# WPCLab/OpenSeg3D

Measured on AMD Instinct MI355X. Metric: points/sec fwd+bwd, Waymo 1-sweep ~180k pts @0.1m voxel; logit parity, higher is better.
Workload: dtype f32 storage/accumulate, bf16x3 products; 1 GPU; waymo_one_sweep (BASELINE configs[1]): synthetic scene, 174633 pts/step/GPU, voxel [0.1, 0.1, 0.1], grid [1440, 1440, 64], fwd (attention dropout p=0.1, DropPath) + criterion (ohem_ce+lovasz on 3 heads) + bwd + SGD step; mode=fwdbwd, segmentor=segformer, voxels=108690, parallelism=dp1

## Files before the change

### __graft_entry__.py

```python
import os
import subprocess
import sys

ROOT = os.path.dirname(os.path.abspath(__file__))
CSRC = os.path.join(ROOT, "openseg3d_amd", "csrc")
LIB = os.path.join(CSRC, "libseg3d_hip.so")
HIP_SOURCES = ["scan.hip", "voxelize.hip", "group.hip", "rulebook.hip", "spconv.hip", "spconv_split.hip", "linear_stream.hip", "linear_x6.hip", "spconv_dma.hip", "spconv_tile.hip", "wgrad_split.hip", "wgrad_dense.hip", "wgrad_dense_lds.hip", "window.hip",
               "attention.hip", "attention_fused.hip", "attention_fused_bwd.hip", "attention_small.hip", "rownorm.hip", "segment.hip", "knn.hip", "knn_attention.hip", "class_context.hip", "loss.hip", "loss_pointwise.hip", "lovasz.hip", "eval.hip", "augment.hip", "augment_instance.hip", "instance_extract.hip", "frame.hip"]
HIPCC_FLAGS = ["--offload-arch=gfx950", "-O3", "-std=c++17", "-fPIC", "-ffp-contract=off",
               "-fhip-fp32-correctly-rounded-divide-sqrt", "-Wall", "-Wno-unused-function"]


def _stale(target, deps):
    if not os.path.exists(target):
        return True
    t = os.path.getmtime(target)
    return any(os.path.getmtime(d) > t for d in deps)


def build_hip(force=False, verbose=False):
    hipcc = os.environ.get("HIPCC", "/opt/rocm/bin/hipcc")
    common = [os.path.join(CSRC, "common.hpp"), os.path.join(CSRC, "attn_common.hpp"), os.path.join(CSRC, "attn_dropout.hpp"), os.path.join(CSRC, "attn_fused.hpp"),
              os.path.join(ROOT, "include", "seg3d_hip.h")]
    objs = []
    procs = []
    for src in HIP_SOURCES:
        s = os.path.join(CSRC, src)
        o = os.path.join(CSRC, src.replace(".hip", ".o"))
        objs.append(o)
        if force or _stale(o, [s] + common):
            cmd = [hipcc] + HIPCC_FLAGS + ["-c", s, "-o", o]
            if verbose:
                print(" ".join(cmd))
            procs.append((src, subprocess.Popen(cmd, stdout=subprocess.PIPE, stderr=subprocess.STDOUT)))
    failed = False
    for src, p in procs:
        out, _ = p.communicate()
        if p.returncode != 0:
            failed = True
            sys.stderr.write(f"--- hipcc failed on {src}\n{out.decode()}\n")
        elif verbose and out.strip():
            print(out.decode())
    if failed:
        raise RuntimeError("hipcc failed")
    if force or procs or _stale(LIB, objs):
        subprocess.check_call([hipcc, "--offload-arch=gfx950", "-shared", "-fPIC", "-o", LIB] + objs)
    return LIB


def build():
    build_hip()
    subprocess.check_call(["make", "-C", os.path.join(ROOT, "oracle")], stdout=subprocess.DEVNULL)
    sys.path.insert(0, ROOT)
    import openseg3d_amd
    from openseg3d_amd import _lib
    _lib.load()


def smoke():
    sys.path.insert(0, ROOT)
    from openseg3d_amd import selfcheck
    selfcheck.run_smoke()


if __name__ == "__main__":
    build_hip(force="--force" in sys.argv, verbose=True)
```

### include/seg3d_hip.h

```cpp
#ifndef SEG3D_HIP_H
#define SEG3D_HIP_H

#include <stddef.h>
#include <stdint.h>

#ifdef __cplusplus
extern "C" {
#endif

#define SEG3D_OK 0
#define SEG3D_EINVAL (-1)
#define SEG3D_EWORKSPACE (-2)
#define SEG3D_ELAUNCH (-3)

#define SEG3D_REDUCE_SUM 0
#define SEG3D_REDUCE_MEAN 1
#define SEG3D_REDUCE_MAX 2

int seg3d_abi_version(void);

const char* seg3d_last_error(void);

int seg3d_grid_size(const float* voxel_size, const float* range, int32_t* grid_xyz);

size_t seg3d_voxelize_workspace_bytes(int64_t n_points);
int seg3d_voxelize_f32(const float* points, int64_t n_points, int32_t row_stride, int32_t xyz_col,
                       int32_t batch_col, const float* voxel_size, const float* range,
                       int32_t* voxel_coords, int32_t* point_voxel_ids, int32_t* n_voxels,
                       void* workspace, size_t workspace_bytes, void* stream);
int seg3d_voxelize_f64(const double* points, int64_t n_points, int32_t row_stride, int32_t xyz_col,
                       int32_t batch_col, const float* voxel_size, const float* range,
                       int32_t* voxel_coords, int32_t* point_voxel_ids, int32_t* n_voxels,
                       void* workspace, size_t workspace_bytes, void* stream);

size_t seg3d_voxelize_host_workspace_bytes(int64_t n_points);
int seg3d_voxelize_host_f32(const float* points, int64_t n_points, int32_t row_stride, int32_t xyz_col,
                            int32_t batch_col, const float* voxel_size, const float* range,
                            int32_t* voxel_coords, int32_t* point_voxel_ids, int32_t* n_voxels,
                            void* workspace, size_t workspace_bytes);
int seg3d_voxelize_host_f64(const double* points, int64_t n_points, int32_t row_stride, int32_t xyz_col,
                            int32_t batch_col, const float* voxel_size, const float* range,
                            int32_t* voxel_coords, int32_t* point_voxel_ids, int32_t* n_voxels,
                            void* workspace, size_t workspace_bytes);

int seg3d_cart2polar_f32(const float* points, int64_t n_points, int32_t row_stride, int32_t xyz_col,
                         float* out , void* stream);
int seg3d_cart2polar_f64(const double* points, int64_t n_points, int32_t row_stride, int32_t xyz_col,
                         double* out , void* stream);

size_t seg3d_group_index_workspace_bytes(int64_t n, int64_t n_groups);
int seg3d_group_index(const int32_t* group_ids, int64_t n, int64_t n_groups, int32_t* rank,
                      int32_t* order, int32_t* offsets, void* workspace, size_t workspace_bytes,
                      void* stream);

size_t seg3d_coord_hash_bytes(int64_t m);
int seg3d_coord_hash_build(const int32_t* coords, int64_t m, const int32_t* shape_zyx ,
                           void* table, size_t table_bytes, void* stream);
int seg3d_rulebook_subm(const int32_t* coords, int64_t m, const int32_t* shape_zyx ,
                        const void* table, size_t table_bytes, int32_t* nbr, void* stream);
size_t seg3d_downsample_workspace_bytes(int32_t batch_size, const int32_t* shape_in_zyx );
int seg3d_downsample_coords(const int32_t* coords_in, int64_t m_in,
                            const int32_t* m_in_dev ,
                            int32_t batch_size, const int32_t* shape_in_zyx , int32_t* coords_out,
                            int64_t cap_out, int32_t* m_out , void* workspace, size_t workspace_bytes,
                            void* stream);
int seg3d_rulebook_strided(const int32_t* coords_out, int64_t m_out, int64_t m_in,
                           const int32_t* shape_in_zyx , const void* table_in,
                           size_t table_bytes, int32_t* nbr_fwd, int32_t* nbr_inv, void* stream);

size_t seg3d_spconv_packed_bytes(int32_t cin, int32_t cout, int32_t flags);
int seg3d_spconv_pack_weight(const float* weight, int32_t cin, int32_t cout, int32_t flags,
                             void* w_packed, void* stream);
int seg3d_spconv_fwd(const float* x, const int32_t* nbr, int64_t m_out, int64_t m_in,
                     const void* w_packed, int32_t pack_flags, const float* bias ,
                     int32_t cin, int32_t cout, float* y,
                     const int32_t* row_order ,
                     void* stream);
int seg3d_spconv_fwd_act(const float* x, const int32_t* nbr, int64_t m_out, int64_t m_in, const void* w_packed,
                         int32_t pack_flags, const float* bias , const float* addend ,
                         int32_t relu, int32_t cin, int32_t cout, float* y, const int32_t* row_order ,
                         void* stream);
int seg3d_spconv_fwd_act_bf16(const void* x, int32_t x_bf16, const int32_t* nbr, int64_t m_out, int64_t m_in,
                              const void* w_packed, int32_t pack_flags, const float* bias,
                              const void* addend_bf16, int32_t relu, int32_t cin, int32_t cout, void* y_bf16,
                              const int32_t* row_order, void* stream);
size_t seg3d_spconv_presplit_bytes(int64_t m_in, int32_t cin);
int seg3d_spconv_presplit(const float* x, int64_t m_in, int32_t cin, void* xs, void* stream);
int seg3d_spconv_fwd_presplit(const void* xs, const int32_t* nbr, int64_t m_out, int64_t m_in, const void* w_packed,
                              int32_t pack_flags, const float* bias , const float* addend ,
                              int32_t relu, int32_t cin, int32_t cout, float* y,
                              const int32_t* row_order , void* stream);
size_t seg3d_conv_plan_bytes(int64_t m_out);
size_t seg3d_conv_plan_workspace_bytes(int64_t m_out);
int seg3d_conv_plan_build(const int32_t* coords, const int32_t* nbr, int64_t m_out, void* plan, void* workspace,
                          size_t workspace_bytes, void* stream);
int32_t seg3d_spconv_tiled_supported(int32_t cin, int32_t cout);
int seg3d_spconv_fwd_tiled(const float* x, const int32_t* nbr, const void* plan, int64_t m_out, int64_t m_in,
                           const void* w_packed, int32_t pack_flags, const float* bias ,
                           const float* addend , int32_t relu, int32_t cin, int32_t cout, float* y, void* stream);
int seg3d_spconv_fwd_tiled_bf16(const void* x, int32_t x_bf16, const int32_t* nbr, const void* plan, int64_t m_out,
                                int64_t m_in, const void* w_packed, int32_t pack_flags, const float* bias ,
                                const void* addend_bf16 , int32_t relu, int32_t cin, int32_t cout, void* y_bf16,
                                void* stream);
int seg3d_debug_set_conv_nbt(int32_t nbt);
int seg3d_debug_set_linear_stream(int32_t on);
size_t seg3d_spconv_wgrad_workspace_bytes(int64_t m_out, int32_t cin, int32_t cout);
int seg3d_spconv_wgrad(const float* x, const float* dy, const int32_t* nbr, int64_t m_out,
                       int64_t m_in, int32_t cin, int32_t cout, int32_t flags ,
                       float* dw, void* workspace, size_t workspace_bytes, void* stream);

int seg3d_spconv_wgrad_partials(const float* x, const float* dy, const int32_t* nbr, int64_t m_out, int64_t m_in,
                                int32_t cin, int32_t cout, void* workspace, size_t workspace_bytes, int32_t* chunks,
                                void* stream);
int seg3d_spconv_wgrad_partials_xbf16(const uint16_t* x_bf16, const float* dy, const int32_t* nbr, int64_t m_out,
                                      int64_t m_in, int32_t cin, int32_t cout, void* workspace, size_t workspace_bytes,
                                      int32_t* chunks, void* stream);

size_t seg3d_linear_wgrad_workspace_bytes(int64_t m, int32_t cin, int32_t cout);
int seg3d_linear_wgrad(const float* x, const float* dy, int64_t m, int32_t cin, int32_t cout, float* dw,
                       float* db , void* workspace, size_t workspace_bytes, void* stream);
int seg3d_linear_wgrad_partials(const float* x, const float* dy, int64_t m, int32_t cin, int32_t cout, int32_t with_bias,
                                void* workspace, size_t workspace_bytes, int32_t* chunks, void* stream);
int seg3d_linear_wgrad_partials_xbf16(const uint16_t* x_bf16, const float* dy, int64_t m, int32_t cin, int32_t cout,
                                      int32_t with_bias, void* workspace, size_t workspace_bytes, int32_t* chunks,
                                      void* stream);
int seg3d_debug_set_wgrad_lds(int32_t on);
int seg3d_reduce_partials(const float* part, int32_t chunks, int64_t n, int64_t nw, float* dw, float* db, void* stream);
int seg3d_reduce_partials_batched(const void* jobs, int32_t n_jobs, int64_t total_blocks, void* stream);
size_t seg3d_linear_packed_bytes_f32(int32_t cin, int32_t cout);
int seg3d_linear_pack_weight_f32(const float* weight, int32_t cin, int32_t cout, int32_t transpose,
                                 void* w_packed, void* stream);
int seg3d_linear_fwd_f32(const float* x, int64_t m, const void* w_packed, const float* bias ,
                         int32_t cin, int32_t cout, float* y, void* stream);
size_t seg3d_linear_packed_bytes_x6(int32_t cin, int32_t cout);
int seg3d_linear_pack_weight_x6(const float* weight, int32_t cin, int32_t cout, int32_t transpose, void* w_packed,
                                void* stream);
int seg3d_linear_fwd_x6(const float* x, int64_t m, const void* w_packed, const float* bias ,
                        const float* scale , const float* shift , int32_t relu, int32_t cin,
                        int32_t cout, float* y, void* stream);

typedef struct {
  const float* src;
  void* dst;
  int32_t cin, cout;
  int32_t kk, transpose, flip, reserved;
  int64_t first_block;
} seg3d_pack_job;
int seg3d_pack_weights_batched(const void* jobs, int32_t n_jobs, int64_t total_blocks, void* stream);

size_t seg3d_linear_packed_bytes(int32_t cin, int32_t cout, int32_t transpose);
int seg3d_linear_pack_weight(const float* weight, int32_t cin, int32_t cout, int32_t transpose,
                             void* w_packed, void* stream);
int seg3d_linear_fwd(const float* x, int64_t m, const void* w_packed, const float* bias ,
                     const float* addend , int32_t cin, int32_t cout,
                     float* y, void* stream);
int seg3d_linear_fwd_sum(const float* x, const float* x_add, int64_t m, const void* w_packed, const float* bias,
                         int32_t cin, int32_t cout, float* y, void* stream);
int seg3d_linear_layernorm_fwd(const float* x, int64_t m, const void* w_packed, const float* bias, const float* res,
                               const float* gamma, const float* beta, float eps, int32_t cin, int32_t cout, float* y,
                               void* stream);
int seg3d_linear_fwd_mul(const float* x, int64_t m, const void* w_packed, const float* factor, int32_t cin, int32_t cout,
                         float* y, void* stream);

size_t seg3d_window_partition_workspace_bytes(int64_t m, int32_t batch_size, const int32_t* nwin_xyz);
int seg3d_window_partition(const int32_t* coords, int64_t m, int32_t batch_size,
                           const int32_t* win_xyz, const int32_t* nwin_xyz, const int32_t* shift_xyz,
                           int32_t n_levels, const int32_t* level_lo, const int32_t* level_hi,
                           const int32_t* level_cap, int32_t* win_id, int32_t* in_win, int32_t* rank,
                           int32_t* level, int32_t* slot, int32_t* tok, int32_t* win_start,
                           int32_t* win_count, int32_t* win_tile0, int32_t* tile_item,
                           int32_t* qg_item, int32_t* counts, void* workspace,
                           size_t workspace_bytes, void* stream);

int seg3d_pos_embed(const int32_t* in_win, int64_t m, const int32_t* win_xyz ,
                    const float* inv_freq, int32_t c, float* pos, void* stream);

int seg3d_window_attn_supported(int32_t heads, int32_t dh);
size_t seg3d_window_attn_workspace_bytes(int64_t m, int32_t n_tiles, int32_t heads, int32_t dh);
int seg3d_window_attn_schedule(int32_t n_tiles, int32_t n_chunks, int32_t heads, int32_t dh, float dropout_p, int32_t* out);
int seg3d_window_attn_fwd(const float* q, const float* k, const float* v, int32_t ldq, int32_t ldk,
                          int32_t ldv, const int32_t* tok, const int32_t* win_start,
                          const int32_t* win_count, const int32_t* win_tile0,
                          const int32_t* tile_item, int32_t n_tiles, const int32_t* qg_item,
                          int32_t n_qgroups, int64_t m, int32_t n_windows, int32_t heads, int32_t dh,
                          const float* tau, float tau_min, float dropout_p, uint64_t dropout_seed, float* out,
                          float* lse, void* workspace, size_t workspace_bytes, void* stream);
int seg3d_window_attn_bwd(const float* q, const float* k, const float* v, int32_t ldq, int32_t ldk,
                          int32_t ldv, const float* out, const float* dout, const float* lse,
                          const int32_t* tok, const int32_t* win_start, const int32_t* win_count,
                          const int32_t* win_tile0, const int32_t* tile_item, int32_t n_tiles,
                          const int32_t* qg_item, int32_t n_qgroups, int64_t m, int32_t n_windows,
                          int32_t heads, int32_t dh, const float* tau,
                          float tau_min, float dropout_p, uint64_t dropout_seed, float* dq, float* dk,
                          float* dv, int32_t lddq, int32_t lddk,
                          int32_t lddv, float* dtau, void* workspace, size_t workspace_bytes,
                          void* stream);

int seg3d_layernorm_fwd(const float* x, const float* res, const float* gamma, const float* beta,
                        const float* rowscale, float eps, int64_t m, int32_t c, float* y, float* mean,
                        float* rstd, void* stream);
size_t seg3d_layernorm_bwd_workspace_bytes(int64_t m, int32_t c);
int seg3d_layernorm_bwd(const float* dy, const float* x, const float* mean, const float* rstd,
                        const float* gamma, const float* rowscale, int64_t m, int32_t c, float* dx,
                        float* dgamma, float* dbeta, void* workspace, size_t workspace_bytes, void* stream);
int seg3d_layernorm_bwd_partials(const float* dy, const float* x, const float* mean, const float* rstd,
                                 const float* gamma, const float* rowscale, int64_t m, int32_t c, float* dx,
                                 void* workspace, size_t workspace_bytes, int32_t* nblocks, void* stream);
size_t seg3d_batchnorm_workspace_bytes(int64_t m, int32_t c);
int seg3d_colstats(const float* x, int64_t m, int32_t c, float* sums, void* workspace, size_t workspace_bytes,
                   void* stream);
int seg3d_batchnorm_stats(const float* x, int64_t m, int32_t c, float eps, const float* gamma, const float* beta,
                          float momentum, float* running_mean, float* running_var, float* stats, void* workspace,
                          size_t workspace_bytes, void* stream);
int seg3d_gelu_fwd(const float* h, int64_t n, float* g, float* gp, void* stream);
int seg3d_affine_act(const float* x, const float* res, const float* scale, const float* shift, int32_t relu,
                     int64_t m, int32_t c, float* y, void* stream);
int seg3d_batchnorm_bwd(const float* dy, const float* y, const float* x, const float* mean, const float* rstd,
                        const float* gamma, int32_t relu, int64_t m, int32_t c, float* dx, float* dres,
                        float* sums, void* workspace, size_t workspace_bytes, void* stream);
int seg3d_batchnorm_bwd_reduce(const float* dy, const float* y, const float* x, const float* mean,
                               const float* rstd, int32_t relu, int64_t m, int32_t c, float* sums,
                               void* workspace, size_t workspace_bytes, void* stream);
int seg3d_batchnorm_bwd_apply(const float* dy, const float* y, const float* x, const float* mean,
                              const float* rstd, const float* gamma, const float* sums, const float* inv_count,
                              int32_t relu, int64_t m, int32_t c, float* dx, float* dres, void* stream);

int seg3d_segment_reduce_fwd(const float* x, int32_t c, const int32_t* order, const int32_t* offsets,
                             int64_t n_seg, int32_t mode, float* out, int32_t* argmax, void* stream);
int seg3d_segment_reduce_bwd(const float* dout, int32_t c, const int32_t* seg_of_row, int64_t n,
                             const int32_t* offsets, const int32_t* argmax, int64_t n_seg,
                             int32_t mode, float* dx, void* stream);

int seg3d_knn_attention_fwd(const float* q, const float* k, const float* v, const int32_t* idx,
                            const uint8_t* invalid, const float* keep, int64_t n, int64_t n_src,
                            int32_t n_neighbors, int32_t d, float scale, float* out, float* prob, void* stream);
int seg3d_knn_attention_bwd(const float* q, const float* k, const float* v, const int32_t* idx, const float* keep,
                            const float* prob, const float* dout, const int32_t* pair_order,
                            const int32_t* pair_offsets, int64_t n, int64_t n_src, int32_t n_neighbors, int32_t d,
                            float scale, float* dq, float* dk, float* dv, float* scratch, void* stream);

int seg3d_class_context_fwd(const float* feats, const float* probs, const int32_t* offsets, const int32_t* chunks,
                            const int32_t* chunk_offsets, int32_t n_chunks, int32_t batch, int64_t m,
                            int32_t classes, int32_t c, float scale, float* weights, float* partials, float* stats,
                            float* context, void* stream);
int seg3d_class_context_bwd(const float* feats, const float* weights, const float* dcontext,
                            const int32_t* offsets, const int32_t* chunks, const int32_t* chunk_offsets,
                            int32_t n_chunks, int32_t batch, int64_t m, int32_t classes, int32_t c, float scale,
                            float* dfeats, float* dprobs, float* scratch, void* stream);

int seg3d_gather_rows(const float* feats, const int32_t* ids, int64_t n, int32_t c, float* out,
                      void* stream);

int seg3d_knn_query(const float* xyz, int64_t n, const float* new_xyz, int64_t m, const int32_t* offset,
                    const int32_t* new_offset, int32_t batch_size, int32_t k, int32_t* idx, float* dist2,
                    void* stream);

size_t seg3d_knn_level_workspace_bytes(int64_t n);
int seg3d_knn_level_build(const float* xyz, int64_t n, const int32_t* offset, int32_t batch_size, float cell,
                          float* sorted_xyz, int32_t* src_index, int32_t* cell_end, void* table_keys, int32_t* table_vals,
                          int64_t capacity, void* workspace, size_t workspace_bytes, void* stream);
int seg3d_knn_query_order(const float* new_xyz, int64_t m, const int32_t* new_offset, int32_t batch_size, float cell,
                          int32_t* order, void* workspace, size_t workspace_bytes, void* stream);
int seg3d_parity_order(const int32_t* coords, int64_t m, int32_t* order, void* workspace, size_t workspace_bytes,
                       void* stream);
typedef struct {
  const float* sorted_xyz;
  const int32_t* src_index;
  const int32_t* cell_end;
  const void* table_keys;
  const int32_t* table_vals;
  int64_t capacity;
  float cell;
  int32_t max_ring;
} seg3d_knn_level;
int seg3d_knn_grid_query(const seg3d_knn_level* levels, int32_t n_levels, const float* new_xyz,
                         const int32_t* query_order , int64_t m,
                         const int32_t* offset, const int32_t* new_offset, int32_t batch_size, int32_t k,
                         int32_t* idx, float* dist2, void* stream);

int seg3d_voxel_majority_labels(const uint8_t* point_labels, const int32_t* order, const int32_t* offsets,
                                int64_t n_voxels, int32_t ignore_index, uint8_t* voxel_labels, void* stream);

size_t seg3d_cross_entropy_workspace_bytes(int64_t n);
int seg3d_cross_entropy_fwd(const float* logits, const int64_t* labels, int64_t n, int32_t c, int64_t ignore_index,
                            float keep_thresh, float* lse, float* stats, void* workspace, size_t workspace_bytes,
                            void* stream);
int seg3d_cross_entropy_bwd(const float* logits, const int64_t* labels, const float* lse, const float* stats,
                            const float* grad_out, int64_t n, int32_t c, float* dlogits, void* stream);

size_t seg3d_lovasz_workspace_bytes(int64_t n, int32_t c);
int seg3d_lovasz_softmax_fwd(const float* logits, const int64_t* labels, int64_t n, int32_t c, int64_t ignore_index,
                             int32_t classes_mode, const int32_t* include, const float* class_weight, float* coef,
                             float* stats, void* workspace, size_t workspace_bytes, void* stream);
int seg3d_lovasz_softmax_bwd(const float* logits, const float* coef, const float* stats, const float* grad_out,
                             int64_t n, int32_t c, float* dlogits, void* stream);

size_t seg3d_pointwise_loss_workspace_bytes(int64_t n);
int seg3d_focal_loss_fwd(const float* logits, const int64_t* labels, int64_t n, int32_t c, int64_t ignore_index, float gamma,
                         float alpha, const float* class_weight, int32_t reduction, float* stats, void* workspace,
                         size_t workspace_bytes, void* stream);
int seg3d_focal_loss_bwd(const float* logits, const int64_t* labels, const float* stats, const float* grad_out, int64_t n,
                         int32_t c, int64_t ignore_index, float gamma, float alpha, const float* class_weight,
                         int32_t reduction, float* dlogits, void* stream);

int seg3d_dice_loss_fwd(const float* logits, const int64_t* labels, int64_t n, int32_t c, int64_t ignore_index, float smooth,
                        float exponent, const float* class_weight, float loss_weight, float avg_factor, float* loss,
                        void* workspace, size_t workspace_bytes, void* stream);
int seg3d_dice_loss_bwd(const float* logits, const int64_t* labels, const float* grad_out, int64_t n, int32_t c,
                        int64_t ignore_index, float smooth, float exponent, const float* class_weight, float loss_weight,
                        float avg_factor, float* dlogits, void* stream);

#define SEG3D_TTA_MAX_VIEWS 64
typedef struct {
  float scale, cos_a, sin_a;
  int32_t flip_x, flip_y;
} seg3d_tta_view;
typedef struct {
  int32_t n_views;
  int32_t batch_period;
  seg3d_tta_view views[SEG3D_TTA_MAX_VIEWS];
} seg3d_tta_table;
int seg3d_tta_views_f32(const float* points, int64_t n_points, int32_t dim, const seg3d_tta_table* table, float* out,
                        void* stream);
int seg3d_tta_views_host_f32(const float* points, int64_t n_points, int32_t dim, const seg3d_tta_table* table,
                             float* out);

int seg3d_softmax_accumulate_f32(const float* logits, int64_t n_points, int32_t n_views, int32_t c, int32_t first,
                                 float* acc, void* stream);

#define SEG3D_ARGMAX_MAX_CLASSES 64
int seg3d_argmax_confusion(const float* scores, const int64_t* pred_in, int64_t n_points, int32_t c, int32_t n_views,
                           const void* labels, int32_t label_bytes, int64_t* pred, int64_t* hist, void* stream);

#define SEG3D_AUG_MAX_PASTE 8
typedef struct {
  double paste_cos[SEG3D_AUG_MAX_PASTE];
  double paste_sin[SEG3D_AUG_MAX_PASTE];
  double offset[3];
  float rot_cos, rot_sin;
  float scale;
  int32_t n_paste;
  int32_t flip_x, flip_y;
  int32_t global_on;
  int32_t batch_col;
  float batch_id;
} seg3d_aug_params;

size_t seg3d_aug_polarmix_workspace_bytes(int64_t n1, int64_t n2);
int seg3d_aug_polarmix_map(const void* points1, int64_t n1, const void* points2, int64_t n2, int32_t dim,
                           int32_t point_bytes, const void* labels2, int32_t label_bytes, int32_t swap, double alpha,
                           double beta, const uint8_t* instance_classes, int32_t n_classes, int32_t n_paste, int64_t cap,
                           int32_t* src, uint8_t* op, int32_t* counts, void* workspace, size_t workspace_bytes,
                           void* stream);
int seg3d_aug_polarmix_map_host(const void* points1, int64_t n1, const void* points2, int64_t n2, int32_t dim,
                                int32_t point_bytes, const void* labels2, int32_t label_bytes, int32_t swap, double alpha,
                                double beta, const uint8_t* instance_classes, int32_t n_classes, int32_t n_paste,
                                int64_t cap, int32_t* src, uint8_t* op, int32_t* counts);

size_t seg3d_aug_far_near_workspace_bytes(int64_t n);
int seg3d_aug_far_near(const void* frame1, int64_t n1, const void* frame2, int64_t n2, int32_t dim, int32_t point_bytes,
                       const int32_t* src, const uint8_t* op, int64_t n_map, const int32_t* idx, int64_t n,
                       const seg3d_aug_params* params , float sample_range, uint8_t* far_flag, int32_t* far_idx,
                       int32_t* near_idx, int32_t* counts, void* workspace, size_t workspace_bytes, void* stream);
int seg3d_aug_far_near_host(const void* frame1, int64_t n1, const void* frame2, int64_t n2, int32_t dim, int32_t point_bytes,
                            const int32_t* src, const uint8_t* op, int64_t n_map, const int32_t* idx, int64_t n,
                            const seg3d_aug_params* params, float sample_range, uint8_t* far_flag, int32_t* far_idx,
                            int32_t* near_idx, int32_t* counts);

size_t seg3d_aug_sample_workspace_bytes(int64_t n);
int seg3d_aug_sample_device(const uint8_t* far_flag, int64_t n, int64_t n_samples, uint64_t seed, int32_t* out,
                            void* workspace, size_t workspace_bytes, void* stream);
int seg3d_aug_sample_host(const uint8_t* far_flag, int64_t n, int64_t n_samples, uint64_t seed, int32_t* out);

size_t seg3d_aug_cur_map_workspace_bytes(int64_t m, int64_t n_points);
int seg3d_aug_cur_map(const int32_t* src, int64_t m, const int32_t* cur_point_indices, int64_t n_cur, int64_t n_points,
                      int32_t* cur_pos, int32_t* cur_gather, int32_t* count, void* workspace, size_t workspace_bytes,
                      void* stream);
int seg3d_aug_cur_map_host(const int32_t* src, int64_t m, const int32_t* cur_point_indices, int64_t n_cur, int64_t n_points,
                           int32_t* cur_pos, int32_t* cur_gather, int32_t* count);

int seg3d_aug_apply_f32(const float* frame1, int64_t n1, const float* frame2, int64_t n2, int32_t dim, const int32_t* src,
                        const uint8_t* op, int64_t n_out, const seg3d_aug_params* params, float* out, void* stream);
int seg3d_aug_apply_f64in(const double* frame1, int64_t n1, const double* frame2, int64_t n2, int32_t dim,
                          const int32_t* src, const uint8_t* op, int64_t n_out, const seg3d_aug_params* params, float* out,
                          void* stream);
int seg3d_aug_apply_host_f32(const float* frame1, int64_t n1, const float* frame2, int64_t n2, int32_t dim,
                             const int32_t* src, const uint8_t* op, int64_t n_out, const seg3d_aug_params* params,
                             float* out);
int seg3d_aug_apply_host_f64in(const double* frame1, int64_t n1, const double* frame2, int64_t n2, int32_t dim,
                               const int32_t* src, const uint8_t* op, int64_t n_out, const seg3d_aug_params* params,
                               float* out);

int seg3d_aug_gather(const void* a, int64_t na, const void* b, int64_t nb, int64_t row_bytes, const int32_t* idx, int64_t m,
                     void* out, void* stream);
int seg3d_aug_gather_host(const void* a, int64_t na, const void* b, int64_t nb, int64_t row_bytes, const int32_t* idx,
                          int64_t m, void* out);

#define SEG3D_AUG_MAX_ANGLES 20
typedef struct {
  int64_t row_begin;
  int32_t n_rows;
  int32_t label;
  double height;
  double loc_noise[3];
  double rot_cos, rot_sin;
  int32_t local_on;
  int32_t flip;
  int32_t n_angles;
  int32_t reserved;
  double ang_cos[SEG3D_AUG_MAX_ANGLES];
  double ang_sin[SEG3D_AUG_MAX_ANGLES];
} seg3d_aug_instance_plan;

size_t seg3d_aug_instance_workspace_bytes(int64_t n, int64_t max_instance_rows, int32_t k);
int seg3d_aug_instance_paste(const void* points, int64_t n, int32_t dim, int32_t point_bytes, const void* labels,
                             int32_t label_bytes, const uint8_t* ground_ids, int32_t n_ground, const double* bank,
                             int64_t bank_rows, const seg3d_aug_instance_plan* plans, int32_t k, int64_t cap_add,
                             double* add_points, void* add_labels, int32_t* decisions, int32_t* counts, void* workspace,
                             size_t workspace_bytes, void* stream);
int seg3d_aug_instance_paste_host(const void* points, int64_t n, int32_t dim, int32_t point_bytes, const void* labels,
                                  int32_t label_bytes, const uint8_t* ground_ids, int32_t n_ground, const double* bank,
                                  int64_t bank_rows, const seg3d_aug_instance_plan* plans, int32_t k, int64_t cap_add,
                                  double* add_points, void* add_labels, int32_t* decisions, int32_t* counts);

typedef struct {
  int32_t label;
  int32_t begin;
  int32_t rows;
  int32_t kept;
  double center[3];
  double radius;
  double height;
} seg3d_instance_cluster;
size_t seg3d_instance_extract_workspace_bytes(int64_t n, int32_t cap_clusters);
int seg3d_instance_extract(const void* points, int64_t n, int32_t dim, int32_t point_bytes, const void* labels,
                           int32_t label_bytes, const uint8_t* target_ids, const int32_t* min_points, int32_t k,
                           const uint8_t* ground_ids, int32_t g, double eps, int32_t cap_clusters, int32_t* point_cluster,
                           int32_t* cluster_rows, seg3d_instance_cluster* clusters, int32_t* counts, void* workspace,
                           size_t workspace_bytes, void* stream);
int seg3d_instance_extract_host(const void* points, int64_t n, int32_t dim, int32_t point_bytes, const void* labels,
                                int32_t label_bytes, const uint8_t* target_ids, const int32_t* min_points, int32_t k,
                                const uint8_t* ground_ids, int32_t g, double eps, int32_t cap_clusters,
                                int32_t* point_cluster, int32_t* cluster_rows, seg3d_instance_cluster* clusters,
                                int32_t* counts);

#define SEG3D_FRAME_MAX_SWEEPS 8
typedef struct {
  const void* rows;
  int64_t n_rows;
  int64_t stride;
  double matrix[12];
  double lag;
  int32_t transform;
  int32_t reserved;
} seg3d_sweep;
typedef struct {
  int32_t n_sweeps;
  int32_t reserved;
  seg3d_sweep sweeps[SEG3D_FRAME_MAX_SWEEPS];
} seg3d_sweep_table;
int seg3d_frame_assemble(const seg3d_sweep_table* table, int32_t dim, int32_t point_bytes, void* out_rows,
                         float* out_f32, float* out_collated, float batch_id, void* stream);
int seg3d_frame_assemble_host(const seg3d_sweep_table* table, int32_t dim, int32_t point_bytes, void* out_rows,
                              float* out_f32, float* out_collated, float batch_id);

size_t seg3d_range_image_workspace_bytes(int32_t rows, int32_t cols);
int seg3d_range_image_labels(const void* pred, int32_t pred_bytes, const int32_t* points_ri, int64_t n, int32_t rows,
                             int32_t cols, int32_t n_classes, int32_t* image1, int32_t* image2, int32_t* n_outside,
                             void* workspace, size_t workspace_bytes, void* stream);
int seg3d_range_image_labels_host(const void* pred, int32_t pred_bytes, const int32_t* points_ri, int64_t n, int32_t rows,
                                  int32_t cols, int32_t n_classes, int32_t* image1, int32_t* image2, int32_t* n_outside);

#ifdef __cplusplus
}
#endif
#endif
```

### openseg3d_amd/_lib.py

```python
import ctypes
import os
import re

_HERE = os.path.dirname(os.path.abspath(__file__))
LIB_PATH = os.path.join(_HERE, "csrc", "libseg3d_hip.so")
HEADER_PATH = os.path.join(os.path.dirname(_HERE), "include", "seg3d_hip.h")

OK, EINVAL, EWORKSPACE, ELAUNCH = 0, -1, -2, -3
REDUCE_SUM, REDUCE_MEAN, REDUCE_MAX = 0, 1, 2
ABI_VERSION = 47

_p, _i32, _i64, _sz, _f = ctypes.c_void_p, ctypes.c_int32, ctypes.c_int64, ctypes.c_size_t, ctypes.c_float
_u64 = ctypes.c_uint64
_d = ctypes.c_double

SIGNATURES = {
    "seg3d_abi_version": (ctypes.c_int, []),
    "seg3d_last_error": (ctypes.c_char_p, []),
    "seg3d_grid_size": (ctypes.c_int, [_p, _p, _p]),
    "seg3d_voxelize_workspace_bytes": (_sz, [_i64]),
    "seg3d_voxelize_f32": (ctypes.c_int, [_p, _i64, _i32, _i32, _i32, _p, _p, _p, _p, _p, _p, _sz, _p]),
    "seg3d_voxelize_f64": (ctypes.c_int, [_p, _i64, _i32, _i32, _i32, _p, _p, _p, _p, _p, _p, _sz, _p]),
    "seg3d_voxelize_host_workspace_bytes": (_sz, [_i64]),
    "seg3d_voxelize_host_f32": (ctypes.c_int, [_p, _i64, _i32, _i32, _i32, _p, _p, _p, _p, _p, _p, _sz]),
    "seg3d_voxelize_host_f64": (ctypes.c_int, [_p, _i64, _i32, _i32, _i32, _p, _p, _p, _p, _p, _p, _sz]),
    "seg3d_cart2polar_f32": (ctypes.c_int, [_p, _i64, _i32, _i32, _p, _p]),
    "seg3d_cart2polar_f64": (ctypes.c_int, [_p, _i64, _i32, _i32, _p, _p]),
    "seg3d_group_index_workspace_bytes": (_sz, [_i64, _i64]),
    "seg3d_group_index": (ctypes.c_int, [_p, _i64, _i64, _p, _p, _p, _p, _sz, _p]),
    "seg3d_coord_hash_bytes": (_sz, [_i64]),
    "seg3d_coord_hash_build": (ctypes.c_int, [_p, _i64, _p, _p, _sz, _p]),
    "seg3d_rulebook_subm": (ctypes.c_int, [_p, _i64, _p, _p, _sz, _p, _p]),
    "seg3d_downsample_workspace_bytes": (_sz, [_i32, _p]),
    "seg3d_downsample_coords": (ctypes.c_int, [_p, _i64, _p, _i32, _p, _p, _i64, _p, _p, _sz, _p]),
    "seg3d_rulebook_strided": (ctypes.c_int, [_p, _i64, _i64, _p, _p, _sz, _p, _p, _p]),
    "seg3d_spconv_packed_bytes": (_sz, [_i32, _i32, _i32]),
    "seg3d_spconv_pack_weight": (ctypes.c_int, [_p, _i32, _i32, _i32, _p, _p]),
    "seg3d_spconv_fwd": (ctypes.c_int, [_p, _p, _i64, _i64, _p, _i32, _p, _i32, _i32, _p, _p, _p]),
    "seg3d_spconv_fwd_act": (ctypes.c_int, [_p, _p, _i64, _i64, _p, _i32, _p, _p, _i32, _i32, _i32, _p, _p, _p]),
    "seg3d_spconv_fwd_act_bf16": (ctypes.c_int, [_p, _i32, _p, _i64, _i64, _p, _i32, _p, _p, _i32, _i32, _i32, _p, _p, _p]),
    "seg3d_spconv_presplit_bytes": (_sz, [_i64, _i32]),
    "seg3d_spconv_presplit": (ctypes.c_int, [_p, _i64, _i32, _p, _p]),
    "seg3d_spconv_fwd_presplit": (ctypes.c_int, [_p, _p, _i64, _i64, _p, _i32, _p, _p, _i32, _i32, _i32, _p, _p, _p]),
    "seg3d_conv_plan_bytes": (_sz, [_i64]),
    "seg3d_conv_plan_workspace_bytes": (_sz, [_i64]),
    "seg3d_conv_plan_build": (ctypes.c_int, [_p, _p, _i64, _p, _p, _sz, _p]),
    "seg3d_spconv_tiled_supported": (_i32, [_i32, _i32]),
    "seg3d_spconv_fwd_tiled": (ctypes.c_int, [_p, _p, _p, _i64, _i64, _p, _i32, _p, _p, _i32, _i32, _i32, _p, _p]),
    "seg3d_spconv_fwd_tiled_bf16": (ctypes.c_int, [_p, _i32, _p, _p, _i64, _i64, _p, _i32, _p, _p, _i32, _i32, _i32, _p, _p]),
    "seg3d_debug_set_conv_nbt": (ctypes.c_int, [_i32]),
    "seg3d_debug_set_linear_stream": (ctypes.c_int, [_i32]),
    "seg3d_spconv_wgrad_workspace_bytes": (_sz, [_i64, _i32, _i32]),
    "seg3d_spconv_wgrad": (ctypes.c_int, [_p, _p, _p, _i64, _i64, _i32, _i32, _i32, _p, _p, _sz, _p]),
    "seg3d_spconv_wgrad_partials": (ctypes.c_int, [_p, _p, _p, _i64, _i64, _i32, _i32, _p, _sz, _p, _p]),
    "seg3d_spconv_wgrad_partials_xbf16": (ctypes.c_int, [_p, _p, _p, _i64, _i64, _i32, _i32, _p, _sz, _p, _p]),
    "seg3d_linear_wgrad_partials_xbf16": (ctypes.c_int, [_p, _p, _i64, _i32, _i32, _i32, _p, ctypes.c_size_t, _p, _p]),
    "seg3d_linear_packed_bytes_f32": (ctypes.c_size_t, [_i32, _i32]),
    "seg3d_linear_pack_weight_f32": (ctypes.c_int, [_p, _i32, _i32, _i32, _p, _p]),
    "seg3d_linear_fwd_f32": (ctypes.c_int, [_p, _i64, _p, _p, _i32, _i32, _p, _p]),
    "seg3d_debug_set_wgrad_lds": (ctypes.c_int, [_i32]),
    "seg3d_linear_packed_bytes_x6": (ctypes.c_size_t, [_i32, _i32]),
    "seg3d_linear_pack_weight_x6": (ctypes.c_int, [_p, _i32, _i32, _i32, _p, _p]),
    "seg3d_linear_fwd_x6": (ctypes.c_int, [_p, _i64, _p, _p, _p, _p, _i32, _i32, _i32, _p, _p]),
    "seg3d_pack_weights_batched": (ctypes.c_int, [_p, _i32, _i64, _p]),
    "seg3d_linear_wgrad_workspace_bytes": (ctypes.c_size_t, [_i64, _i32, _i32]),
    "seg3d_linear_wgrad": (ctypes.c_int, [_p, _p, _i64, _i32, _i32, _p, _p, _p, ctypes.c_size_t, _p]),
    "seg3d_linear_wgrad_partials": (ctypes.c_int, [_p, _p, _i64, _i32, _i32, _i32, _p, ctypes.c_size_t, _p, _p]),
    "seg3d_reduce_partials": (ctypes.c_int, [_p, _i32, _i64, _i64, _p, _p, _p]),
    "seg3d_reduce_partials_batched": (ctypes.c_int, [_p, _i32, _i64, _p]),
    "seg3d_linear_packed_bytes": (_sz, [_i32, _i32, _i32]),
    "seg3d_linear_pack_weight": (ctypes.c_int, [_p, _i32, _i32, _i32, _p, _p]),
    "seg3d_linear_fwd": (ctypes.c_int, [_p, _i64, _p, _p, _p, _i32, _i32, _p, _p]),
    "seg3d_linear_fwd_sum": (ctypes.c_int, [_p, _p, _i64, _p, _p, _i32, _i32, _p, _p]),
    "seg3d_linear_fwd_mul": (ctypes.c_int, [_p, _i64, _p, _p, _i32, _i32, _p, _p]),
    "seg3d_linear_layernorm_fwd": (ctypes.c_int, [_p, _i64, _p, _p, _p, _p, _p, ctypes.c_float, _i32, _i32, _p, _p]),
    "seg3d_window_partition_workspace_bytes": (_sz, [_i64, _i32, _p]),
    "seg3d_window_partition": (ctypes.c_int, [_p, _i64, _i32, _p, _p, _p, _i32, _p, _p, _p,
                                              _p, _p, _p, _p, _p, _p, _p, _p, _p, _p, _p, _p, _p, _sz, _p]),
    "seg3d_pos_embed": (ctypes.c_int, [_p, _i64, _p, _p, _i32, _p, _p]),
    "seg3d_window_attn_supported": (ctypes.c_int, [_i32, _i32]),
    "seg3d_window_attn_workspace_bytes": (_sz, [_i64, _i32, _i32, _i32]),
    "seg3d_window_attn_schedule": (ctypes.c_int, [_i32, _i32, _i32, _i32, _f, _p]),
    "seg3d_window_attn_fwd": (ctypes.c_int, [_p, _p, _p, _i32, _i32, _i32, _p, _p, _p, _p, _p, _i32, _p, _i32,
                                             _i64, _i32, _i32, _i32, _p, _f, _f, _u64, _p, _p, _p, _sz, _p]),
    "seg3d_window_attn_bwd": (ctypes.c_int, [_p, _p, _p, _i32, _i32, _i32, _p, _p, _p, _p, _p, _p, _p, _p, _i32, _p,
                                             _i32, _i64, _i32, _i32, _i32, _p, _f, _f, _u64, _p, _p, _p, _i32, _i32, _i32,
                                             _p, _p, _sz, _p]),
    "seg3d_layernorm_fwd": (ctypes.c_int, [_p, _p, _p, _p, _p, _f, _i64, _i32, _p, _p, _p, _p]),
    "seg3d_layernorm_bwd_workspace_bytes": (ctypes.c_size_t, [_i64, _i32]),
    "seg3d_layernorm_bwd": (ctypes.c_int, [_p, _p, _p, _p, _p, _p, _i64, _i32, _p, _p, _p, _p, ctypes.c_size_t, _p]),
    "seg3d_layernorm_bwd_partials": (ctypes.c_int, [_p, _p, _p, _p, _p, _p, _i64, _i32, _p, _p, ctypes.c_size_t, _p, _p]),
    "seg3d_batchnorm_workspace_bytes": (ctypes.c_size_t, [_i64, _i32]),
    "seg3d_colstats": (ctypes.c_int, [_p, _i64, _i32, _p, _p, ctypes.c_size_t, _p]),
    "seg3d_batchnorm_stats": (ctypes.c_int, [_p, _i64, _i32, _f, _p, _p, _f, _p, _p, _p, _p, ctypes.c_size_t, _p]),
    "seg3d_affine_act": (ctypes.c_int, [_p, _p, _p, _p, _i32, _i64, _i32, _p, _p]),
    "seg3d_gelu_fwd": (ctypes.c_int, [_p, _i64, _p, _p, _p]),
    "seg3d_batchnorm_bwd": (ctypes.c_int, [_p, _p, _p, _p, _p, _p, _i32, _i64, _i32, _p, _p, _p, _p, ctypes.c_size_t, _p]),
    "seg3d_batchnorm_bwd_reduce": (ctypes.c_int, [_p, _p, _p, _p, _p, _i32, _i64, _i32, _p, _p, ctypes.c_size_t, _p]),
    "seg3d_batchnorm_bwd_apply": (ctypes.c_int, [_p, _p, _p, _p, _p, _p, _p, _p, _i32, _i64, _i32, _p, _p, _p]),
    "seg3d_segment_reduce_fwd": (ctypes.c_int, [_p, _i32, _p, _p, _i64, _i32, _p, _p, _p]),
    "seg3d_segment_reduce_bwd": (ctypes.c_int, [_p, _i32, _p, _i64, _p, _p, _i64, _i32, _p, _p]),
    "seg3d_voxel_majority_labels": (ctypes.c_int, [_p, _p, _p, _i64, _i32, _p, _p]),
    "seg3d_cross_entropy_workspace_bytes": (ctypes.c_size_t, [_i64]),
    "seg3d_cross_entropy_fwd": (ctypes.c_int, [_p, _p, _i64, _i32, _i64, _f, _p, _p, _p, ctypes.c_size_t, _p]),
    "seg3d_cross_entropy_bwd": (ctypes.c_int, [_p, _p, _p, _p, _p, _i64, _i32, _p, _p]),
    "seg3d_lovasz_workspace_bytes": (ctypes.c_size_t, [_i64, _i32]),
    "seg3d_lovasz_softmax_fwd": (ctypes.c_int, [_p, _p, _i64, _i32, _i64, _i32, _p, _p, _p, _p, _p, ctypes.c_size_t, _p]),
    "seg3d_lovasz_softmax_bwd": (ctypes.c_int, [_p, _p, _p, _p, _i64, _i32, _p, _p]),
    "seg3d_pointwise_loss_workspace_bytes": (ctypes.c_size_t, [_i64]),
    "seg3d_focal_loss_fwd": (ctypes.c_int, [_p, _p, _i64, _i32, _i64, _f, _f, _p, _i32, _p, _p, ctypes.c_size_t, _p]),
    "seg3d_focal_loss_bwd": (ctypes.c_int, [_p, _p, _p, _p, _i64, _i32, _i64, _f, _f, _p, _i32, _p, _p]),
    "seg3d_dice_loss_fwd": (ctypes.c_int, [_p, _p, _i64, _i32, _i64, _f, _f, _p, _f, _f, _p, _p, ctypes.c_size_t, _p]),
    "seg3d_dice_loss_bwd": (ctypes.c_int, [_p, _p, _p, _i64, _i32, _i64, _f, _f, _p, _f, _f, _p, _p]),
    "seg3d_knn_level_workspace_bytes": (ctypes.c_size_t, [_i64]),
    "seg3d_knn_level_build": (ctypes.c_int, [_p, _i64, _p, _i32, _f, _p, _p, _p, _p, _p, _i64, _p, ctypes.c_size_t, _p]),
    "seg3d_parity_order": (ctypes.c_int, [_p, _i64, _p, _p, ctypes.c_size_t, _p]),
    "seg3d_knn_query_order": (ctypes.c_int, [_p, _i64, _p, _i32, _f, _p, _p, ctypes.c_size_t, _p]),
    "seg3d_knn_grid_query": (ctypes.c_int, [_p, _i32, _p, _p, _i64, _p, _p, _i32, _i32, _p, _p, _p]),
    "seg3d_knn_query": (ctypes.c_int, [_p, _i64, _p, _i64, _p, _p, _i32, _i32, _p, _p, _p]),
    "seg3d_gather_rows": (ctypes.c_int, [_p, _p, _i64, _i32, _p, _p]),
    "seg3d_class_context_fwd": (ctypes.c_int, [_p, _p, _p, _p, _p, _i32, _i32, _i64, _i32, _i32, _f, _p, _p, _p, _p, _p]),
    "seg3d_class_context_bwd": (ctypes.c_int, [_p, _p, _p, _p, _p, _p, _i32, _i32, _i64, _i32, _i32, _f, _p, _p, _p, _p]),
    "seg3d_knn_attention_fwd": (ctypes.c_int, [_p, _p, _p, _p, _p, _p, _i64, _i64, _i32, _i32, _f, _p, _p, _p]),
    "seg3d_knn_attention_bwd": (ctypes.c_int, [_p, _p, _p, _p, _p, _p, _p, _p, _p, _i64, _i64, _i32, _i32, _f, _p, _p, _p, _p, _p]),
    "seg3d_tta_views_f32": (ctypes.c_int, [_p, _i64, _i32, _p, _p, _p]),
    "seg3d_tta_views_host_f32": (ctypes.c_int, [_p, _i64, _i32, _p, _p]),
    "seg3d_softmax_accumulate_f32": (ctypes.c_int, [_p, _i64, _i32, _i32, _i32, _p, _p]),
    "seg3d_argmax_confusion": (ctypes.c_int, [_p, _p, _i64, _i32, _i32, _p, _i32, _p, _p, _p]),
    "seg3d_aug_polarmix_workspace_bytes": (_sz, [_i64, _i64]),
    "seg3d_aug_polarmix_map": (ctypes.c_int, [_p, _i64, _p, _i64, _i32, _i32, _p, _i32, _i32, _d, _d, _p, _i32, _i32, _i64,
                                              _p, _p, _p, _p, _sz, _p]),
    "seg3d_aug_polarmix_map_host": (ctypes.c_int, [_p, _i64, _p, _i64, _i32, _i32, _p, _i32, _i32, _d, _d, _p, _i32, _i32,
                                                   _i64, _p, _p, _p]),
    "seg3d_aug_far_near_workspace_bytes": (_sz, [_i64]),
    "seg3d_aug_far_near": (ctypes.c_int, [_p, _i64, _p, _i64, _i32, _i32, _p, _p, _i64, _p, _i64, _p, _f, _p, _p, _p, _p,
                                          _p, _sz, _p]),
    "seg3d_aug_far_near_host": (ctypes.c_int, [_p, _i64, _p, _i64, _i32, _i32, _p, _p, _i64, _p, _i64, _p, _f, _p, _p, _p,
                                               _p]),
    "seg3d_aug_sample_workspace_bytes": (_sz, [_i64]),
    "seg3d_aug_sample_device": (ctypes.c_int, [_p, _i64, _i64, _u64, _p, _p, _sz, _p]),
    "seg3d_aug_sample_host": (ctypes.c_int, [_p, _i64, _i64, _u64, _p]),
    "seg3d_aug_cur_map_workspace_bytes": (_sz, [_i64, _i64]),
    "seg3d_aug_cur_map": (ctypes.c_int, [_p, _i64, _p, _i64, _i64, _p, _p, _p, _p, _sz, _p]),
    "seg3d_aug_cur_map_host": (ctypes.c_int, [_p, _i64, _p, _i64, _i64, _p, _p, _p]),
    "seg3d_aug_apply_f32": (ctypes.c_int, [_p, _i64, _p, _i64, _i32, _p, _p, _i64, _p, _p, _p]),
    "seg3d_aug_apply_f64in": (ctypes.c_int, [_p, _i64, _p, _i64, _i32, _p, _p, _i64, _p, _p, _p]),
    "seg3d_aug_apply_host_f32": (ctypes.c_int, [_p, _i64, _p, _i64, _i32, _p, _p, _i64, _p, _p]),
    "seg3d_aug_apply_host_f64in": (ctypes.c_int, [_p, _i64, _p, _i64, _i32, _p, _p, _i64, _p, _p]),
    "seg3d_aug_gather": (ctypes.c_int, [_p, _i64, _p, _i64, _i64, _p, _i64, _p, _p]),
    "seg3d_aug_gather_host": (ctypes.c_int, [_p, _i64, _p, _i64, _i64, _p, _i64, _p]),
    "seg3d_aug_instance_workspace_bytes": (_sz, [_i64, _i64, _i32]),
    "seg3d_aug_instance_paste": (ctypes.c_int, [_p, _i64, _i32, _i32, _p, _i32, _p, _i32, _p, _i64, _p, _i32, _i64, _p, _p,
                                                _p, _p, _p, _sz, _p]),
    "seg3d_aug_instance_paste_host": (ctypes.c_int, [_p, _i64, _i32, _i32, _p, _i32, _p, _i32, _p, _i64, _p, _i32, _i64, _p,
                                                     _p, _p, _p]),
    "seg3d_instance_extract_workspace_bytes": (_sz, [_i64, _i32]),
    "seg3d_instance_extract": (ctypes.c_int, [_p, _i64, _i32, _i32, _p, _i32, _p, _p, _i32, _p, _i32, _d, _i32, _p, _p, _p, _p,
                                              _p, _sz, _p]),
    "seg3d_instance_extract_host": (ctypes.c_int, [_p, _i64, _i32, _i32, _p, _i32, _p, _p, _i32, _p, _i32, _d, _i32, _p, _p, _p,
                                                   _p]),
    "seg3d_frame_assemble": (ctypes.c_int, [_p, _i32, _i32, _p, _p, _p, _f, _p]),
    "seg3d_frame_assemble_host": (ctypes.c_int, [_p, _i32, _i32, _p, _p, _p, _f]),
    "seg3d_range_image_workspace_bytes": (_sz, [_i32, _i32]),
    "seg3d_range_image_labels": (ctypes.c_int, [_p, _i32, _p, _i64, _i32, _i32, _i32, _p, _p, _p, _p, _sz, _p]),
    "seg3d_range_image_labels_host": (ctypes.c_int, [_p, _i32, _p, _i64, _i32, _i32, _i32, _p, _p, _p]),
}

_ERR = {EINVAL: "SEG3D_EINVAL (bad argument)", EWORKSPACE: "SEG3D_EWORKSPACE (workspace too small)",
        ELAUNCH: "SEG3D_ELAUNCH (HIP launch/runtime error)"}

_lib = None


class Seg3dError(RuntimeError):
    pass


def header_symbols():
    with open(HEADER_PATH) as f:
        text = f.read()
    text = re.sub(r"/\*.*?\*/", "", text, flags=re.S)
    return sorted(set(re.findall(r"\b(seg3d_[a-z0-9_]+)\s*\(", text)))


def load():
    global _lib
    if _lib is not None:
        return _lib
    if not os.path.exists(LIB_PATH):
        raise Seg3dError(
            f"{LIB_PATH} not found: the HIP library is required (no CPU fallback). "
            "Build it with `python __graft_entry__.py`.")
    import torch
    lib = ctypes.CDLL(LIB_PATH)
    for name, (res, args) in SIGNATURES.items():
        fn = getattr(lib, name)
        fn.restype = res
        fn.argtypes = args
    if lib.seg3d_abi_version() != ABI_VERSION:
        raise Seg3dError(f"libseg3d_hip.so ABI {lib.seg3d_abi_version()} != binding {ABI_VERSION}")
    _lib = lib
    return lib


def call(name, *args):
    lib = load()
    rc = getattr(lib, name)(*args)
    if rc != OK:
        detail = ""
        if rc == ELAUNCH:
            text = lib.seg3d_last_error()
            detail = f": {text.decode(errors='replace')}" if text else ""
        raise Seg3dError(f"{name} failed: {_ERR.get(rc, rc)}{detail}")


def query(name, *args):
    return int(getattr(load(), name)(*args))
```

### openseg3d_amd/csrc/loss.hip

```cpp
#include "common.hpp"

namespace {

constexpr int kThreads = 256;
constexpr int kMaxBlocks = 1024;

__global__ __launch_bounds__(kThreads) void ce_fwd_kernel(const float* __restrict__ x, const int64_t* __restrict__ label,
                                                          int64_t n, int c, int64_t ignore_index, float keep_thresh,
                                                          float* __restrict__ lse,
                                                          float* __restrict__ part ) {
    float loss = 0.f, cnt = 0.f;
    for (int64_t r = (int64_t)blockIdx.x * kThreads + threadIdx.x; r < n; r += (int64_t)gridDim.x * kThreads) {
        const float* row = x + r * c;
        float m = row[0];
        for (int j = 1; j < c; ++j) m = fmaxf(m, row[j]);
        float s = 0.f;
        for (int j = 0; j < c; ++j) s += expf(row[j] - m);
        const float l = m + logf(s);
        const int64_t y = label[r];
        bool counted = y != ignore_index && y >= 0 && y < c;
        if (counted && keep_thresh > 0.f) counted = expf(row[y] - m) / s < keep_thresh;
        lse[r] = counted ? l : INFINITY;
        if (counted) {
            loss += l - row[y];
            cnt += 1.f;
        }
    }
    for (int off = 32; off > 0; off >>= 1) {
        loss += __shfl_xor(loss, off, SEG3D_WAVE);
        cnt += __shfl_xor(cnt, off, SEG3D_WAVE);
    }
    __shared__ float red[2][kThreads / 64];
    if ((threadIdx.x & 63) == 0) {
        red[0][threadIdx.x >> 6] = loss;
        red[1][threadIdx.x >> 6] = cnt;
    }
    __syncthreads();
    if (threadIdx.x == 0) {
        float a = 0.f, b = 0.f;
        for (int w = 0; w < kThreads / 64; ++w) {
            a += red[0][w];
            b += red[1][w];
        }
        part[2 * blockIdx.x] = a;
        part[2 * blockIdx.x + 1] = b;
    }
}

__global__ __launch_bounds__(kThreads) void ce_finalize_kernel(const float* __restrict__ part, int nblocks,
                                                               float* __restrict__ out) {
    float a = 0.f, b = 0.f;
    for (int i = threadIdx.x; i < nblocks; i += kThreads) {
        a += part[2 * i];
        b += part[2 * i + 1];
    }
    for (int off = 32; off > 0; off >>= 1) {
        a += __shfl_xor(a, off, SEG3D_WAVE);
        b += __shfl_xor(b, off, SEG3D_WAVE);
    }
    __shared__ float red[2][kThreads / 64];
    if ((threadIdx.x & 63) == 0) {
        red[0][threadIdx.x >> 6] = a;
        red[1][threadIdx.x >> 6] = b;
    }
    __syncthreads();
    if (threadIdx.x == 0) {
        float sa = 0.f, sb = 0.f;
        for (int w = 0; w < kThreads / 64; ++w) {
            sa += red[0][w];
            sb += red[1][w];
        }
        out[0] = sb > 0.f ? sa / sb : 0.f;
        out[1] = sb;
    }
}

__global__ __launch_bounds__(kThreads) void ce_bwd_kernel(const float* __restrict__ x, const int64_t* __restrict__ label,
                                                          const float* __restrict__ lse, const float* __restrict__ stats,
                                                          const float* __restrict__ gout, int64_t n, int c,
                                                          float* __restrict__ dx) {
    const float cnt = stats[1];
    const float scale = cnt > 0.f ? gout[0] / cnt : 0.f;
    const int64_t total = n * c;
    for (int64_t e = (int64_t)blockIdx.x * kThreads + threadIdx.x; e < total; e += (int64_t)gridDim.x * kThreads) {
        const int64_t r = e / c;
        const int j = (int)(e - r * c);
        const float l = lse[r];
        float g = 0.f;
        if (l != INFINITY) g = (expf(x[e] - l) - (j == label[r] ? 1.f : 0.f)) * scale;
        dx[e] = g;
    }
}

}

extern "C" size_t seg3d_cross_entropy_workspace_bytes(int64_t n) {
    return n < 0 ? 0 : (size_t)kMaxBlocks * 2 * sizeof(float);
}

extern "C" int seg3d_cross_entropy_fwd(const float* logits, const int64_t* labels, int64_t n, int32_t c,
                                       int64_t ignore_index, float keep_thresh, float* lse,
                                       float* stats ,
                                       void* workspace, size_t workspace_bytes, void* stream) {
    if (n < 0 || c <= 0 || c > 4096 || !stats || !workspace || workspace_bytes < seg3d_cross_entropy_workspace_bytes(n))
        return SEG3D_EINVAL;
    if (n > 0 && (!logits || !labels || !lse)) return SEG3D_EINVAL;
    hipStream_t st = as_stream(stream);
    float* part = static_cast<float*>(workspace);
    int nb = (int)(n > 0 ? ceil_div64(n, kThreads) : 0);
    if (nb > kMaxBlocks) nb = kMaxBlocks;
    if (nb > 0) {
        hipLaunchKernelGGL(ce_fwd_kernel, dim3((unsigned)nb), dim3(kThreads), 0, st, logits, labels, n, c, ignore_index,
                           keep_thresh, lse, part);
        SEG3D_CHECK_LAUNCH();
    }
    hipLaunchKernelGGL(ce_finalize_kernel, dim3(1), dim3(kThreads), 0, st, part, nb, stats);
    SEG3D_CHECK_LAUNCH();
    return SEG3D_OK;
}

extern "C" int seg3d_cross_entropy_bwd(const float* logits, const int64_t* labels, const float* lse, const float* stats,
                                       const float* grad_out , int64_t n, int32_t c, float* dlogits,
                                       void* stream) {
    if (n < 0 || c <= 0 || c > 4096 || !stats || !grad_out) return SEG3D_EINVAL;
    if (n == 0) return SEG3D_OK;
    if (!logits || !labels || !lse || !dlogits) return SEG3D_EINVAL;
    int64_t nb = ceil_div64(n * c, (int64_t)kThreads * 4);
    if (nb > 4096) nb = 4096;
    hipLaunchKernelGGL(ce_bwd_kernel, dim3((unsigned)nb), dim3(kThreads), 0, as_stream(stream), logits, labels, lse, stats,
                       grad_out, n, c, dlogits);
    SEG3D_CHECK_LAUNCH();
    return SEG3D_OK;
}
```

### openseg3d_amd/csrc/lovasz.hip

```cpp
#include <cstring>

#include <rocprim/device/device_radix_sort.hpp>

#include "common.hpp"

namespace {

constexpr int kThreads = 256;
constexpr int kItems = 8;
constexpr int kChunk = kThreads * kItems;
constexpr int kMaxClasses = 64;

__device__ __forceinline__ void softmax_stats(const float* __restrict__ row, int c, float* m_out, float* s_out) {
    float m = row[0];
    for (int j = 1; j < c; ++j) m = fmaxf(m, row[j]);
    float s = 0.f;
    for (int j = 0; j < c; ++j) s += expf(row[j] - m);
    *m_out = m;
    *s_out = s;
}

__global__ __launch_bounds__(kThreads) void lovasz_keys(const float* __restrict__ x, const int64_t* __restrict__ label,
                                                        int n, int c, int64_t ignore_index,
                                                        unsigned long long* __restrict__ keys, uint32_t* __restrict__ vals) {
    const int r = blockIdx.x * kThreads + threadIdx.x;
    if (r >= n) return;
    const float* row = x + (int64_t)r * c;
    float m, s;
    softmax_stats(row, c, &m, &s);
    const int64_t y = label[r];
    const bool valid = y != ignore_index;
    for (int j = 0; j < c; ++j) {
        const bool fg = valid && y == j;
        const float err = valid ? fabsf((fg ? 1.f : 0.f) - expf(row[j] - m) / s) : 0.f;
        const int64_t at = (int64_t)j * n + r;
        keys[at] = ((unsigned long long)j << 32) | __float_as_uint(err);
        vals[at] = (uint32_t)r | (fg ? 0x80000000u : 0u);
    }
}

__global__ __launch_bounds__(kThreads) void lovasz_count(const uint32_t* __restrict__ vals, int n, int nchunks,
                                                         int* __restrict__ chunk_cnt ) {
    const int seg = blockIdx.y, chunk = blockIdx.x;
    const uint32_t* v = vals + (int64_t)seg * n;
    int cnt = 0;
    const int base = chunk * kChunk + threadIdx.x * kItems;
    for (int j = 0; j < kItems; ++j)
        if (base + j < n) cnt += (int)(v[base + j] >> 31);
    for (int off = 32; off > 0; off >>= 1) cnt += __shfl_xor(cnt, off, SEG3D_WAVE);
    __shared__ int red[kThreads / 64];
    if ((threadIdx.x & 63) == 0) red[threadIdx.x >> 6] = cnt;
    __syncthreads();
    if (threadIdx.x == 0) {
        int t = 0;
        for (int w = 0; w < kThreads / 64; ++w) t += red[w];
        chunk_cnt[seg * nchunks + chunk] = t;
    }
}

__global__ __launch_bounds__(64) void lovasz_offsets(const int* __restrict__ chunk_cnt, int nchunks,
                                                     int* __restrict__ chunk_off, int* __restrict__ total) {
    const int seg = blockIdx.x, lane = threadIdx.x;
    int carry = 0;
    for (int t0 = 0; t0 < nchunks; t0 += 64) {
        const int i = t0 + lane;
        const int v = i < nchunks ? chunk_cnt[seg * nchunks + i] : 0;
        int inc = v;
        for (int off = 1; off < 64; off <<= 1) {
            const int o = __shfl_up(inc, off, SEG3D_WAVE);
            if (lane >= off) inc += o;
        }
        if (i < nchunks) chunk_off[seg * nchunks + i] = carry + inc - v;
        carry += __shfl(inc, 63, SEG3D_WAVE);
    }
    if (lane == 0) total[seg] = carry;
}

__global__ __launch_bounds__(kThreads) void lovasz_grad(const unsigned long long* __restrict__ keys,
                                                        const uint32_t* __restrict__ vals, int n, int c, int nchunks,
                                                        const int* __restrict__ chunk_off, const int* __restrict__ total,
                                                        float* __restrict__ coef ,
                                                        float* __restrict__ part ) {
    const int seg = blockIdx.y, chunk = blockIdx.x;
    const int cls = c - 1 - seg;
    const int64_t seg0 = (int64_t)seg * n;
    const int base = chunk * kChunk + threadIdx.x * kItems;
    uint32_t v[kItems];
    float err[kItems];
    int mine = 0;
    for (int j = 0; j < kItems; ++j) {
        const bool in = base + j < n;
        v[j] = in ? vals[seg0 + base + j] : 0u;
        err[j] = in ? __uint_as_float((uint32_t)keys[seg0 + base + j]) : 0.f;
        mine += (int)(v[j] >> 31);
    }
    const int lane = threadIdx.x & 63, wave = threadIdx.x >> 6;
    int inc = mine;
    for (int off = 1; off < 64; off <<= 1) {
        const int o = __shfl_up(inc, off, SEG3D_WAVE);
        if (lane >= off) inc += o;
    }
    __shared__ int wsum[kThreads / 64];
    __shared__ float wdot[kThreads / 64];
    if (lane == 63) wsum[wave] = inc;
    __syncthreads();
    int before = chunk_off[seg * nchunks + chunk] + inc - mine;
    for (int w = 0; w < wave; ++w) before += wsum[w];

    const float gts = (float)total[seg];
    float dot = 0.f;
    int cum = before;
    for (int j = 0; j < kItems; ++j) {
        const int k = base + j;
        if (k >= n) break;
        const int fg = (int)(v[j] >> 31);
        const int cum_prev = cum;
        cum += fg;
        float g = 1.f - (gts - (float)cum) / (gts + (float)(k + 1 - cum));
        if (k > 0) g -= 1.f - (gts - (float)cum_prev) / (gts + (float)(k - cum_prev));
        dot += err[j] * g;
        const float sgn = err[j] == 0.f ? 0.f : (fg ? -1.f : 1.f);
        coef[(int64_t)(v[j] & 0x7FFFFFFFu) * c + cls] = sgn * g;
    }
    for (int off = 32; off > 0; off >>= 1) dot += __shfl_xor(dot, off, SEG3D_WAVE);
    if (lane == 0) wdot[wave] = dot;
    __syncthreads();
    if (threadIdx.x == 0) {
        float t = 0.f;
        for (int w = 0; w < kThreads / 64; ++w) t += wdot[w];
        part[seg * nchunks + chunk] = t;
    }
}

__global__ __launch_bounds__(kMaxClasses) void lovasz_finalize(const float* __restrict__ part, const int* __restrict__ total,
                                                               int c, int nchunks, int mode,
                                                               const int32_t* __restrict__ include,
                                                               const float* __restrict__ class_weight,
                                                               float* __restrict__ stats) {
    __shared__ float loss_c[kMaxClasses];
    __shared__ float w_c[kMaxClasses];
    const int cls = threadIdx.x;
    if (cls < c) {
        const int seg = c - 1 - cls;
        float s = 0.f;
        for (int i = 0; i < nchunks; ++i) s += part[seg * nchunks + i];
        bool use = mode == 0 ? total[seg] > 0 : true;
        if (include) use = include[cls] != 0;
        const float w = use ? (class_weight ? class_weight[cls] : 1.f) : 0.f;
        loss_c[cls] = use ? s * w : 0.f;
        w_c[cls] = use ? w : -1.f;
    }
    __syncthreads();
    if (threadIdx.x == 0) {
        float sum = 0.f;
        int used = 0;
        for (int j = 0; j < c; ++j)
            if (w_c[j] >= 0.f) {
                sum += loss_c[j];
                ++used;
            }
        stats[0] = used ? sum / (float)used : 0.f;
        stats[1] = (float)used;
        for (int j = 0; j < c; ++j) stats[2 + j] = (w_c[j] >= 0.f && used) ? w_c[j] / (float)used : 0.f;
    }
}

__global__ __launch_bounds__(kThreads) void lovasz_bwd(const float* __restrict__ x, const float* __restrict__ coef,
                                                       const float* __restrict__ stats, const float* __restrict__ gout,
                                                       int n, int c, float* __restrict__ dx) {
    const int r = blockIdx.x * kThreads + threadIdx.x;
    if (r >= n) return;
    const float* row = x + (int64_t)r * c;
    float m, s;
    softmax_stats(row, c, &m, &s);
    const float g = gout[0];
    const float* cf = coef + (int64_t)r * c;
    float dot = 0.f;
    for (int j = 0; j < c; ++j) dot += expf(row[j] - m) / s * (cf[j] * stats[2 + j] * g);
    float* out = dx + (int64_t)r * c;
    for (int j = 0; j < c; ++j) out[j] = expf(row[j] - m) / s * (cf[j] * stats[2 + j] * g - dot);
}

using Key = unsigned long long;

int class_bits(int c) {
    int b = 0;
    while ((1 << b) < c) ++b;
    return b;
}

struct Plan {
    int64_t total;
    int nchunks;
    size_t sort_bytes;
};

bool make_plan(int64_t n, int c, Plan* pl) {
    pl->total = n * c;
    pl->nchunks = (int)ceil_div64(n, kChunk);
    pl->sort_bytes = 0;
    if (pl->total == 0) return true;
    rocprim::double_buffer<Key> k(nullptr, nullptr);
    rocprim::double_buffer<uint32_t> v(nullptr, nullptr);
    size_t bytes = 0;
    if (rocprim::radix_sort_pairs_desc(nullptr, bytes, k, v, (size_t)pl->total, 0u, 32u + class_bits(c)) != hipSuccess)
        return false;
    pl->sort_bytes = bytes;
    return true;
}

}

extern "C" size_t seg3d_lovasz_workspace_bytes(int64_t n, int32_t c) {
    if (n < 0 || c <= 0 || c > kMaxClasses || n * c >= (int64_t)1 << 31) return 0;
    Plan pl;
    if (!make_plan(n, c, &pl)) return 0;
    const size_t t = (size_t)pl.total, cc = (size_t)c * pl.nchunks;
    return 2 * align_up(t * sizeof(Key), 256) + 2 * align_up(t * sizeof(uint32_t), 256) + align_up(pl.sort_bytes, 256) +
           2 * align_up(cc * sizeof(int), 256) + align_up(cc * sizeof(float), 256) + align_up(c * sizeof(int), 256) + 256;
}

extern "C" int seg3d_lovasz_softmax_fwd(const float* logits, const int64_t* labels, int64_t n, int32_t c,
                                        int64_t ignore_index, int32_t classes_mode, const int32_t* include,
                                        const float* class_weight, float* coef, float* stats, void* workspace,
                                        size_t workspace_bytes, void* stream) {
    if (n < 0 || c <= 0 || c > kMaxClasses || n * c >= (int64_t)1 << 31 || !stats || (classes_mode != 0 && classes_mode != 1))
        return SEG3D_EINVAL;
    hipStream_t st = as_stream(stream);
    Plan pl;
    if (!make_plan(n, c, &pl)) return SEG3D_ELAUNCH;
    const size_t need = seg3d_lovasz_workspace_bytes(n, c);
    if (!workspace || need == 0 || workspace_bytes < need) return SEG3D_EWORKSPACE;
    if (n > 0 && (!logits || !labels || !coef)) return SEG3D_EINVAL;
    const size_t t = (size_t)pl.total, cc = (size_t)c * (size_t)(pl.nchunks > 0 ? pl.nchunks : 0);
    WsCarver ws(workspace);
    Key* k0 = ws.take<Key>(t);
    Key* k1 = ws.take<Key>(t);
    uint32_t* v0 = ws.take<uint32_t>(t);
    uint32_t* v1 = ws.take<uint32_t>(t);
    void* sort_tmp = ws.take<char>(pl.sort_bytes);
    int* chunk_cnt = ws.take<int>(cc);
    int* chunk_off = ws.take<int>(cc);
    float* part = ws.take<float>(cc);
    int* total = ws.take<int>((size_t)c);
    const int ni = (int)n;
    if (n > 0) {
        hipLaunchKernelGGL(lovasz_keys, dim3((unsigned)ceil_div64(n, kThreads)), dim3(kThreads), 0, st, logits, labels, ni, c,
                           ignore_index, k0, v0);
        SEG3D_CHECK_LAUNCH();
        rocprim::double_buffer<Key> kb(k0, k1);
        rocprim::double_buffer<uint32_t> vb(v0, v1);
        size_t bytes = pl.sort_bytes;
        SEG3D_CHECK_HIP(rocprim::radix_sort_pairs_desc(sort_tmp, bytes, kb, vb, t, 0u, 32u + class_bits(c), st));
        const dim3 grid((unsigned)pl.nchunks, (unsigned)c);
        hipLaunchKernelGGL(lovasz_count, grid, dim3(kThreads), 0, st, vb.current(), ni, pl.nchunks, chunk_cnt);
        SEG3D_CHECK_LAUNCH();
        hipLaunchKernelGGL(lovasz_offsets, dim3((unsigned)c), dim3(64), 0, st, chunk_cnt, pl.nchunks, chunk_off, total);
        SEG3D_CHECK_LAUNCH();
        hipLaunchKernelGGL(lovasz_grad, grid, dim3(kThreads), 0, st, kb.current(), vb.current(), ni, c, pl.nchunks, chunk_off,
                           total, coef, part);
        SEG3D_CHECK_LAUNCH();
    } else {
        hipLaunchKernelGGL(lovasz_offsets, dim3((unsigned)c), dim3(64), 0, st, chunk_cnt, 0, chunk_off, total);
        SEG3D_CHECK_LAUNCH();
    }
    hipLaunchKernelGGL(lovasz_finalize, dim3(1), dim3(kMaxClasses), 0, st, part, total, c, pl.nchunks, classes_mode, include,
                       class_weight, stats);
    SEG3D_CHECK_LAUNCH();
    return SEG3D_OK;
}

extern "C" int seg3d_lovasz_softmax_bwd(const float* logits, const float* coef, const float* stats, const float* grad_out,
                                        int64_t n, int32_t c, float* dlogits, void* stream) {
    if (n < 0 || c <= 0 || c > kMaxClasses || n * c >= (int64_t)1 << 31 || !stats || !grad_out) return SEG3D_EINVAL;
    if (n == 0) return SEG3D_OK;
    if (!logits || !coef || !dlogits) return SEG3D_EINVAL;
    hipLaunchKernelGGL(lovasz_bwd, dim3((unsigned)ceil_div64(n, kThreads)), dim3(kThreads), 0, as_stream(stream), logits, coef,
                       stats, grad_out, (int)n, c, dlogits);
    SEG3D_CHECK_LAUNCH();
    return SEG3D_OK;
}
```

### openseg3d_amd/csrc/voxelize.hip

```cpp
#include <cstdio>

#include "common.hpp"

namespace {

constexpr int kThreads = 256;

struct VoxParams {
    int32_t grid[3];
    int32_t row_stride, xyz_col, batch_col;
};

template <typename T>
struct VoxConst {
    T lo[3];
    T vs[3];
};

__device__ __forceinline__ float floor_t(float v) { return floorf(v); }
__device__ __forceinline__ double floor_t(double v) { return floor(v); }

template <typename T>
__global__ __launch_bounds__(kThreads) void vox_insert(const T* __restrict__ pts, int64_t n, VoxParams p,
                                                       VoxConst<T> c, HashView h, uint32_t* __restrict__ slot_of) {
    const int64_t i = (int64_t)blockIdx.x * kThreads + threadIdx.x;
    const int lane = threadIdx.x & 63;
    bool valid = i < n;
    uint64_t key = 0;
    if (valid) {
        const T* row = pts + i * p.row_stride;
        int32_t cc[3];
#pragma unroll
        for (int j = 0; j < 3; ++j) {
            T v = floor_t((row[p.xyz_col + j] - c.lo[j]) / c.vs[j]);
            if (v < (T)0 || v >= (T)p.grid[j]) valid = false;
            cc[j] = (int32_t)v;
        }
        if (valid) {
            int64_t b = p.batch_col >= 0 ? (int64_t)row[p.batch_col] : 0;
            key = (uint64_t)(((b * p.grid[2] + cc[2]) * p.grid[1] + cc[1]) * (int64_t)p.grid[0] + cc[0]);
        }
    }
    const uint32_t klo = (uint32_t)key, khi = (uint32_t)(key >> 32);
    const uint32_t plo = __shfl_up(klo, 1, SEG3D_WAVE), phi = __shfl_up(khi, 1, SEG3D_WAVE);
    const int pvalid = __shfl_up((int)valid, 1, SEG3D_WAVE);
    const bool head = valid && (lane == 0 || !pvalid || plo != klo || phi != khi);
    const unsigned long long heads = __ballot(head);
    uint32_t slot = 0xFFFFFFFFu;
    if (head) {
        slot = (uint32_t)hash_insert_slot(h, key);
        atomicMin(&h.vals[slot], (int32_t)i);
    }
    const unsigned long long below = heads & ((2ull << lane) - 1ull);
    int src = below ? 63 - __clzll((long long)below) : 0;
    const uint32_t run_slot = __shfl(slot, src, SEG3D_WAVE);
    if (i < n) slot_of[i] = valid ? run_slot : 0xFFFFFFFFu;
}

__global__ __launch_bounds__(kThreads) void vox_flag(const uint32_t* __restrict__ slot_of, int64_t n, HashView h,
                                                     uint32_t* __restrict__ flag) {
    const int64_t i = (int64_t)blockIdx.x * kThreads + threadIdx.x;
    if (i >= n) return;
    const uint32_t s = slot_of[i];
    flag[i] = (s != 0xFFFFFFFFu && h.vals[s] == (int32_t)i) ? 1u : 0u;
}

__global__ __launch_bounds__(kThreads) void vox_emit(const uint32_t* __restrict__ slot_of, const uint32_t* __restrict__ rank,
                                                     int64_t n, HashView h, VoxParams p, int32_t* __restrict__ coords,
                                                     int32_t* __restrict__ ids) {
    const int64_t i = (int64_t)blockIdx.x * kThreads + threadIdx.x;
    if (i >= n) return;
    const uint32_t s = slot_of[i];
    if (s == 0xFFFFFFFFu) {
        ids[i] = -1;
        return;
    }
    const int32_t first = h.vals[s];
    const int32_t id = (int32_t)rank[first];
    ids[i] = id;
    if (first == (int32_t)i) {
        uint64_t key = h.keys[s];
        const int32_t x = (int32_t)(key % (uint64_t)p.grid[0]); key /= (uint64_t)p.grid[0];
        const int32_t y = (int32_t)(key % (uint64_t)p.grid[1]); key /= (uint64_t)p.grid[1];
        const int32_t z = (int32_t)(key % (uint64_t)p.grid[2]); key /= (uint64_t)p.grid[2];
        int4 row = make_int4((int32_t)key, z, y, x);
        reinterpret_cast<int4*>(coords)[id] = row;
    }
}

struct VoxWs {
    void* table;
    uint64_t cap;
    uint32_t *slot_of, *flag, *rank, *tmp;
};

VoxWs carve(void* ws, int64_t n) {
    WsCarver c(ws);
    VoxWs w;
    w.cap = hash_capacity(n);
    w.table = c.take<char>(w.cap * 12);
    w.slot_of = c.take<uint32_t>((size_t)n + 1);
    w.flag = c.take<uint32_t>((size_t)n + 1);
    w.rank = c.take<uint32_t>((size_t)n + 1);
    w.tmp = c.take<uint32_t>(scan_tmp_count(n));
    return w;
}

size_t ws_bytes(int64_t n) {
    WsCarver c(nullptr);
    const uint64_t cap = hash_capacity(n);
    c.take<char>(cap * 12);
    c.take<uint32_t>((size_t)n + 1);
    c.take<uint32_t>((size_t)n + 1);
    c.take<uint32_t>((size_t)n + 1);
    c.take<uint32_t>(scan_tmp_count(n));
    return c.off;
}

template <typename T>
int voxelize_impl(const T* points, int64_t n, int32_t row_stride, int32_t xyz_col, int32_t batch_col,
                  const float* voxel_size, const float* range, int32_t* voxel_coords, int32_t* point_voxel_ids,
                  int32_t* n_voxels, void* workspace, size_t workspace_bytes, void* stream) {
    if (n < 0 || n >= (int64_t)0x7F000000 || !voxel_size || !range || !voxel_coords || !n_voxels || !workspace ||
        row_stride < 3 || xyz_col < 0 || xyz_col + 3 > row_stride || batch_col >= row_stride)
        return SEG3D_EINVAL;
    if (n > 0 && (!points || !point_voxel_ids)) return SEG3D_EINVAL;
    if (workspace_bytes < ws_bytes(n)) return SEG3D_EWORKSPACE;
    hipStream_t st = as_stream(stream);
    VoxParams p;
    if (seg3d_grid_size(voxel_size, range, p.grid) != SEG3D_OK) return SEG3D_EINVAL;
    p.row_stride = row_stride;
    p.xyz_col = xyz_col;
    p.batch_col = batch_col;
    VoxConst<T> c;
    for (int j = 0; j < 3; ++j) {
        c.lo[j] = (T)range[j];
        c.vs[j] = (T)voxel_size[j];
    }
    VoxWs w = carve(workspace, n);
    HashView h = hash_view(w.table, w.cap);
    SEG3D_CHECK_HIP(hipMemsetAsync(h.keys, 0xFF, w.cap * 8, st));
    SEG3D_CHECK_HIP(hipMemsetAsync(h.vals, 0x7F, w.cap * 4, st));
    if (n == 0) {
        SEG3D_CHECK_HIP(hipMemsetAsync(n_voxels, 0, 4, st));
        return SEG3D_OK;
    }
    const unsigned nb = (unsigned)ceil_div64(n, kThreads);
    hipLaunchKernelGGL(vox_insert<T>, dim3(nb), dim3(kThreads), 0, st, points, n, p, c, h, w.slot_of);
    SEG3D_CHECK_LAUNCH();
    hipLaunchKernelGGL(vox_flag, dim3(nb), dim3(kThreads), 0, st, w.slot_of, n, h, w.flag);
    SEG3D_CHECK_LAUNCH();
    int rc = scan_exclusive_u32(w.flag, w.rank, n, reinterpret_cast<uint32_t*>(n_voxels), w.tmp, st);
    if (rc != SEG3D_OK) return rc;
    hipLaunchKernelGGL(vox_emit, dim3(nb), dim3(kThreads), 0, st, w.slot_of, w.rank, n, h, p, voxel_coords,
                       point_voxel_ids);
    SEG3D_CHECK_LAUNCH();
    return SEG3D_OK;
}

__device__ __forceinline__ float atan2_t(float y, float x) { return (float)atan2((double)y, (double)x); }
__device__ __forceinline__ double atan2_t(double y, double x) { return atan2(y, x); }
__device__ __forceinline__ float sqrt_t(float v) { return sqrtf(v); }
__device__ __forceinline__ double sqrt_t(double v) { return sqrt(v); }

template <typename T>
__global__ __launch_bounds__(kThreads) void cart2polar_rows(const T* __restrict__ pts, int64_t n, int row_stride, int xyz_col,
                                                            T* __restrict__ out) {
    const int64_t i = (int64_t)blockIdx.x * kThreads + threadIdx.x;
    if (i >= n) return;
    const T* row = pts + i * row_stride;
    T* o = out + i * (row_stride + 2);
    for (int j = 0; j < xyz_col; ++j) o[j] = row[j];
    const T x = row[xyz_col], y = row[xyz_col + 1], z = row[xyz_col + 2];
    o[xyz_col] = sqrt_t(x * x + y * y);
    o[xyz_col + 1] = atan2_t(y, x);
    o[xyz_col + 2] = z;
    o[xyz_col + 3] = x;
    o[xyz_col + 4] = y;
    for (int j = xyz_col + 3; j < row_stride; ++j) o[j + 2] = row[j];
}

template <typename T>
int cart2polar_impl(const T* points, int64_t n, int32_t row_stride, int32_t xyz_col, T* out, void* stream) {
    if (n < 0 || row_stride < 3 || xyz_col < 0 || xyz_col + 3 > row_stride) return SEG3D_EINVAL;
    if (n == 0) return SEG3D_OK;
    if (!points || !out) return SEG3D_EINVAL;
    hipLaunchKernelGGL(cart2polar_rows<T>, dim3((unsigned)ceil_div64(n, kThreads)), dim3(kThreads), 0, as_stream(stream), points, n,
                       row_stride, xyz_col, out);
    SEG3D_CHECK_LAUNCH();
    return SEG3D_OK;
}


inline float floor_h(float v) { return __builtin_floorf(v); }
inline double floor_h(double v) { return __builtin_floor(v); }

inline uint64_t host_capacity(int64_t n) {
    uint64_t cap = 64;
    while (cap < (uint64_t)(2 * n + 2)) cap <<= 1;
    return cap;
}

template <typename T>
int voxelize_host_impl(const T* points, int64_t n, int32_t row_stride, int32_t xyz_col, int32_t batch_col,
                       const float* voxel_size, const float* range, int32_t* voxel_coords, int32_t* point_voxel_ids,
                       int32_t* n_voxels, void* workspace, size_t workspace_bytes) {
    if (n < 0 || n >= (int64_t)0x7F000000 || !voxel_size || !range || !n_voxels || row_stride < 3 || xyz_col < 0 ||
        xyz_col + 3 > row_stride || batch_col >= row_stride)
        return SEG3D_EINVAL;
    if (n > 0 && (!points || !point_voxel_ids || !voxel_coords || !workspace)) return SEG3D_EINVAL;
    const uint64_t cap = host_capacity(n);
    if (n > 0 && workspace_bytes < cap * 12) return SEG3D_EWORKSPACE;
    int32_t grid[3];
    if (seg3d_grid_size(voxel_size, range, grid) != SEG3D_OK) return SEG3D_EINVAL;
    *n_voxels = 0;
    if (n == 0) return SEG3D_OK;
    uint64_t* keys = static_cast<uint64_t*>(workspace);
    int32_t* vals = reinterpret_cast<int32_t*>(keys + cap);
    for (uint64_t s = 0; s < cap; ++s) keys[s] = ~0ull;
    T lo[3], vs[3];
    for (int j = 0; j < 3; ++j) {
        lo[j] = (T)range[j];
        vs[j] = (T)voxel_size[j];
    }
    int32_t count = 0;
    for (int64_t i = 0; i < n; ++i) {
        const T* row = points + i * row_stride;
        int32_t cc[3];
        bool ok = true;
        for (int j = 0; j < 3 && ok; ++j) {
            volatile T d = row[xyz_col + j] - lo[j];
            volatile T q = d / vs[j];
            const T v = floor_h((T)q);
            if (!(v >= (T)0) || v >= (T)grid[j]) ok = false;
            else cc[j] = (int32_t)v;
        }
        if (!ok) {
            point_voxel_ids[i] = -1;
            continue;
        }
        const int64_t b = batch_col >= 0 ? (int64_t)row[batch_col] : 0;
        const uint64_t key = (uint64_t)(((b * grid[2] + cc[2]) * grid[1] + cc[1]) * (int64_t)grid[0] + cc[0]);
        uint64_t h = key * 0x9E3779B97F4A7C15ull;
        uint64_t s = (h ^ (h >> 29)) & (cap - 1);
        while (keys[s] != key && keys[s] != ~0ull) s = (s + 1) & (cap - 1);
        if (keys[s] == ~0ull) {
            keys[s] = key;
            vals[s] = count;
            int32_t* o = voxel_coords + 4 * (int64_t)count;
            o[0] = (int32_t)b;
            o[1] = cc[2];
            o[2] = cc[1];
            o[3] = cc[0];
            ++count;
        }
        point_voxel_ids[i] = vals[s];
    }
    *n_voxels = count;
    return SEG3D_OK;
}

}

extern "C" {

int seg3d_cart2polar_f32(const float* points, int64_t n_points, int32_t row_stride, int32_t xyz_col, float* out, void* stream) {
    return cart2polar_impl<float>(points, n_points, row_stride, xyz_col, out, stream);
}

int seg3d_cart2polar_f64(const double* points, int64_t n_points, int32_t row_stride, int32_t xyz_col, double* out,
                         void* stream) {
    return cart2polar_impl<double>(points, n_points, row_stride, xyz_col, out, stream);
}

int seg3d_abi_version(void) { return 47; }

namespace {
thread_local char g_last_error[320] = "";
}

const char* seg3d_last_error(void) { return g_last_error; }

int seg3d_grid_size(const float* voxel_size, const float* range, int32_t* grid_xyz) {
    if (!voxel_size || !range || !grid_xyz) return SEG3D_EINVAL;
    for (int j = 0; j < 3; ++j) {
        volatile float span = range[3 + j] - range[j];
        volatile float g = span / voxel_size[j];
        grid_xyz[j] = (int32_t)__builtin_rintf(g);
        if (grid_xyz[j] <= 0) return SEG3D_EINVAL;
    }
    return SEG3D_OK;
}

size_t seg3d_voxelize_workspace_bytes(int64_t n_points) { return ws_bytes(n_points < 0 ? 0 : n_points); }

int seg3d_voxelize_f32(const float* points, int64_t n_points, int32_t row_stride, int32_t xyz_col, int32_t batch_col,
                       const float* voxel_size, const float* range, int32_t* voxel_coords, int32_t* point_voxel_ids,
                       int32_t* n_voxels, void* workspace, size_t workspace_bytes, void* stream) {
    return voxelize_impl<float>(points, n_points, row_stride, xyz_col, batch_col, voxel_size, range, voxel_coords,
                                point_voxel_ids, n_voxels, workspace, workspace_bytes, stream);
}

int seg3d_voxelize_f64(const double* points, int64_t n_points, int32_t row_stride, int32_t xyz_col, int32_t batch_col,
                       const float* voxel_size, const float* range, int32_t* voxel_coords, int32_t* point_voxel_ids,
                       int32_t* n_voxels, void* workspace, size_t workspace_bytes, void* stream) {
    return voxelize_impl<double>(points, n_points, row_stride, xyz_col, batch_col, voxel_size, range, voxel_coords,
                                 point_voxel_ids, n_voxels, workspace, workspace_bytes, stream);
}

size_t seg3d_voxelize_host_workspace_bytes(int64_t n_points) { return (size_t)host_capacity(n_points < 0 ? 0 : n_points) * 12; }

int seg3d_voxelize_host_f32(const float* points, int64_t n_points, int32_t row_stride, int32_t xyz_col, int32_t batch_col,
                            const float* voxel_size, const float* range, int32_t* voxel_coords, int32_t* point_voxel_ids,
                            int32_t* n_voxels, void* workspace, size_t workspace_bytes) {
    return voxelize_host_impl<float>(points, n_points, row_stride, xyz_col, batch_col, voxel_size, range, voxel_coords,
                                     point_voxel_ids, n_voxels, workspace, workspace_bytes);
}

int seg3d_voxelize_host_f64(const double* points, int64_t n_points, int32_t row_stride, int32_t xyz_col, int32_t batch_col,
                            const float* voxel_size, const float* range, int32_t* voxel_coords, int32_t* point_voxel_ids,
                            int32_t* n_voxels, void* workspace, size_t workspace_bytes) {
    return voxelize_host_impl<double>(points, n_points, row_stride, xyz_col, batch_col, voxel_size, range, voxel_coords,
                                      point_voxel_ids, n_voxels, workspace, workspace_bytes);
}

}

void seg3d_note_hip_error(int code, const char* file, int line) {
    const char* base = file;
    for (const char* p = file; *p; ++p)
        if (*p == '/') base = p + 1;
    snprintf(g_last_error, sizeof(g_last_error), "%s (%s) at %s:%d", hipGetErrorString((hipError_t)code),
             hipGetErrorName((hipError_t)code), base, line);
}
```

### openseg3d_amd/losses.py

```python
import contextlib
import os

import numpy as np
import torch
import torch.nn as nn
import torch.nn.functional as F

from . import ops


class CrossEntropyLoss(nn.Module):

    def __init__(self, ignore_index=255, loss_name="loss_cross_entropy"):
        super().__init__()
        self.ignore_index = ignore_index
        self._loss_name = loss_name

    def forward(self, inputs, targets):
        return ops.cross_entropy(inputs, targets, ignore_index=self.ignore_index)

    @property
    def loss_name(self):
        return self._loss_name


class OHEMCrossEntropyLoss(nn.Module):
    def __init__(self, keep_ratio=None, keep_thresh=None, ignore_index=255, class_weight=None,
                 loss_name="loss_ohem_cross_entropy"):
        super().__init__()
        self.keep_ratio, self.keep_thresh = keep_ratio, keep_thresh
        self.ignore_index, self.class_weight = ignore_index, class_weight
        self._loss_name = loss_name

    def forward(self, inputs, targets):
        if self.class_weight is None and not self.keep_ratio:
            return ops.cross_entropy(inputs, targets, ignore_index=self.ignore_index, keep_thresh=self.keep_thresh)
        mask = targets != self.ignore_index
        losses = F.cross_entropy(inputs, targets, weight=self.class_weight, ignore_index=self.ignore_index,
                                 reduction="none")[mask]
        if self.keep_ratio:
            kept = int(losses.shape[0] * self.keep_ratio)
            losses = torch.topk(losses, kept, sorted=False)[0]
        elif self.keep_thresh:
            probs = F.softmax(inputs, dim=1)[mask].gather(1, targets[mask].unsqueeze(1)).squeeze(1)
            losses = losses[probs < self.keep_thresh]
        return losses.mean()

    @property
    def loss_name(self):
        return self._loss_name


def _lovasz_grad(gt_sorted):
    gts = gt_sorted.sum()
    intersection = gts - gt_sorted.float().cumsum(0)
    union = gts + (1 - gt_sorted).float().cumsum(0)
    jaccard = 1.0 - intersection / union
    if gt_sorted.shape[0] > 1:
        jaccard = torch.cat([jaccard[:1], jaccard[1:] - jaccard[:-1]])
    return jaccard


def _lovasz_hinge_flat(logits, labels):
    if labels.numel() == 0:
        return logits.sum() * 0.0
    signs = 2.0 * labels.float() - 1.0
    errors_sorted, perm = torch.sort(1.0 - logits * signs, dim=0, descending=True)
    return torch.dot(F.relu(errors_sorted), _lovasz_grad(labels[perm]))


class LovaszLoss(nn.Module):
    def __init__(self, loss_type="multi_class", classes="present", per_image=False, reduction="none", class_weight=None,
                 loss_weight=1.0, ignore_index=255, loss_name="loss_lovasz"):
        super().__init__()
        assert loss_type in ("binary", "multi_class")
        if not per_image:
            assert reduction == "none", "reduction should be 'none' when per_image is False."
        self.loss_type, self.classes, self.per_image, self.reduction = loss_type, classes, per_image, reduction
        self.class_weight, self.loss_weight, self.ignore_index = class_weight, loss_weight, ignore_index
        self._loss_name = loss_name

    def forward(self, cls_score, label, avg_factor=None, reduction_override=None):
        assert reduction_override in (None, "none", "mean", "sum")
        reduction = reduction_override if reduction_override else self.reduction
        if self.loss_type == "multi_class" and not self.per_image:
            return self.loss_weight * ops.lovasz_softmax(cls_score, label, self.ignore_index, self.classes, self.class_weight)
        if self.loss_type == "binary" and not self.per_image:
            valid = label.view(-1) != self.ignore_index
            return self.loss_weight * _lovasz_hinge_flat(cls_score.view(-1)[valid], label.view(-1)[valid])
        raise NotImplementedError("LovaszLoss(per_image=True) on [n, C] rows degenerates to one loss per row; "
                                  "no configuration of the reference uses it")

    @property
    def loss_name(self):
        return self._loss_name


def get_class_weight(class_weight):
    if isinstance(class_weight, str):
        if not class_weight.endswith(".npy"):
            raise ValueError("unsupported class weight file format")
        class_weight = np.load(class_weight)
    return class_weight


def _on_device_path(inputs, targets):
    return (inputs.is_cuda and inputs.dtype == torch.float32 and inputs.dim() == 2 and inputs.shape[1] <= 64
            and targets.dtype == torch.int64 and targets.dim() == 1)


class _ClassWeightCache:

    def _device_weight(self, device):
        if self.class_weight is None:
            return None
        cache = self.__dict__.setdefault("_weight_cache", {})
        if device not in cache:
            cache[device] = torch.as_tensor(np.asarray(self.class_weight), dtype=torch.float32).to(device)
        return cache[device]


class FocalLoss(nn.Module, _ClassWeightCache):

    def __init__(self, gamma=2.0, alpha=0.5, num_classes=-1, ignore_index=255, class_weight=None, reduction="mean",
                 loss_name="loss_focal"):
        super().__init__()
        assert reduction in ("none", "mean", "sum"), "AssertionError: reduction should be 'none', 'mean' or 'sum'"
        assert isinstance(alpha, (float, list)), "AssertionError: alpha should be of type float"
        assert isinstance(gamma, float), "AssertionError: gamma should be of type float"
        assert isinstance(loss_name, str), "AssertionError: loss_name should be of type str"
        if isinstance(alpha, list):
            raise NotImplementedError("FocalLoss: a list alpha passes the reference's assertion but not its forward")
        self.gamma, self.alpha, self.num_classes, self.ignore_index = gamma, alpha, num_classes, ignore_index
        self.class_weight, self.reduction = get_class_weight(class_weight), reduction
        self._loss_name = loss_name

    def forward(self, inputs, targets):
        num_classes = inputs.size(1) if self.num_classes < 0 else self.num_classes
        if (self.reduction != "none" and self.gamma >= 0 and num_classes == inputs.size(1)
                and _on_device_path(inputs, targets)):
            return ops.focal_loss(inputs, targets, gamma=self.gamma, alpha=self.alpha, ignore_index=self.ignore_index,
                                  class_weight=self._device_weight(inputs.device), reduction=self.reduction)
        final_weight = torch.ones(1, inputs.size(1)).type_as(inputs)
        if self.class_weight is not None:
            final_weight = final_weight * inputs.new_tensor(np.asarray(self.class_weight))
        valid_mask = targets != self.ignore_index
        inputs, targets = inputs[valid_mask], targets[valid_mask]
        p = torch.sigmoid(inputs)
        targets = F.one_hot(targets, num_classes).to(inputs.dtype)
        ce_loss = F.binary_cross_entropy_with_logits(inputs, targets, reduction="none")
        p_t = p * targets + (1 - p) * (1 - targets)
        loss = ce_loss * ((1 - p_t) ** self.gamma)
        if self.alpha >= 0:
            loss = (self.alpha * targets + (1 - self.alpha) * (1 - targets)) * loss
        loss = loss * final_weight
        if self.reduction == "mean":
            loss = loss.mean()
        elif self.reduction == "sum":
            loss = loss.sum()
        return loss

    @property
    def loss_name(self):
        return self._loss_name


class DiceLoss(nn.Module, _ClassWeightCache):

    def __init__(self, smooth=1, exponent=2, reduction="mean", class_weight=None, loss_weight=1.0, ignore_index=255,
                 loss_name="loss_dice"):
        super().__init__()
        self.smooth, self.exponent, self.reduction = smooth, exponent, reduction
        self.class_weight = get_class_weight(class_weight)
        self.loss_weight, self.ignore_index = loss_weight, ignore_index
        self._loss_name = loss_name

    def forward(self, pred, target, avg_factor=None, reduction_override=None):
        assert reduction_override in (None, "none", "mean", "sum")
        reduction = reduction_override if reduction_override else self.reduction
        if avg_factor is not None and reduction not in ("mean", "none"):
            raise ValueError('avg_factor can not be used with reduction="sum"')
        divide = avg_factor is not None and reduction == "mean"
        ignore_index = -(1 << 62) if self.ignore_index is None else self.ignore_index
        if _on_device_path(pred, target) and not (divide and avg_factor < 0):
            return ops.dice_loss(pred, target, smooth=self.smooth, exponent=self.exponent, ignore_index=ignore_index,
                                 class_weight=self._device_weight(pred.device), loss_weight=self.loss_weight,
                                 avg_factor=avg_factor if divide else None)
        p = F.softmax(pred, dim=1)
        num_classes = p.shape[1]
        one_hot = F.one_hot(torch.clamp(target.long(), 0, num_classes - 1), num_classes=num_classes)
        valid = (target != ignore_index).long().view(-1, 1)
        num = p * one_hot * valid * 2 + self.smooth
        den = p.pow(self.exponent) + one_hot.pow(self.exponent) + self.smooth
        per_class = (1 - num / den).mean(dim=0)
        if self.class_weight is not None:
            per_class = per_class * p.new_tensor(np.asarray(self.class_weight))
        keep = torch.arange(num_classes, device=p.device) != ignore_index
        loss = self.loss_weight * (per_class * keep).sum() / num_classes
        if divide:
            loss = loss / (avg_factor + torch.finfo(torch.float32).eps)
        return loss

    @property
    def loss_name(self):
        return self._loss_name


def build_criterion(cfg, dataset):
    losses = []
    for name in cfg.MODEL.LOSSES:
        if name == "ce":
            criterion = CrossEntropyLoss(ignore_index=dataset.ignore_index)
        elif name == "ohem_ce":
            criterion = OHEMCrossEntropyLoss(keep_thresh=cfg.MODEL.OHEM_KEEP_THRESH, ignore_index=dataset.ignore_index)
        elif name == "lovasz":
            criterion = LovaszLoss(ignore_index=dataset.ignore_index)
        elif name == "focal":
            criterion = FocalLoss(num_classes=dataset.num_classes, ignore_index=dataset.ignore_index)
        elif name == "dice":
            criterion = DiceLoss(ignore_index=dataset.ignore_index)
        else:
            raise NotImplementedError(name)
        losses.append((criterion, cfg.MODEL.LOSSES[name]))
    return losses


AUX_OVERLAP = os.environ.get("SEG3D_AUX_OVERLAP", "1") != "0"


def compute_loss(pred_result, data_dict, criterion, cfg):
    aux_gt = side = None
    if "aux_voxel_out" in pred_result:
        dev = pred_result["aux_voxel_out"].device
        overlap = AUX_OVERLAP and dev.type == "cuda"
        if overlap:
            main, side = torch.cuda.current_stream(dev), ops.side_stream(dev)
            side.wait_stream(main)
        with torch.no_grad(), torch.cuda.stream(side) if overlap else contextlib.nullcontext():
            aux_gt = ops.aux_voxel_labels(pred_result["voxel_coords"], pred_result["aux_voxel_coords"],
                                          data_dict["voxel_labels"], data_dict["batch_size"], cfg.DATASET.VOXEL_SIZE,
                                          cfg.DATASET.POINT_CLOUD_RANGE)
    loss = 0
    for fn, w in criterion:
        loss = loss + fn(pred_result["point_out"], data_dict["point_labels"]) * w
    if "voxel_out" in pred_result:
        voxel_gt = data_dict["voxel_labels"]
        for fn, w in criterion:
            loss = loss + fn(pred_result["voxel_out"], voxel_gt) * w
    if aux_gt is not None:
        if side is not None:
            main.wait_stream(side)
        for fn, w in criterion:
            loss = loss + cfg.MODEL.AUX_LOSS_WEIGHT * fn(pred_result["aux_voxel_out"], aux_gt) * w
    return loss
```

### openseg3d_amd/ops.py

```python
import ctypes
import weakref
import os

import numpy as np
import torch

from . import _lib
from ._lib import REDUCE_MAX, REDUCE_MEAN, REDUCE_SUM

_F3 = ctypes.c_float * 3
_F6 = ctypes.c_float * 6
_I3 = ctypes.c_int32 * 3


def _need_gpu(*tensors):
    for t in tensors:
        if t is not None and not t.is_cuda:
            raise _lib.Seg3dError("openseg3d_amd ops run on the GPU only (no CPU fallback); got a CPU tensor")


def _ptr(t):
    return None if t is None else ctypes.c_void_p(t.data_ptr())


# ... 1584 lines not shown
        fk.join((w_out, dw_out), (w1, dw1), (w2, dw2), (b_out, db_out), (b1, db1), (b2, db2), (g1, dg1), (be1, dbe1),
                (g2, dg2), (be2, dbe2))
        c_n1.fork = c_n2.fork = None
        ctx.parts = None
        return dx, None, dw_in, db_in, dtau, dw_out, db_out, dg1, dbe1, dw1, db1, dw2, db2, dg2, dbe2, None


def encoder_layer_fits(x, c, hid, heads):
    return (x.is_cuda and x.dim() == 2 and x.dtype == torch.float32 and c % 16 == 0 and hid % 16 == 0 and c <= 512
            and c % heads == 0 and CONV_PRECISION == "bf16x3")


class _SegmentReduceFn(torch.autograd.Function):
    @staticmethod
    def forward(ctx, x, seg, mode):
        x = _f32c(x)
        n, c = x.shape
        out = torch.empty((seg.n_segments, c), dtype=torch.float32, device=x.device)
        arg = torch.empty((seg.n_segments, c), dtype=torch.int32, device=x.device) if mode == REDUCE_MAX else None
        _lib.call("seg3d_segment_reduce_fwd", _ptr(x), c, _ptr(seg.order), _ptr(seg.offsets), seg.n_segments, mode,
                  _ptr(out), _ptr(arg), _stream())
        ctx.seg, ctx.mode, ctx.arg, ctx.n = seg, mode, arg, n
        return out

    @staticmethod
    def backward(ctx, dout):
        dout = _f32c(dout)
        c = dout.shape[1]
        seg = ctx.seg
        if ctx.mode == REDUCE_MAX:
            dx = torch.zeros((ctx.n, c), dtype=torch.float32, device=dout.device)
        else:
            dx = torch.empty((ctx.n, c), dtype=torch.float32, device=dout.device)
        _lib.call("seg3d_segment_reduce_bwd", _ptr(dout), c, _ptr(seg.ids), ctx.n, _ptr(seg.offsets), _ptr(ctx.arg),
                  seg.n_segments, ctx.mode, _ptr(dx), _stream())
        return dx, None, None


def segment_reduce(x, seg, mode):
    _need_gpu(x)
    return _SegmentReduceFn.apply(x, seg, mode)


_MODES = {"sum": REDUCE_SUM, "add": REDUCE_SUM, "mean": REDUCE_MEAN, "max": REDUCE_MAX}


def scatter(src, index, dim=0, reduce="sum", dim_size=None):
    if dim != 0 or src.dim() != 2:
        raise _lib.Seg3dError("scatter: only dim=0 on [N, C] tensors is on this path")
    _need_gpu(src, index)
    n_seg = int(index.max().item()) + 1 if dim_size is None else int(dim_size)
    return segment_reduce(src, SegmentIndex(index, n_seg), _MODES[reduce])


class _GatherRowsFn(torch.autograd.Function):
    @staticmethod
    def forward(ctx, feats, ids, seg):
        feats = _f32c(feats)
        n, c = ids.shape[0], feats.shape[1]
        out = torch.empty((n, c), dtype=torch.float32, device=feats.device)
        _lib.call("seg3d_gather_rows", _ptr(feats), _ptr(ids), n, c, _ptr(out), _stream())
        ctx.ids, ctx.seg, ctx.m = ids, seg, feats.shape[0]
        return out

    @staticmethod
    def backward(ctx, dout):
        dout = _f32c(dout)
        seg = ctx.seg if ctx.seg is not None else SegmentIndex(ctx.ids, ctx.m)
        c = dout.shape[1]
        dfeat = torch.empty((ctx.m, c), dtype=torch.float32, device=dout.device)
        _lib.call("seg3d_segment_reduce_fwd", _ptr(dout), c, _ptr(seg.order), _ptr(seg.offsets), ctx.m, REDUCE_SUM,
                  _ptr(dfeat), None, _stream())
        return dfeat, None, None


def gather_rows(feats, ids, seg=None):
    _need_gpu(feats, ids)
    return _GatherRowsFn.apply(feats, _i32c(ids), seg)


def voxel_to_point(feats, coords):
    return gather_rows(feats, coords)


def voxel_max_pooling(feats, coords):
    return scatter(feats, coords, reduce="max")


def voxel_avg_pooling(feats, coords, counts):
    _need_gpu(feats, coords, counts)
    m = counts.shape[0]
    ids = _i32c(coords)
    ids = torch.where((ids >= 0) & (ids < m), ids, torch.full_like(ids, -1))
    return segment_reduce(feats, SegmentIndex(ids, m), REDUCE_MEAN)


KNN_GRID_MIN_POINTS = int(os.environ.get("SEG3D_KNN_GRID_MIN", "8192"))
KNN_GRID_LEVELS = ((0.05, 2), (0.4, 3), (3.2, 4))
if os.environ.get("SEG3D_KNN_LEVELS"):
    KNN_GRID_LEVELS = tuple((float(a), int(b)) for a, b in (t.split(":") for t in os.environ["SEG3D_KNN_LEVELS"].split(",")))


class _KnnLevel(ctypes.Structure):
    _fields_ = [("sorted_xyz", ctypes.c_void_p), ("src_index", ctypes.c_void_p), ("cell_end", ctypes.c_void_p),
                ("table_keys", ctypes.c_void_p), ("table_vals", ctypes.c_void_p), ("capacity", ctypes.c_int64),
                ("cell", ctypes.c_float), ("max_ring", ctypes.c_int32)]


def knn_query(nsample, xyz, new_xyz, offset, new_offset, levels=None):
    if new_xyz is None:
        new_xyz = xyz
    _need_gpu(xyz, new_xyz, offset, new_offset)
    if xyz.dim() != 2 or new_xyz.dim() != 2 or not xyz.is_contiguous() or not new_xyz.is_contiguous():
        raise _lib.Seg3dError("knn_query: xyz and new_xyz must be contiguous 2-D tensors (knn_query.py:16)")
    xyz, new_xyz = xyz.detach(), new_xyz.detach()
    if xyz.dtype != torch.float32 or new_xyz.dtype != torch.float32:
        raise _lib.Seg3dError("knn_query: float32 coordinates expected")
    n, m = xyz.shape[0], new_xyz.shape[0]
    off, noff = _i32c(offset), _i32c(new_offset)
    idx = torch.empty((m, nsample), dtype=torch.int32, device=xyz.device)
    d2 = torch.empty((m, nsample), dtype=torch.float32, device=xyz.device)
    if n >= KNN_GRID_MIN_POINTS and nsample <= 64 and off.shape[0] <= 255:
        dev = xyz.device
        grid = tuple(levels) if levels is not None else KNN_GRID_LEVELS
        ws_bytes = _lib.query("seg3d_knn_level_workspace_bytes", max(n, m))
        if ws_bytes == 0:
            raise _lib.Seg3dError("seg3d_knn_level_workspace_bytes = 0: no device visible or too many points")
        ws = _workspace(ws_bytes, dev)
        cap = 1 << max(4, (2 * n - 1).bit_length())
        keep, lv = [], (_KnnLevel * len(grid))()
        for li, (cell, max_ring) in enumerate(grid):
            sorted_xyz = torch.empty((n, 3), dtype=torch.float32, device=dev)
            src_index = torch.empty((n,), dtype=torch.int32, device=dev)
            cell_end = torch.empty((n,), dtype=torch.int32, device=dev)
            tkeys = torch.empty((cap,), dtype=torch.int64, device=dev)
            tvals = torch.empty((cap,), dtype=torch.int32, device=dev)
            _lib.call("seg3d_knn_level_build", _ptr(xyz), n, _ptr(off), off.shape[0], float(cell), _ptr(sorted_xyz),
                      _ptr(src_index), _ptr(cell_end), _ptr(tkeys), _ptr(tvals), cap, _ptr(ws), ws_bytes, _stream())
            keep.append((sorted_xyz, src_index, cell_end, tkeys, tvals))
            lv[li] = _KnnLevel(sorted_xyz.data_ptr(), src_index.data_ptr(), cell_end.data_ptr(), tkeys.data_ptr(),
                               tvals.data_ptr(), cap, float(cell), int(max_ring))
        if new_xyz.data_ptr() == xyz.data_ptr() and m == n:
            qorder = keep[0][1]
        else:
            qorder = torch.empty((m,), dtype=torch.int32, device=dev)
            _lib.call("seg3d_knn_query_order", _ptr(new_xyz), m, _ptr(noff), noff.shape[0], float(grid[0][0]), _ptr(qorder),
                      _ptr(ws), ws_bytes, _stream())
        _lib.call("seg3d_knn_grid_query", ctypes.cast(lv, ctypes.c_void_p), len(grid), _ptr(new_xyz),
                  _ptr(qorder), m, _ptr(off), _ptr(noff), off.shape[0], int(nsample), _ptr(idx), _ptr(d2), _stream())
        return idx, torch.sqrt(d2)
    _lib.call("seg3d_knn_query", _ptr(xyz), n, _ptr(new_xyz), m, _ptr(off), _ptr(noff), off.shape[0], int(nsample),
              _ptr(idx), _ptr(d2), _stream())
    return idx, torch.sqrt(d2)


class _KnnAttentionFn(torch.autograd.Function):

    @staticmethod
    def forward(ctx, q, k, v, idx, invalid, keep, scale):
        q, k, v = _f32c(q), _f32c(k), _f32c(v)
        n, d = q.shape
        kk = idx.shape[1]
        out = torch.empty((n, d), dtype=torch.float32, device=q.device)
        need = any(ctx.needs_input_grad[:3])
        prob = torch.empty((n, kk), dtype=torch.float32, device=q.device) if need else None
        _lib.call("seg3d_knn_attention_fwd", _ptr(q), _ptr(k), _ptr(v), _ptr(idx), _ptr(invalid), _ptr(keep), n, k.shape[0], kk, d,
                  float(scale), _ptr(out), _ptr(prob), _stream())
        if need:
            ctx.save_for_backward(q, k, v, idx, keep, prob)
        ctx.scale = scale
        return out

    @staticmethod
    def backward(ctx, dout):
        q, k, v, idx, keep, prob = ctx.saved_tensors
        dout = _f32c(dout)
        n, d = q.shape
        kk, n_src = idx.shape[1], k.shape[0]
        _, order, offsets = group_index(idx.reshape(-1), n_src, rank=False)
        dq = torch.empty_like(q)
        dk = torch.empty_like(k)
        dv = torch.empty_like(v)
        scratch = torch.empty((2 * n * kk,), dtype=torch.float32, device=q.device)
        _lib.call("seg3d_knn_attention_bwd", _ptr(q), _ptr(k), _ptr(v), _ptr(idx), _ptr(keep), _ptr(prob), _ptr(dout),
                  _ptr(order), _ptr(offsets), n, n_src, kk, d, float(ctx.scale), _ptr(dq), _ptr(dk), _ptr(dv), _ptr(scratch),
                  _stream())
        return dq, dk, dv, None, None, None, None


def knn_attention(q, k, v, idx, invalid=None, keep=None, scale=None):
    _need_gpu(q, k, v, idx)
    if q.shape[1] != 32 or k.shape[1] != 32 or v.shape[1] != 32 or idx.dim() != 2 or idx.shape[1] > 16:
        raise _lib.Seg3dError("knn_attention: 32 channels and at most 16 neighbours (DeepFusionBlock, segformer.py:51-53)")
    idx = _i32c(idx)
    inv = None if invalid is None else invalid.to(torch.uint8).contiguous()
    kp = None if keep is None else _f32c(keep)
    return _KnnAttentionFn.apply(q, k, v, idx, inv, kp, (q.shape[1] ** -0.5) if scale is None else float(scale))


class _ClassContextFn(torch.autograd.Function):

    @staticmethod
    def forward(ctx, feats, probs, plan, scale):
        feats, probs = _f32c(feats), _f32c(probs)
        offsets, chunks, chunk_offsets, batch = plan
        m, c = feats.shape
        k = probs.shape[1]
        dev = feats.device
        n_chunks = chunks.shape[0]
        weights = torch.empty((m, k), dtype=torch.float32, device=dev)
        partials = torch.empty((max(n_chunks, 1), k, c), dtype=torch.float32, device=dev)
        stats = torch.empty((batch, k, 2), dtype=torch.float32, device=dev)
        context = torch.empty((batch, k, c), dtype=torch.float32, device=dev)
        _lib.call("seg3d_class_context_fwd", _ptr(feats), _ptr(probs), _ptr(offsets), _ptr(chunks), _ptr(chunk_offsets),
                  n_chunks, batch, m, k, c, float(scale), _ptr(weights), _ptr(partials), _ptr(stats), _ptr(context), _stream())
        ctx.save_for_backward(feats, weights)
        ctx.plan, ctx.scale = plan, scale
        return context

    @staticmethod
    def backward(ctx, dcontext):
        feats, weights = ctx.saved_tensors
        offsets, chunks, chunk_offsets, batch = ctx.plan
        m, c = feats.shape
        k = weights.shape[1]
        dcontext = _f32c(dcontext)
        dfeats = torch.empty_like(feats)
        dprobs = torch.empty_like(weights)
        scratch = torch.empty((m * k + max(chunks.shape[0], 1) * k,), dtype=torch.float32, device=feats.device)
        _lib.call("seg3d_class_context_bwd", _ptr(feats), _ptr(weights), _ptr(dcontext), _ptr(offsets), _ptr(chunks),
                  _ptr(chunk_offsets), chunks.shape[0], batch, m, k, c, float(ctx.scale), _ptr(dfeats), _ptr(dprobs),
                  _ptr(scratch), _stream())
        return dfeats, dprobs, None, None


_CONTEXT_PLANS = {}


def class_context_plan(row_offsets, device):
    key = (tuple(int(o) for o in row_offsets), str(device))
    plan = _CONTEXT_PLANS.get(key)
    if plan is None:
        chunks, chunk_offsets, lo = [], [], 0
        for b, hi in enumerate(key[0]):
            chunks += [(b, r) for r in range(lo, hi, 128)]
            chunk_offsets.append(len(chunks))
            lo = hi
        i32 = dict(dtype=torch.int32, device=device)
        plan = (torch.tensor(key[0], **i32), torch.tensor(chunks, **i32).reshape(-1, 2), torch.tensor(chunk_offsets, **i32),
                len(key[0]))
        if len(_CONTEXT_PLANS) > 16:
            _CONTEXT_PLANS.clear()
        _CONTEXT_PLANS[key] = plan
    return plan


def class_context_fits(classes, channels):
    return 1 <= classes <= 32 and channels % 4 == 0 and 4 <= channels <= 1024 and (classes * channels + 128 * 32) * 4 <= 64 * 1024


def class_context(feats, probs, row_offsets, scale=1.0):
    _need_gpu(feats, probs)
    if not class_context_fits(probs.shape[1], feats.shape[1]):
        raise _lib.Seg3dError("class_context: at most 32 classes, channels a multiple of 4, classes * channels <= 12288")
    return _ClassContextFn.apply(feats, probs, class_context_plan(row_offsets, feats.device), float(scale))


def prepare_voxel_labels(point_voxel_ids, point_labels, n_voxels, ignore_index=255, cur_point_indices=None):
    _need_gpu(point_voxel_ids, point_labels)
    ids = point_voxel_ids if cur_point_indices is None else point_voxel_ids[cur_point_indices]
    if ids.shape[0] != point_labels.shape[0]:
        raise _lib.Seg3dError("prepare_voxel_labels: one label per (current-sweep) point expected")
    seg = SegmentIndex(ids, n_voxels)
    lab = point_labels.to(torch.uint8).contiguous()
    out = torch.empty((int(n_voxels),), dtype=torch.uint8, device=lab.device)
    _lib.call("seg3d_voxel_majority_labels", _ptr(lab), _ptr(seg.order), _ptr(seg.offsets), int(n_voxels), int(ignore_index),
              _ptr(out), _stream())
    return out


def get_voxel_centers(voxel_coords, downsample_scale, voxel_size, point_cloud_range):
    centers = voxel_coords.flip(1).float()
    vs, lo = _grid_constants(tuple(float(v) * float(downsample_scale) for v in voxel_size),
                             tuple(float(v) for v in point_cloud_range[0:3]), centers.device)
    return (centers + 0.5) * vs + lo


_GRID_CONSTANTS = {}


def _grid_constants(voxel_size, lo, device):
    key = (voxel_size, lo, str(device))
    if key not in _GRID_CONSTANTS:
        _GRID_CONSTANTS[key] = (torch.tensor(voxel_size, dtype=torch.float32, device=device),
                                torch.tensor(lo, dtype=torch.float32, device=device))
    return _GRID_CONSTANTS[key]


def _sample_offsets_nosync(batch_col, batch_size):
    ids = torch.arange(batch_size, device=batch_col.device, dtype=batch_col.dtype)
    return (batch_col.view(-1, 1) == ids.view(1, -1)).sum(dim=0).cumsum(0).to(torch.int32)


def aux_voxel_labels(voxel_coords, aux_voxel_coords, voxel_labels, batch_size, voxel_size, point_cloud_range,
                     aux_scale=8.0):
    centers = get_voxel_centers(voxel_coords[:, 1:], 1.0, voxel_size, point_cloud_range).contiguous()
    aux_centers = get_voxel_centers(aux_voxel_coords[:, 1:], aux_scale, voxel_size, point_cloud_range).contiguous()
    off = _sample_offsets_nosync(voxel_coords[:, 0], batch_size)
    aux_off = _sample_offsets_nosync(aux_voxel_coords[:, 0], batch_size)
    pitch = float(max(voxel_size))
    idx, _ = knn_query(1, centers, aux_centers, off, aux_off, levels=((pitch, 0), (8 * pitch, 3), (64 * pitch, 2)))
    return voxel_labels[idx.reshape(-1).long()]


class _CrossEntropyFn(torch.autograd.Function):
    @staticmethod
    def forward(ctx, logits, labels, ignore_index, keep_thresh):
        x = _f32c(logits)
        n, c = x.shape
        lab = labels.contiguous()
        lse = torch.empty((n,), dtype=torch.float32, device=x.device)
        stats = torch.empty((2,), dtype=torch.float32, device=x.device)
        ws_bytes = _lib.query("seg3d_cross_entropy_workspace_bytes", n)
        ws = _workspace(ws_bytes, x.device)
        _lib.call("seg3d_cross_entropy_fwd", _ptr(x), _ptr(lab), n, c, int(ignore_index), float(keep_thresh), _ptr(lse),
                  _ptr(stats), _ptr(ws), ws_bytes, _stream())
        ctx.save_for_backward(x, lab, lse, stats)
        return stats[0]

    @staticmethod
    def backward(ctx, g):
        x, lab, lse, stats = ctx.saved_tensors
        n, c = x.shape
        dx = torch.empty_like(x)
        gg = _f32c(g.reshape(1))
        _lib.call("seg3d_cross_entropy_bwd", _ptr(x), _ptr(lab), _ptr(lse), _ptr(stats), _ptr(gg), n, c, _ptr(dx), _stream())
        return dx, None, None, None


def _loss_args_ok(logits, labels, max_classes):
    return (logits.is_cuda and logits.dim() == 2 and logits.dtype == torch.float32 and labels.dtype == torch.int64
            and labels.dim() == 1 and labels.shape[0] == logits.shape[0] and logits.shape[1] <= max_classes)


def cross_entropy(logits, labels, ignore_index=-100, keep_thresh=None):
    if not _loss_args_ok(logits, labels, 4096):
        raise ValueError("cross_entropy: float32 [n, C <= 4096] logits and int64 [n] labels on the GPU")
    return _CrossEntropyFn.apply(logits, labels, ignore_index, keep_thresh if keep_thresh else 0.0)


def _class_weight_f32(class_weight, c, device, what):
    if class_weight is None:
        return None
    w = _f32c(torch.as_tensor(class_weight, dtype=torch.float32, device=device))
    if tuple(w.shape) != (c,):
        raise ValueError(f"{what}: class_weight must hold one value per class ({c}), got shape {tuple(w.shape)}")
    return w


class _FocalLossFn(torch.autograd.Function):
    @staticmethod
    def forward(ctx, logits, labels, ignore_index, gamma, alpha, class_weight, reduction):
        x = _f32c(logits)
        n, c = x.shape
        lab = labels.contiguous()
        stats = torch.empty((2,), dtype=torch.float32, device=x.device)
        ws_bytes = _lib.query("seg3d_pointwise_loss_workspace_bytes", n)
        ws = _workspace(ws_bytes, x.device)
        _lib.call("seg3d_focal_loss_fwd", _ptr(x), _ptr(lab), n, c, int(ignore_index), float(gamma), float(alpha),
                  _ptr(class_weight) if class_weight is not None else None, reduction, _ptr(stats), _ptr(ws), ws_bytes,
                  _stream())
        ctx.save_for_backward(x, lab, stats, class_weight)
        ctx.args = (int(ignore_index), float(gamma), float(alpha), reduction)
        return stats[0]

    @staticmethod
    def backward(ctx, g):
        x, lab, stats, class_weight = ctx.saved_tensors
        ignore_index, gamma, alpha, reduction = ctx.args
        n, c = x.shape
        dx = torch.empty_like(x)
        gg = _f32c(g.reshape(1))
        _lib.call("seg3d_focal_loss_bwd", _ptr(x), _ptr(lab), _ptr(stats), _ptr(gg), n, c, ignore_index, gamma, alpha,
                  _ptr(class_weight) if class_weight is not None else None, reduction, _ptr(dx), _stream())
        return dx, None, None, None, None, None, None


def focal_loss(logits, labels, gamma=2.0, alpha=0.5, ignore_index=255, class_weight=None, reduction="mean"):
    if not _loss_args_ok(logits, labels, 64):
        raise ValueError("focal_loss: float32 [n, C <= 64] logits and int64 [n] labels on the GPU")
    if reduction not in ("mean", "sum"):
        raise ValueError("focal_loss: reduction 'mean' or 'sum' (the compacted 'none' result is FocalLoss's torch branch)")
    if not float(gamma) >= 0.0:
        raise ValueError("focal_loss: gamma >= 0")
    w = _class_weight_f32(class_weight, logits.shape[1], logits.device, "focal_loss")
    return _FocalLossFn.apply(logits, labels, ignore_index, gamma, alpha, w,
                              _lib.REDUCE_MEAN if reduction == "mean" else _lib.REDUCE_SUM)


class _DiceLossFn(torch.autograd.Function):
    @staticmethod
    def forward(ctx, logits, labels, ignore_index, smooth, exponent, class_weight, loss_weight, avg_factor):
        x = _f32c(logits)
        n, c = x.shape
        lab = labels.contiguous()
        out = torch.empty((1,), dtype=torch.float32, device=x.device)
        ws_bytes = _lib.query("seg3d_pointwise_loss_workspace_bytes", n)
        ws = _workspace(ws_bytes, x.device)
        ctx.args = (int(ignore_index), float(smooth), float(exponent), float(loss_weight), float(avg_factor))
        _lib.call("seg3d_dice_loss_fwd", _ptr(x), _ptr(lab), n, c, ctx.args[0], ctx.args[1], ctx.args[2],
                  _ptr(class_weight) if class_weight is not None else None, ctx.args[3], ctx.args[4], _ptr(out), _ptr(ws),
                  ws_bytes, _stream())
        ctx.save_for_backward(x, lab, class_weight)
        return out[0]

    @staticmethod
    def backward(ctx, g):
        x, lab, class_weight = ctx.saved_tensors
        ignore_index, smooth, exponent, loss_weight, avg_factor = ctx.args
        n, c = x.shape
        dx = torch.empty_like(x)
        gg = _f32c(g.reshape(1))
        _lib.call("seg3d_dice_loss_bwd", _ptr(x), _ptr(lab), _ptr(gg), n, c, ignore_index, smooth, exponent,
                  _ptr(class_weight) if class_weight is not None else None, loss_weight, avg_factor, _ptr(dx), _stream())
        return dx, None, None, None, None, None, None, None


def dice_loss(logits, labels, smooth=1.0, exponent=2.0, ignore_index=255, class_weight=None, loss_weight=1.0,
              avg_factor=None):
    if not _loss_args_ok(logits, labels, 64):
        raise ValueError("dice_loss: float32 [n, C <= 64] logits and int64 [n] labels on the GPU")
    if avg_factor is not None and not float(avg_factor) >= 0.0:
        raise ValueError("dice_loss: avg_factor >= 0")
    w = _class_weight_f32(class_weight, logits.shape[1], logits.device, "dice_loss")
    return _DiceLossFn.apply(logits, labels, ignore_index, smooth, exponent, w, loss_weight,
                             -1.0 if avg_factor is None else avg_factor)


class _LovaszSoftmaxFn(torch.autograd.Function):
    @staticmethod
    def forward(ctx, logits, labels, ignore_index, classes_mode, include, class_weight):
        x = _f32c(logits)
        n, c = x.shape
        lab = labels.contiguous()
        coef = torch.empty((n, c), dtype=torch.float32, device=x.device)
        stats = torch.empty((2 + c,), dtype=torch.float32, device=x.device)
        ws_bytes = _lib.query("seg3d_lovasz_workspace_bytes", n, c)
        if ws_bytes == 0:
            raise _lib.Seg3dError(f"seg3d_lovasz_workspace_bytes({n}, {c}) = 0: n * c must stay below 2^31, c <= 64")
        ws = _workspace(ws_bytes, x.device)
        _lib.call("seg3d_lovasz_softmax_fwd", _ptr(x), _ptr(lab), n, c, int(ignore_index), int(classes_mode),
                  _ptr(include) if include is not None else None, _ptr(class_weight) if class_weight is not None else None,
                  _ptr(coef), _ptr(stats), _ptr(ws), ws_bytes, _stream())
        ctx.save_for_backward(x, coef, stats)
        return stats[0]

    @staticmethod
    def backward(ctx, g):
        x, coef, stats = ctx.saved_tensors
        n, c = x.shape
        dx = torch.empty_like(x)
        gg = _f32c(g.reshape(1))
        _lib.call("seg3d_lovasz_softmax_bwd", _ptr(x), _ptr(coef), _ptr(stats), _ptr(gg), n, c, _ptr(dx), _stream())
        return dx, None, None, None, None, None


def lovasz_softmax(logits, labels, ignore_index=255, classes="present", class_weight=None):
    if not _loss_args_ok(logits, labels, 64):
        raise ValueError("lovasz_softmax: float32 [n, C <= 64] logits and int64 [n] labels on the GPU")
    c = logits.shape[1]
    include = None
    if classes == "present":
        mode = 0
    elif classes == "all":
        mode = 1
    else:
        mode = 1
        include = torch.zeros((c,), dtype=torch.int32)
        include[torch.as_tensor(list(classes), dtype=torch.long)] = 1
        include = include.to(logits.device)
    if class_weight is not None:
        class_weight = _f32c(torch.as_tensor(class_weight, dtype=torch.float32, device=logits.device))
    return _LovaszSoftmaxFn.apply(logits, labels, ignore_index, mode, include, class_weight)


class TtaView(ctypes.Structure):
    _fields_ = [("scale", ctypes.c_float), ("cos_a", ctypes.c_float), ("sin_a", ctypes.c_float),
                ("flip_x", ctypes.c_int32), ("flip_y", ctypes.c_int32)]


TTA_MAX_VIEWS = 64


class TtaTable(ctypes.Structure):
    _fields_ = [("n_views", ctypes.c_int32), ("batch_period", ctypes.c_int32), ("views", TtaView * TTA_MAX_VIEWS)]


def tta_table(scales, angles, flip_x, flip_y, batch_period=0):
    fx = list(flip_x) if isinstance(flip_x, (list, tuple)) else ([True, False] if flip_x else [False])
    fy = list(flip_y) if isinstance(flip_y, (list, tuple)) else ([True, False] if flip_y else [False])
    views = [(s, a, x, y) for s in scales for a in angles for x in fx for y in fy]
    if not 1 <= len(views) <= TTA_MAX_VIEWS:
        raise ValueError(f"{len(views)} test-time views: the kernels take 1 .. {TTA_MAX_VIEWS}")
    ang = torch.tensor([float(a) for _, a, _, _ in views], dtype=torch.float32)
    cos, sin = torch.cos(ang).tolist(), torch.sin(ang).tolist()
    t = TtaTable()
    t.n_views, t.batch_period = len(views), int(batch_period)
    for v, (s, _, x, y) in enumerate(views):
        t.views[v] = TtaView(float(np.float32(s)), cos[v], sin[v], int(bool(x)), int(bool(y)))
    return t


def tta_views(points, table):
    _need_gpu(points)
    if points.dim() != 2 or points.dtype != torch.float32:
        raise _lib.Seg3dError("points must be a float32 [N, D] tensor")
    points = points.contiguous()
    n, d = points.shape
    out = torch.empty((table.n_views * n, d + 1), dtype=torch.float32, device=points.device)
    _lib.call("seg3d_tta_views_f32", _ptr(points), n, d, ctypes.byref(table), _ptr(out), _stream())
    return out


def tta_views_host(points, table):
    pts = np.ascontiguousarray(points, dtype=np.float32)
    if pts.ndim != 2:
        raise _lib.Seg3dError("points must be a float32 [N, D] array")
    n, d = pts.shape
    out = np.empty((table.n_views * n, d + 1), dtype=np.float32)
    _lib.call("seg3d_tta_views_host_f32", ctypes.c_void_p(pts.ctypes.data), n, d, ctypes.byref(table),
              ctypes.c_void_p(out.ctypes.data))
    return out


def softmax_accumulate(logits, acc, first):
    _need_gpu(logits, acc)
    if logits.dtype != torch.float32 or acc.dtype != torch.float32 or not acc.is_contiguous() or acc.dim() != 2 \
            or logits.dim() != 2 or logits.shape[1] != acc.shape[1] or (acc.shape[0] and logits.shape[0] % acc.shape[0]):
        raise _lib.Seg3dError("softmax_accumulate: float32 logits [K*N, C] and a contiguous float32 accumulator [N, C]")
    n, c = acc.shape
    k = logits.shape[0] // n if n else 1
    _lib.call("seg3d_softmax_accumulate_f32", _ptr(logits.contiguous()), n, k, c, int(bool(first)), _ptr(acc), _stream())
    return acc


def argmax_confusion(scores=None, n_classes=None, pred_in=None, labels=None, hist=None, n_views=0, want_pred=True):
    src = scores if scores is not None else pred_in
    _need_gpu(src, labels, hist)
    c = int(scores.shape[1]) if scores is not None else int(n_classes)
    n = int(src.shape[0])
    if scores is not None:
        if scores.dtype != torch.float32 or scores.dim() != 2:
            raise _lib.Seg3dError("scores must be a float32 [N, C] tensor")
        scores = scores.contiguous()
    if pred_in is not None:
        pred_in = pred_in.contiguous() if pred_in.dtype == torch.int64 else pred_in.long().contiguous()
    lb = 0
    if labels is not None:
        if labels.dtype == torch.uint8:
            lb = 1
        elif labels.dtype == torch.int64:
            lb = 8
        else:
            labels = labels.long()
            lb = 8
        labels = labels.contiguous()
        if labels.numel() != n:
            raise _lib.Seg3dError(f"{labels.numel()} labels for {n} points")
    if hist is not None and labels is None:
        raise _lib.Seg3dError("a confusion matrix needs labels")
    if hist is not None and (hist.dtype != torch.int64 or not hist.is_contiguous() or hist.numel() != c * c):
        raise _lib.Seg3dError(f"hist must be a contiguous int64 tensor of {c * c} counters")
    pred = torch.empty((n,), dtype=torch.int64, device=src.device) if want_pred and pred_in is None else None
    _lib.call("seg3d_argmax_confusion", _ptr(scores), _ptr(pred_in), n, c, int(n_views), _ptr(labels), lb, _ptr(pred),
              _ptr(hist), _stream())
    return pred


AUG_MAX_PASTE = 8


class AugParams(ctypes.Structure):
    _fields_ = [("paste_cos", ctypes.c_double * AUG_MAX_PASTE), ("paste_sin", ctypes.c_double * AUG_MAX_PASTE),
                ("offset", ctypes.c_double * 3), ("rot_cos", ctypes.c_float), ("rot_sin", ctypes.c_float),
                ("scale", ctypes.c_float), ("n_paste", ctypes.c_int32), ("flip_x", ctypes.c_int32),
                ("flip_y", ctypes.c_int32), ("global_on", ctypes.c_int32), ("batch_col", ctypes.c_int32),
                ("batch_id", ctypes.c_float)]


def aug_params(paste_angles=(), rot_angle=None, scale=1.0, offsets=(0.0, 0.0, 0.0), flip_x=False, flip_y=False,
               batch_id=None):
    if len(paste_angles) > AUG_MAX_PASTE:
        raise _lib.Seg3dError(f"{len(paste_angles)} paste angles: the kernels take at most {AUG_MAX_PASTE}")
    p = AugParams()
    p.n_paste = len(paste_angles)
    for r, a in enumerate(paste_angles):
        p.paste_cos[r], p.paste_sin[r] = float(np.cos(a)), float(np.sin(a))
    p.global_on = int(rot_angle is not None)
    ang = torch.tensor([0.0 if rot_angle is None else float(rot_angle)], dtype=torch.float64).float()
    p.rot_cos, p.rot_sin = float(torch.cos(ang)[0]), float(torch.sin(ang)[0])
    p.scale = float(np.float32(scale))
    for j in range(3):
        p.offset[j] = float(offsets[j])
    p.flip_x, p.flip_y = int(bool(flip_x)), int(bool(flip_y))
    p.batch_col, p.batch_id = int(batch_id is not None), float(batch_id or 0)
    return p


def _hp(a):
    return None if a is None else ctypes.c_void_p(a.ctypes.data)


def _aug_frames(frame1, frame2, host):
    f32, f64 = (np.float32, np.float64) if host else (torch.float32, torch.float64)
    if host:
        frame1 = np.ascontiguousarray(frame1)
        frame2 = None if frame2 is None else np.ascontiguousarray(frame2)
    else:
        _need_gpu(frame1, frame2)
        frame1 = frame1.contiguous()
        frame2 = None if frame2 is None else frame2.contiguous()
    if frame1.ndim != 2 or frame1.dtype not in (f32, f64):
        raise _lib.Seg3dError("points must be a float32/float64 [N, D] array")
    if frame2 is not None and (frame2.ndim != 2 or frame2.dtype != frame1.dtype or frame2.shape[1] != frame1.shape[1]):
        raise _lib.Seg3dError("both frames must have the same float dtype and the same number of columns")
    d = int(frame1.shape[1])
    if not 3 <= d <= 16:
        raise _lib.Seg3dError(f"points have {d} columns: the augmentation kernels take 3 .. 16")
    return frame1, frame2, int(frame1.shape[0]), 0 if frame2 is None else int(frame2.shape[0]), d, \
        4 if frame1.dtype == f32 else 8


def _aug_labels(labels, host):
    u8, i64 = (np.uint8, np.int64) if host else (torch.uint8, torch.int64)
    if labels.dtype not in (u8, i64) or labels.ndim != 1:
        raise _lib.Seg3dError("labels must be a uint8 or int64 [N] array")
    return (np.ascontiguousarray(labels) if host else labels.contiguous()), (1 if labels.dtype == u8 else 8)


def _aug_classes(instance_classes):
    cls = [int(c) for c in instance_classes]
    if any(c < 0 or c > 255 for c in cls) or len(set(cls)) != len(cls):
        raise _lib.Seg3dError("instance_classes must be distinct labels in 0 .. 255")
    return (ctypes.c_uint8 * max(len(cls), 1))(*cls), len(cls)


def polarmix_map(points1, points2, labels2, swap, alpha, beta, instance_classes, n_paste):
    p1, p2, n1, n2, d, pb = _aug_frames(points1, points2, False)
    _need_gpu(labels2)
    lab, lb = _aug_labels(labels2, False)
    if lab.numel() != n2:
        raise _lib.Seg3dError(f"{lab.numel()} labels for {n2} points")
    cls, nc = _aug_classes(instance_classes)
    dev = p1.device
    cap = n1 + n2 * (2 + int(n_paste))
    src = torch.empty((cap,), dtype=torch.int32, device=dev)
    op = torch.empty((cap,), dtype=torch.uint8, device=dev)
    counts = torch.zeros((4,), dtype=torch.int32, device=dev)
    ws = _workspace(_lib.query("seg3d_aug_polarmix_workspace_bytes", n1, n2), dev)
    _lib.call("seg3d_aug_polarmix_map", _ptr(p1), n1, _ptr(p2), n2, d, pb, _ptr(lab), lb, int(bool(swap)), float(alpha),
              float(beta), cls, nc, int(n_paste), cap, _ptr(src), _ptr(op), _ptr(counts), _ptr(ws), ws.numel(), _stream())
    n_out, base, n_inst, _ = counts.tolist()
    return src[:n_out], op[:n_out], base, n_inst


def polarmix_map_host(points1, points2, labels2, swap, alpha, beta, instance_classes, n_paste):
    p1, p2, n1, n2, d, pb = _aug_frames(points1, points2, True)
    lab, lb = _aug_labels(np.asarray(labels2), True)
    if lab.size != n2:
        raise _lib.Seg3dError(f"{lab.size} labels for {n2} points")
    cls, nc = _aug_classes(instance_classes)
    cap = n1 + n2 * (2 + int(n_paste))
    src = np.empty((cap,), dtype=np.int32)
    op = np.empty((cap,), dtype=np.uint8)
    counts = np.zeros((4,), dtype=np.int32)
    _lib.call("seg3d_aug_polarmix_map_host", _hp(p1), n1, _hp(p2), n2, d, pb, _hp(lab), lb, int(bool(swap)),
              float(alpha), float(beta), cls, nc, int(n_paste), cap, _hp(src), _hp(op), _hp(counts))
    n_out, base, n_inst, _ = counts.tolist()
    return src[:n_out], op[:n_out], base, n_inst


def _aug_map_args(src, op, idx, n1, n2, host):
    i32, u8 = (np.int32, np.uint8) if host else (torch.int32, torch.uint8)
    for name, a, dt in (("src", src, i32), ("op", op, u8), ("idx", idx, i32)):
        if a is not None and (a.dtype != dt or a.ndim != 1):
            raise _lib.Seg3dError(f"{name} must be a 1-d {dt} array")
    if op is not None and (src is None or op.shape[0] != src.shape[0]):
        raise _lib.Seg3dError("op needs a src map of the same length")
    c = (lambda a: None if a is None else np.ascontiguousarray(a)) if host else \
        (lambda a: None if a is None else a.contiguous())
    n_map = n1 + n2 if src is None else int(src.shape[0])
    return c(src), c(op), c(idx), n_map


def aug_far_near(frame1, frame2, src, op, idx, params, sample_range, lists=True):
    f1, f2, n1, n2, d, pb = _aug_frames(frame1, frame2, False)
    _need_gpu(src, op, idx)
    src, op, idx, n_map = _aug_map_args(src, op, idx, n1, n2, False)
    n = n_map if idx is None else int(idx.shape[0])
    dev = f1.device
    if not lists:
        flag = torch.empty((n,), dtype=torch.uint8, device=dev)
        _lib.call("seg3d_aug_far_near", _ptr(f1), n1, _ptr(f2), n2, d, pb, _ptr(src), _ptr(op), n_map, _ptr(idx), n,
                  ctypes.byref(params), float(sample_range), _ptr(flag), None, None, None, None, 0, _stream())
        return flag
    far = torch.empty((max(n, 1),), dtype=torch.int32, device=dev)
    near = torch.empty((max(n, 1),), dtype=torch.int32, device=dev)
    counts = torch.zeros((2,), dtype=torch.int32, device=dev)
    ws = _workspace(_lib.query("seg3d_aug_far_near_workspace_bytes", n), dev)
    _lib.call("seg3d_aug_far_near", _ptr(f1), n1, _ptr(f2), n2, d, pb, _ptr(src), _ptr(op), n_map, _ptr(idx), n,
              ctypes.byref(params), float(sample_range), None, _ptr(far), _ptr(near), _ptr(counts), _ptr(ws), ws.numel(),
              _stream())
    nf, nn = counts.tolist()
    return far[:nf], near[:nn]


def aug_far_near_host(frame1, frame2, src, op, idx, params, sample_range, lists=True):
    f1, f2, n1, n2, d, pb = _aug_frames(frame1, frame2, True)
    src, op, idx, n_map = _aug_map_args(src, op, idx, n1, n2, True)
    n = n_map if idx is None else int(idx.shape[0])
    flag = np.empty((n,), dtype=np.uint8)
    far = np.empty((max(n, 1),), dtype=np.int32)
    near = np.empty((max(n, 1),), dtype=np.int32)
    counts = np.zeros((2,), dtype=np.int32)
    _lib.call("seg3d_aug_far_near_host", _hp(f1), n1, _hp(f2), n2, d, pb, _hp(src), _hp(op), n_map, _hp(idx), n,
              ctypes.byref(params), float(sample_range), _hp(flag), _hp(far), _hp(near), _hp(counts))
    return (far[:counts[0]], near[:counts[1]]) if lists else flag


def aug_sample_device(far_flag, n, n_samples, seed, device=None):
    _need_gpu(far_flag)
    if far_flag is not None and (far_flag.dtype != torch.uint8 or far_flag.numel() != n):
        raise _lib.Seg3dError("far_flag must be a uint8 [n] tensor")
    dev = far_flag.device if far_flag is not None else torch.device(device or "cuda")
    out = torch.empty((int(n_samples),), dtype=torch.int32, device=dev)
    if n_samples:
        ws = _workspace(_lib.query("seg3d_aug_sample_workspace_bytes", int(n)), dev)
        _lib.call("seg3d_aug_sample_device", _ptr(None if far_flag is None else far_flag.contiguous()), int(n),
                  int(n_samples), int(seed) & (2 ** 64 - 1), _ptr(out), _ptr(ws), ws.numel(), _stream())
    return out


def aug_sample_host(far_flag, n, n_samples, seed):
    if far_flag is not None:
        far_flag = np.ascontiguousarray(far_flag, dtype=np.uint8)
        if far_flag.size != n:
            raise _lib.Seg3dError("far_flag must be a uint8 [n] array")
    out = np.empty((int(n_samples),), dtype=np.int32)
    _lib.call("seg3d_aug_sample_host", _hp(far_flag), int(n), int(n_samples), int(seed) & (2 ** 64 - 1), _hp(out))
    return out


def aug_cur_map(src, cur_point_indices, n_points):
    _need_gpu(src, cur_point_indices)
    src, cur = _i32c(src), _i32c(cur_point_indices)
    m, dev = int(src.shape[0]), src.device
    pos = torch.empty((max(m, 1),), dtype=torch.int32, device=dev)
    gat = torch.empty((max(m, 1),), dtype=torch.int32, device=dev)
    count = torch.zeros((1,), dtype=torch.int32, device=dev)
    ws = _workspace(_lib.query("seg3d_aug_cur_map_workspace_bytes", m, int(n_points)), dev)
    _lib.call("seg3d_aug_cur_map", _ptr(src), m, _ptr(cur), int(cur.shape[0]), int(n_points), _ptr(pos), _ptr(gat),
              _ptr(count), _ptr(ws), ws.numel(), _stream())
    k = int(count.item())
    return pos[:k], gat[:k]


def aug_cur_map_host(src, cur_point_indices, n_points):
# ... 328 lines not shown
```

Measured before the change: 4.178 million points/s.

## Batch criterion heads into fused kernels and add lattice-hash nearest lookup for aux labels

Replaces the per-head OHEM cross-entropy and Lovasz loss calls with one batched criterion that processes all three heads through shared row, finish and backward kernels. This cuts kernel launches and separate passes per head. Aux voxel label assignment moves from a multi-level kNN query to a dedicated hash-lattice nearest-neighbour kernel that searches shells of 4x4x4 occupancy blocks and falls back to brute force when needed. The change adds a lot of new kernel code and risks numerical or tie-breaking differences in the loss and label outputs.

```diff
diff --git a/__graft_entry__.py b/__graft_entry__.py
--- a/__graft_entry__.py
+++ b/__graft_entry__.py
@@ -6,7 +6,7 @@
 CSRC = os.path.join(ROOT, "openseg3d_amd", "csrc")
 LIB = os.path.join(CSRC, "libseg3d_hip.so")
 HIP_SOURCES = ["scan.hip", "voxelize.hip", "group.hip", "rulebook.hip", "spconv.hip", "spconv_split.hip", "linear_stream.hip", "linear_x6.hip", "spconv_dma.hip", "spconv_tile.hip", "wgrad_split.hip", "wgrad_dense.hip", "wgrad_dense_lds.hip", "window.hip",
-               "attention.hip", "attention_fused.hip", "attention_fused_bwd.hip", "attention_small.hip", "rownorm.hip", "segment.hip", "knn.hip", "knn_attention.hip", "class_context.hip", "loss.hip", "loss_pointwise.hip", "lovasz.hip", "eval.hip", "augment.hip", "augment_instance.hip", "instance_extract.hip", "frame.hip"]
+               "attention.hip", "attention_fused.hip", "attention_fused_bwd.hip", "attention_small.hip", "rownorm.hip", "segment.hip", "knn.hip", "knn_attention.hip", "class_context.hip", "loss.hip", "loss_pointwise.hip", "lovasz.hip", "lattice_nearest.hip", "eval.hip", "augment.hip", "augment_instance.hip", "instance_extract.hip", "frame.hip"]
 HIPCC_FLAGS = ["--offload-arch=gfx950", "-O3", "-std=c++17", "-fPIC", "-ffp-contract=off",
                "-fhip-fp32-correctly-rounded-divide-sqrt", "-Wall", "-Wno-unused-function"]
 
@@ -20,7 +20,7 @@
 
 def build_hip(force=False, verbose=False):
     hipcc = os.environ.get("HIPCC", "/opt/rocm/bin/hipcc")
-    common = [os.path.join(CSRC, "common.hpp"), os.path.join(CSRC, "attn_common.hpp"), os.path.join(CSRC, "attn_dropout.hpp"), os.path.join(CSRC, "attn_fused.hpp"),
+    common = [os.path.join(CSRC, "common.hpp"), os.path.join(CSRC, "attn_common.hpp"), os.path.join(CSRC, "attn_dropout.hpp"), os.path.join(CSRC, "attn_fused.hpp"), os.path.join(CSRC, "loss_rows.hpp"),
               os.path.join(ROOT, "include", "seg3d_hip.h")]
     objs = []
     procs = []
diff --git a/include/seg3d_hip.h b/include/seg3d_hip.h
--- a/include/seg3d_hip.h
+++ b/include/seg3d_hip.h
@@ -295,6 +295,28 @@
 int seg3d_lovasz_softmax_bwd(const float* logits, const float* coef, const float* stats, const float* grad_out,
                              int64_t n, int32_t c, float* dlogits, void* stream);
 
+typedef struct {
+  const float* logits;
+  const int64_t* labels;
+  int64_t row_offset;
+  int64_t rows;
+  float weight;
+} seg3d_criterion_head;
+size_t seg3d_criterion_workspace_bytes(const seg3d_criterion_head* heads, int32_t n_heads, int32_t c);
+int seg3d_criterion_rows_fwd(const seg3d_criterion_head* heads, int32_t n_heads, int32_t head_begin, int32_t head_end,
+                             int32_t c, int64_t ignore_index, float keep_thresh, float* lse, void* workspace,
+                             size_t workspace_bytes, void* stream);
+int seg3d_criterion_finish_fwd(const seg3d_criterion_head* heads, int32_t n_heads, int32_t c, float w_ce, float w_lovasz,
+                               float* coef, float* stats, void* workspace, size_t workspace_bytes, void* stream);
+int seg3d_criterion_bwd(const seg3d_criterion_head* heads, float* const* dlogits, int32_t n_heads, int32_t c, float w_ce,
+                        float w_lovasz, const float* lse, const float* coef, const float* stats, const float* grad_out,
+                        void* stream);
+
+size_t seg3d_lattice_nearest_workspace_bytes(int64_t m);
+int seg3d_lattice_nearest(const int32_t* fine_coords, int64_t m, const int32_t* coarse_coords, int64_t ma,
+                          const double* voxel_size, const double* origin, int32_t scale, const int64_t* labels, int32_t* idx,
+                          int64_t* labels_out, void* workspace, size_t workspace_bytes, void* stream);
+
 size_t seg3d_pointwise_loss_workspace_bytes(int64_t n);
 int seg3d_focal_loss_fwd(const float* logits, const int64_t* labels, int64_t n, int32_t c, int64_t ignore_index, float gamma,
                          float alpha, const float* class_weight, int32_t reduction, float* stats, void* workspace,
diff --git a/openseg3d_amd/_lib.py b/openseg3d_amd/_lib.py
--- a/openseg3d_amd/_lib.py
+++ b/openseg3d_amd/_lib.py
@@ -8,7 +8,7 @@
 
 OK, EINVAL, EWORKSPACE, ELAUNCH = 0, -1, -2, -3
 REDUCE_SUM, REDUCE_MEAN, REDUCE_MAX = 0, 1, 2
-ABI_VERSION = 47
+ABI_VERSION = 48
 
 _p, _i32, _i64, _sz, _f = ctypes.c_void_p, ctypes.c_int32, ctypes.c_int64, ctypes.c_size_t, ctypes.c_float
 _u64 = ctypes.c_uint64
@@ -107,6 +107,12 @@
     "seg3d_lovasz_workspace_bytes": (ctypes.c_size_t, [_i64, _i32]),
     "seg3d_lovasz_softmax_fwd": (ctypes.c_int, [_p, _p, _i64, _i32, _i64, _i32, _p, _p, _p, _p, _p, ctypes.c_size_t, _p]),
     "seg3d_lovasz_softmax_bwd": (ctypes.c_int, [_p, _p, _p, _p, _i64, _i32, _p, _p]),
+    "seg3d_criterion_workspace_bytes": (ctypes.c_size_t, [_p, _i32, _i32]),
+    "seg3d_criterion_rows_fwd": (ctypes.c_int, [_p, _i32, _i32, _i32, _i32, _i64, _f, _p, _p, ctypes.c_size_t, _p]),
+    "seg3d_criterion_finish_fwd": (ctypes.c_int, [_p, _i32, _i32, _f, _f, _p, _p, _p, ctypes.c_size_t, _p]),
+    "seg3d_criterion_bwd": (ctypes.c_int, [_p, _p, _i32, _i32, _f, _f, _p, _p, _p, _p, _p]),
+    "seg3d_lattice_nearest_workspace_bytes": (ctypes.c_size_t, [_i64]),
+    "seg3d_lattice_nearest": (ctypes.c_int, [_p, _i64, _p, _i64, _p, _p, _i32, _p, _p, _p, _p, ctypes.c_size_t, _p]),
     "seg3d_pointwise_loss_workspace_bytes": (ctypes.c_size_t, [_i64]),
     "seg3d_focal_loss_fwd": (ctypes.c_int, [_p, _p, _i64, _i32, _i64, _f, _f, _p, _i32, _p, _p, ctypes.c_size_t, _p]),
     "seg3d_focal_loss_bwd": (ctypes.c_int, [_p, _p, _p, _p, _i64, _i32, _i64, _f, _f, _p, _i32, _p, _p]),
diff --git a/openseg3d_amd/csrc/lattice_nearest.hip b/openseg3d_amd/csrc/lattice_nearest.hip
--- /dev/null
+++ b/openseg3d_amd/csrc/lattice_nearest.hip
@@ -0,0 +1,226 @@
+#include "common.hpp"
+
+namespace {
+
+constexpr int kThreads = 256;
+constexpr int kMaxShell = 6;
+constexpr unsigned kCoordLimit = 1u << 18;
+constexpr unsigned kBatchLimit = 512;
+
+struct LatticeGeom {
+    float pitch[3];
+    float qpitch[3];
+    float lo[3];
+    int scale;
+};
+
+struct LatticeTables {
+    HashView cells;
+    unsigned long long* block_keys;
+    unsigned long long* block_masks;
+    uint64_t mask;
+};
+
+__device__ __forceinline__ uint64_t lattice_key(int b, int z, int y, int x) {
+    return ((uint64_t)(unsigned)b << 54) | ((uint64_t)(unsigned)z << 36) | ((uint64_t)(unsigned)y << 18) | (uint64_t)(unsigned)x;
+}
+
+__device__ __forceinline__ bool in_domain(int b, int z, int y, int x) {
+    return (unsigned)b < kBatchLimit && (unsigned)z < kCoordLimit && (unsigned)y < kCoordLimit && (unsigned)x < kCoordLimit;
+}
+
+__global__ __launch_bounds__(kThreads) void lattice_fill(unsigned long long* __restrict__ ones, int64_t n_ones,
+                                                         unsigned long long* __restrict__ zeros, int64_t n_zeros) {
+    const int64_t i = (int64_t)blockIdx.x * kThreads + threadIdx.x;
+    if (i < n_ones) ones[i] = SEG3D_HASH_EMPTY;
+    if (i < n_zeros) zeros[i] = 0ull;
+}
+
+__global__ __launch_bounds__(kThreads) void lattice_insert(const int32_t* __restrict__ coords, int64_t m, LatticeTables t) {
+    const int64_t i = (int64_t)blockIdx.x * kThreads + threadIdx.x;
+    if (i >= m) return;
+    const int4 c = reinterpret_cast<const int4*>(coords)[i];
+    if (!in_domain(c.x, c.y, c.z, c.w)) return;
+    const uint64_t slot = hash_insert_slot(t.cells, lattice_key(c.x, c.y, c.z, c.w));
+    atomicMin(reinterpret_cast<unsigned*>(&t.cells.vals[slot]), (unsigned)i);
+    HashView blocks;
+    blocks.keys = t.block_keys;
+    blocks.vals = nullptr;
+    blocks.mask = t.mask;
+    const uint64_t bslot = hash_insert_slot(blocks, lattice_key(c.x, c.y >> 2, c.z >> 2, c.w >> 2));
+    atomicOr(&t.block_masks[bslot], 1ull << (((c.y & 3) << 4) | ((c.z & 3) << 2) | (c.w & 3)));
+}
+
+struct Best {
+    float d2;
+    int32_t row;
+    __device__ __forceinline__ void offer(float d, int32_t r) {
+        if (d > 1e10f) return;
+        if (row < 0 || d < d2 || (d == d2 && r < row)) {
+            d2 = d;
+            row = r;
+        }
+    }
+};
+
+__device__ __forceinline__ float centre(int c, float pitch, float lo) { return ((float)c + 0.5f) * pitch + lo; }
+
+__global__ __launch_bounds__(kThreads) void lattice_query(const int32_t* __restrict__ fine, int64_t m,
+                                                          const int32_t* __restrict__ coarse, int64_t ma, LatticeGeom g,
+                                                          LatticeTables t, const int64_t* __restrict__ labels,
+                                                          int32_t* __restrict__ idx, int64_t* __restrict__ labels_out) {
+    const int64_t site = ((int64_t)blockIdx.x * kThreads + threadIdx.x) >> 6;
+    const int lane = threadIdx.x & 63;
+    if (site >= ma) return;
+    const int4 cq = reinterpret_cast<const int4*>(coarse)[site];
+    const int b = cq.x;
+    const int qc[3] = {cq.y, cq.z, cq.w};
+    float q[3];
+    int p2[3], bl[3], bh[3];
+    bool usable = (unsigned)b < kBatchLimit;
+    for (int a = 0; a < 3; ++a) {
+        q[a] = centre(qc[a], g.qpitch[a], g.lo[a]);
+        usable = usable && (unsigned)qc[a] < kCoordLimit;
+        const int64_t p = 2ll * g.scale * qc[a] + g.scale;
+        usable = usable && p < (int64_t)4 * kCoordLimit;
+        p2[a] = (int)p;
+        bl[a] = ((p2[a] - 1) >> 1) >> 2;
+        bh[a] = (p2[a] >> 1) >> 2;
+    }
+    Best best{1e10f, -1};
+    bool done = false;
+    for (int r = 0; usable && r <= kMaxShell && !done; ++r) {
+        const int wz = bh[0] - bl[0] + 1 + 2 * r, wy = bh[1] - bl[1] + 1 + 2 * r, wx = bh[2] - bl[2] + 1 + 2 * r;
+        const int total = wz * wy * wx;
+        for (int e0 = 0; e0 < total; e0 += 64) {
+            const int e = e0 + lane;
+            const int iz = e / (wy * wx), rem = e - iz * (wy * wx), iy = rem / wx, ix = rem - iy * wx;
+            const int bz = bl[0] - r + iz, by = bl[1] - r + iy, bx = bl[2] - r + ix;
+            unsigned long long occ = 0ull;
+            const bool earlier = r > 0 && iz >= 1 && iz < wz - 1 && iy >= 1 && iy < wy - 1 && ix >= 1 && ix < wx - 1;
+            if (e < total && !earlier && (unsigned)bz < (kCoordLimit >> 2) && (unsigned)by < (kCoordLimit >> 2) &&
+                (unsigned)bx < (kCoordLimit >> 2)) {
+                const uint64_t key = lattice_key(b, bz, by, bx);
+                uint64_t s = hash_mix(key) & t.mask;
+                for (;;) {
+                    const unsigned long long cur = t.block_keys[s];
+                    if (cur == key) {
+                        occ = t.block_masks[s];
+                        break;
+                    }
+                    if (cur == SEG3D_HASH_EMPTY) break;
+                    s = (s + 1) & t.mask;
+                }
+            }
+            unsigned long long any = __ballot(occ != 0ull);
+            while (any) {
+                const int src = __ffsll((long long)any) - 1;
+                any &= any - 1;
+                const unsigned lo32 = (unsigned)__shfl((int)(unsigned)occ, src, SEG3D_WAVE);
+                const unsigned hi32 = (unsigned)__shfl((int)(unsigned)(occ >> 32), src, SEG3D_WAVE);
+                const int sz = __shfl(bz, src, SEG3D_WAVE), sy = __shfl(by, src, SEG3D_WAVE), sx = __shfl(bx, src, SEG3D_WAVE);
+                if (!(((((unsigned long long)hi32 << 32) | lo32) >> lane) & 1ull)) continue;
+                const int z = 4 * sz + (lane >> 4), y = 4 * sy + ((lane >> 2) & 3), x = 4 * sx + (lane & 3);
+                const int32_t row = hash_lookup(t.cells, lattice_key(b, z, y, x));
+                if (row < 0) continue;
+                const float dx = q[2] - centre(x, g.pitch[2], g.lo[2]);
+                const float dy = q[1] - centre(y, g.pitch[1], g.lo[1]);
+                const float dz = q[0] - centre(z, g.pitch[0], g.lo[0]);
+                best.offer((dx * dx + dy * dy) + dz * dz, row);
+            }
+        }
+        for (int off = 32; off > 0; off >>= 1) {
+            const float od = __shfl_xor(best.d2, off, SEG3D_WAVE);
+            const int32_t orow = __shfl_xor(best.row, off, SEG3D_WAVE);
+            if (orow >= 0) best.offer(od, orow);
+        }
+        float bound = 1e30f;
+        for (int a = 0; a < 3; ++a) {
+            const int below = p2[a] - 8 * (bl[a] - r) + 1, above = 8 * (bh[a] + r + 1) + 1 - p2[a];
+            const float reach = 0.5f * (float)min(below, above) * g.pitch[a];
+            bound = fminf(bound, reach - 0x1p-21f * (fabsf(q[a]) + fabsf(g.lo[a]) + reach));
+        }
+        done = best.row >= 0 && bound > 0.f && best.d2 < bound * bound * 0.99999f;
+    }
+    if (!done) {
+        int64_t seg0 = 0, seg1 = 0;
+        for (int which = 0; which < 2; ++which) {
+            int64_t lo = 0, hi = m;
+            while (lo < hi) {
+                const int64_t mid = (lo + hi) >> 1;
+                if (fine[4 * mid] < b + which) lo = mid + 1;
+                else hi = mid;
+            }
+            if (which == 0) seg0 = lo;
+            else seg1 = lo;
+        }
+#pragma unroll 4
+        for (int64_t i = seg0 + lane; i < seg1; i += 64) {
+            const int4 c = reinterpret_cast<const int4*>(fine)[i];
+            const float dx = q[2] - centre(c.w, g.pitch[2], g.lo[2]);
+            const float dy = q[1] - centre(c.z, g.pitch[1], g.lo[1]);
+            const float dz = q[0] - centre(c.y, g.pitch[0], g.lo[0]);
+            best.offer((dx * dx + dy * dy) + dz * dz, (int32_t)i);
+        }
+        for (int off = 32; off > 0; off >>= 1) {
+            const float od = __shfl_xor(best.d2, off, SEG3D_WAVE);
+            const int32_t orow = __shfl_xor(best.row, off, SEG3D_WAVE);
+            if (orow >= 0) best.offer(od, orow);
+        }
+        if (best.row < 0) best.row = seg0 < m ? (int32_t)seg0 : (int32_t)(m - 1);
+    }
+    if (lane == 0) {
+        idx[site] = best.row;
+        if (labels_out) labels_out[site] = labels[best.row];
+    }
+}
+
+}
+
+extern "C" size_t seg3d_lattice_nearest_workspace_bytes(int64_t m) {
+    if (m < 0 || m >= (int64_t)0x3FFFFFF0) return 0;
+    const uint64_t cap = hash_capacity(m);
+    return (size_t)cap * (8 + 8 + 4 + 8);
+}
+
+extern "C" int seg3d_lattice_nearest(const int32_t* fine_coords, int64_t m, const int32_t* coarse_coords, int64_t ma,
+                                     const double* voxel_size, const double* origin, int32_t scale, const int64_t* labels,
+                                     int32_t* idx, int64_t* labels_out, void* workspace, size_t workspace_bytes,
+                                     void* stream) {
+    if (m < 0 || ma < 0 || scale < 1 || scale > 4096 || m >= (int64_t)0x3FFFFFF0 || ma >= (int64_t)0x01FFFFF0 || !voxel_size ||
+        !origin)
+        return SEG3D_EINVAL;
+    if (ma == 0) return SEG3D_OK;
+    if ((labels == nullptr) != (labels_out == nullptr)) return SEG3D_EINVAL;
+    if (m == 0 || !fine_coords || !coarse_coords || !idx) return SEG3D_EINVAL;
+    const size_t need = seg3d_lattice_nearest_workspace_bytes(m);
+    if (!workspace || workspace_bytes < need) return SEG3D_EWORKSPACE;
+    LatticeGeom g;
+    for (int a = 0; a < 3; ++a) {
+        if (!(voxel_size[2 - a] > 0.0)) return SEG3D_EINVAL;
+        g.pitch[a] = (float)(voxel_size[2 - a] * 1.0);
+        g.qpitch[a] = (float)(voxel_size[2 - a] * (double)scale);
+        g.lo[a] = (float)origin[2 - a];
+    }
+    g.scale = scale;
+    const uint64_t cap = hash_capacity(m);
+    unsigned long long* words = static_cast<unsigned long long*>(workspace);
+    LatticeTables t;
+    t.cells.keys = words;
+    t.block_keys = words + cap;
+    t.cells.vals = reinterpret_cast<int32_t*>(words + 2 * cap);
+    t.block_masks = words + 2 * cap + cap / 2;
+    t.cells.mask = cap - 1;
+    t.mask = cap - 1;
+    hipStream_t st = as_stream(stream);
+    const int64_t n_ones = (int64_t)(2 * cap + cap / 2);
+    hipLaunchKernelGGL(lattice_fill, dim3((unsigned)ceil_div64(n_ones, kThreads)), dim3(kThreads), 0, st, words, n_ones,
+                       t.block_masks, (int64_t)cap);
+    SEG3D_CHECK_LAUNCH();
+    hipLaunchKernelGGL(lattice_insert, dim3((unsigned)ceil_div64(m, kThreads)), dim3(kThreads), 0, st, fine_coords, m, t);
+    SEG3D_CHECK_LAUNCH();
+    hipLaunchKernelGGL(lattice_query, dim3((unsigned)ceil_div64(ma * 64, kThreads)), dim3(kThreads), 0, st, fine_coords, m,
+                       coarse_coords, ma, g, t, labels, idx, labels_out);
+    SEG3D_CHECK_LAUNCH();
+    return SEG3D_OK;
+}
diff --git a/openseg3d_amd/csrc/loss.hip b/openseg3d_amd/csrc/loss.hip
--- a/openseg3d_amd/csrc/loss.hip
+++ b/openseg3d_amd/csrc/loss.hip
@@ -1,9 +1,9 @@
-#include "common.hpp"
+#include "loss_rows.hpp"
 
 namespace {
 
-constexpr int kThreads = 256;
-constexpr int kMaxBlocks = 1024;
+constexpr int kThreads = kLossThreads;
+constexpr int kMaxBlocks = kCeMaxBlocks;
 
 __global__ __launch_bounds__(kThreads) void ce_fwd_kernel(const float* __restrict__ x, const int64_t* __restrict__ label,
                                                           int64_t n, int c, int64_t ignore_index, float keep_thresh,
@@ -12,67 +12,26 @@
     float loss = 0.f, cnt = 0.f;
     for (int64_t r = (int64_t)blockIdx.x * kThreads + threadIdx.x; r < n; r += (int64_t)gridDim.x * kThreads) {
         const float* row = x + r * c;
-        float m = row[0];
-        for (int j = 1; j < c; ++j) m = fmaxf(m, row[j]);
-        float s = 0.f;
-        for (int j = 0; j < c; ++j) s += expf(row[j] - m);
-        const float l = m + logf(s);
+        float m, s, l;
+        softmax_stats(row, c, &m, &s);
         const int64_t y = label[r];
-        bool counted = y != ignore_index && y >= 0 && y < c;
-        if (counted && keep_thresh > 0.f) counted = expf(row[y] - m) / s < keep_thresh;
+        const bool counted = ce_row(row, c, m, s, y, ignore_index, keep_thresh, &l);
         lse[r] = counted ? l : INFINITY;
         if (counted) {
             loss += l - row[y];
             cnt += 1.f;
         }
     }
-    for (int off = 32; off > 0; off >>= 1) {
-        loss += __shfl_xor(loss, off, SEG3D_WAVE);
-        cnt += __shfl_xor(cnt, off, SEG3D_WAVE);
-    }
-    __shared__ float red[2][kThreads / 64];
-    if ((threadIdx.x & 63) == 0) {
-        red[0][threadIdx.x >> 6] = loss;
-        red[1][threadIdx.x >> 6] = cnt;
-    }
-    __syncthreads();
+    block_sum2(&loss, &cnt);
     if (threadIdx.x == 0) {
-        float a = 0.f, b = 0.f;
-        for (int w = 0; w < kThreads / 64; ++w) {
-            a += red[0][w];
-            b += red[1][w];
-        }
-        part[2 * blockIdx.x] = a;
-        part[2 * blockIdx.x + 1] = b;
+        part[2 * blockIdx.x] = loss;
+        part[2 * blockIdx.x + 1] = cnt;
     }
 }
 
 __global__ __launch_bounds__(kThreads) void ce_finalize_kernel(const float* __restrict__ part, int nblocks,
                                                                float* __restrict__ out) {
-    float a = 0.f, b = 0.f;
-    for (int i = threadIdx.x; i < nblocks; i += kThreads) {
-        a += part[2 * i];
-        b += part[2 * i + 1];
-    }
-    for (int off = 32; off > 0; off >>= 1) {
-        a += __shfl_xor(a, off, SEG3D_WAVE);
-        b += __shfl_xor(b, off, SEG3D_WAVE);
-    }
-    __shared__ float red[2][kThreads / 64];
-    if ((threadIdx.x & 63) == 0) {
-        red[0][threadIdx.x >> 6] = a;
-        red[1][threadIdx.x >> 6] = b;
-    }
-    __syncthreads();
-    if (threadIdx.x == 0) {
-        float sa = 0.f, sb = 0.f;
-        for (int w = 0; w < kThreads / 64; ++w) {
-            sa += red[0][w];
-            sb += red[1][w];
-        }
-        out[0] = sb > 0.f ? sa / sb : 0.f;
-        out[1] = sb;
-    }
+    ce_finalize_block(part, nblocks, out);
 }
 
 __global__ __launch_bounds__(kThreads) void ce_bwd_kernel(const float* __restrict__ x, const int64_t* __restrict__ label,
diff --git a/openseg3d_amd/csrc/loss_rows.hpp b/openseg3d_amd/csrc/loss_rows.hpp
--- /dev/null
+++ b/openseg3d_amd/csrc/loss_rows.hpp
@@ -0,0 +1,58 @@
+#pragma once
+#include "common.hpp"
+
+constexpr int kLossThreads = 256;
+constexpr int kCeMaxBlocks = 1024;
+
+__device__ __forceinline__ void softmax_stats(const float* __restrict__ row, int c, float* m_out, float* s_out) {
+    float m = row[0];
+    for (int j = 1; j < c; ++j) m = fmaxf(m, row[j]);
+    float s = 0.f;
+    for (int j = 0; j < c; ++j) s += expf(row[j] - m);
+    *m_out = m;
+    *s_out = s;
+}
+
+__device__ __forceinline__ bool ce_row(const float* __restrict__ row, int c, float m, float s, int64_t y, int64_t ignore_index,
+                                       float keep_thresh, float* lse) {
+    *lse = m + logf(s);
+    bool counted = y != ignore_index && y >= 0 && y < c;
+    if (counted && keep_thresh > 0.f) counted = expf(row[y] - m) / s < keep_thresh;
+    return counted;
+}
+
+__device__ __forceinline__ void block_sum2(float* a, float* b) {
+    for (int off = 32; off > 0; off >>= 1) {
+        *a += __shfl_xor(*a, off, SEG3D_WAVE);
+        *b += __shfl_xor(*b, off, SEG3D_WAVE);
+    }
+    __shared__ float red[2][kLossThreads / 64];
+    __syncthreads();
+    if ((threadIdx.x & 63) == 0) {
+        red[0][threadIdx.x >> 6] = *a;
+        red[1][threadIdx.x >> 6] = *b;
+    }
+    __syncthreads();
+    if (threadIdx.x == 0) {
+        float sa = 0.f, sb = 0.f;
+        for (int w = 0; w < kLossThreads / 64; ++w) {
+            sa += red[0][w];
+            sb += red[1][w];
+        }
+        *a = sa;
+        *b = sb;
+    }
+}
+
+__device__ __forceinline__ void ce_finalize_block(const float* __restrict__ part, int nblocks, float* __restrict__ out) {
+    float a = 0.f, b = 0.f;
+    for (int i = threadIdx.x; i < nblocks; i += kLossThreads) {
+        a += part[2 * i];
+        b += part[2 * i + 1];
+    }
+    block_sum2(&a, &b);
+    if (threadIdx.x == 0) {
+        out[0] = b > 0.f ? a / b : 0.f;
+        out[1] = b;
+    }
+}
diff --git a/openseg3d_amd/csrc/lovasz.hip b/openseg3d_amd/csrc/lovasz.hip
--- a/openseg3d_amd/csrc/lovasz.hip
+++ b/openseg3d_amd/csrc/lovasz.hip
@@ -2,22 +2,35 @@
 
 #include <rocprim/device/device_radix_sort.hpp>
 
-#include "common.hpp"
+#include "loss_rows.hpp"
 
 namespace {
 
-constexpr int kThreads = 256;
+constexpr int kThreads = kLossThreads;
 constexpr int kItems = 8;
 constexpr int kChunk = kThreads * kItems;
 constexpr int kMaxClasses = 64;
-
-__device__ __forceinline__ void softmax_stats(const float* __restrict__ row, int c, float* m_out, float* s_out) {
-    float m = row[0];
-    for (int j = 1; j < c; ++j) m = fmaxf(m, row[j]);
-    float s = 0.f;
-    for (int j = 0; j < c; ++j) s += expf(row[j] - m);
-    *m_out = m;
-    *s_out = s;
+constexpr int kMaxHeads = 4;
+
+struct SortedHeads {
+    int n[kMaxHeads];
+    int64_t sorted0[kMaxHeads];
+    int64_t row0[kMaxHeads];
+    int count;
+    int stride;
+};
+
+__device__ __forceinline__ void lovasz_row_pairs(const float* __restrict__ row, int c, float m, float s, int64_t y,
+                                                 int64_t ignore_index, int r, int n, unsigned long long tag,
+                                                 unsigned long long* __restrict__ keys, uint32_t* __restrict__ vals) {
+    const bool valid = y != ignore_index;
+    for (int j = 0; j < c; ++j) {
+        const bool fg = valid && y == j;
+        const float err = valid ? fabsf((fg ? 1.f : 0.f) - expf(row[j] - m) / s) : 0.f;
+        const int64_t at = (int64_t)j * n + r;
+        keys[at] = tag | ((unsigned long long)j << 32) | __float_as_uint(err);
+        vals[at] = (uint32_t)r | (fg ? 0x80000000u : 0u);
+    }
 }
 
 __global__ __launch_bounds__(kThreads) void lovasz_keys(const float* __restrict__ x, const int64_t* __restrict__ label,
@@ -28,21 +41,15 @@
     const float* row = x + (int64_t)r * c;
     float m, s;
     softmax_stats(row, c, &m, &s);
-    const int64_t y = label[r];
-    const bool valid = y != ignore_index;
-    for (int j = 0; j < c; ++j) {
-        const bool fg = valid && y == j;
-        const float err = valid ? fabsf((fg ? 1.f : 0.f) - expf(row[j] - m) / s) : 0.f;
-        const int64_t at = (int64_t)j * n + r;
-        keys[at] = ((unsigned long long)j << 32) | __float_as_uint(err);
-        vals[at] = (uint32_t)r | (fg ? 0x80000000u : 0u);
-    }
-}
-
-__global__ __launch_bounds__(kThreads) void lovasz_count(const uint32_t* __restrict__ vals, int n, int nchunks,
+    lovasz_row_pairs(row, c, m, s, label[r], ignore_index, r, n, 0ull, keys, vals);
+}
+
+__global__ __launch_bounds__(kThreads) void lovasz_count(const uint32_t* __restrict__ vals, SortedHeads hs,
                                                          int* __restrict__ chunk_cnt ) {
-    const int seg = blockIdx.y, chunk = blockIdx.x;
-    const uint32_t* v = vals + (int64_t)seg * n;
+    const int head = blockIdx.z, seg = blockIdx.y, chunk = blockIdx.x;
+    const int n = hs.n[head];
+    if ((int64_t)chunk * kChunk >= n) return;
+    const uint32_t* v = vals + hs.sorted0[head] + (int64_t)seg * n;
     int cnt = 0;
     const int base = chunk * kChunk + threadIdx.x * kItems;
     for (int j = 0; j < kItems; ++j)
@@ -54,36 +61,41 @@
     if (threadIdx.x == 0) {
         int t = 0;
         for (int w = 0; w < kThreads / 64; ++w) t += red[w];
-        chunk_cnt[seg * nchunks + chunk] = t;
-    }
-}
-
-__global__ __launch_bounds__(64) void lovasz_offsets(const int* __restrict__ chunk_cnt, int nchunks,
+        chunk_cnt[((int64_t)head * gridDim.y + seg) * hs.stride + chunk] = t;
+    }
+}
+
+__global__ __launch_bounds__(64) void lovasz_offsets(const int* __restrict__ chunk_cnt, SortedHeads hs,
                                                      int* __restrict__ chunk_off, int* __restrict__ total) {
-    const int seg = blockIdx.x, lane = threadIdx.x;
+    const int head = blockIdx.y, seg = blockIdx.x, lane = threadIdx.x;
+    const int nchunks = (hs.n[head] + kChunk - 1) / kChunk;
+    const int64_t at = ((int64_t)head * gridDim.x + seg) * hs.stride;
     int carry = 0;
     for (int t0 = 0; t0 < nchunks; t0 += 64) {
         const int i = t0 + lane;
-        const int v = i < nchunks ? chunk_cnt[seg * nchunks + i] : 0;
+        const int v = i < nchunks ? chunk_cnt[at + i] : 0;
         int inc = v;
         for (int off = 1; off < 64; off <<= 1) {
             const int o = __shfl_up(inc, off, SEG3D_WAVE);
             if (lane >= off) inc += o;
         }
-        if (i < nchunks) chunk_off[seg * nchunks + i] = carry + inc - v;
+        if (i < nchunks) chunk_off[at + i] = carry + inc - v;
         carry += __shfl(inc, 63, SEG3D_WAVE);
     }
-    if (lane == 0) total[seg] = carry;
+    if (lane == 0) total[head * gridDim.x + seg] = carry;
 }
 
 __global__ __launch_bounds__(kThreads) void lovasz_grad(const unsigned long long* __restrict__ keys,
-                                                        const uint32_t* __restrict__ vals, int n, int c, int nchunks,
+                                                        const uint32_t* __restrict__ vals, SortedHeads hs, int c,
                                                         const int* __restrict__ chunk_off, const int* __restrict__ total,
                                                         float* __restrict__ coef ,
                                                         float* __restrict__ part ) {
-    const int seg = blockIdx.y, chunk = blockIdx.x;
+    const int head = blockIdx.z, seg = blockIdx.y, chunk = blockIdx.x;
+    const int n = hs.n[head];
+    if ((int64_t)chunk * kChunk >= n) return;
     const int cls = c - 1 - seg;
-    const int64_t seg0 = (int64_t)seg * n;
+    const int64_t seg0 = hs.sorted0[head] + (int64_t)seg * n;
+    const int64_t slot = ((int64_t)head * c + seg) * hs.stride + chunk;
     const int base = chunk * kChunk + threadIdx.x * kItems;
     uint32_t v[kItems];
     float err[kItems];
@@ -104,12 +116,13 @@
     __shared__ float wdot[kThreads / 64];
     if (lane == 63) wsum[wave] = inc;
     __syncthreads();
-    int before = chunk_off[seg * nchunks + chunk] + inc - mine;
+    int before = chunk_off[slot] + inc - mine;
     for (int w = 0; w < wave; ++w) before += wsum[w];
 
-    const float gts = (float)total[seg];
+    const float gts = (float)total[head * c + seg];
     float dot = 0.f;
     int cum = before;
+    float* coef_head = coef + hs.row0[head] * c;
     for (int j = 0; j < kItems; ++j) {
         const int k = base + j;
         if (k >= n) break;
@@ -120,7 +133,7 @@
         if (k > 0) g -= 1.f - (gts - (float)cum_prev) / (gts + (float)(k - cum_prev));
         dot += err[j] * g;
         const float sgn = err[j] == 0.f ? 0.f : (fg ? -1.f : 1.f);
-        coef[(int64_t)(v[j] & 0x7FFFFFFFu) * c + cls] = sgn * g;
+        coef_head[(int64_t)(v[j] & 0x7FFFFFFFu) * c + cls] = sgn * g;
     }
     for (int off = 32; off > 0; off >>= 1) dot += __shfl_xor(dot, off, SEG3D_WAVE);
     if (lane == 0) wdot[wave] = dot;
@@ -128,22 +141,21 @@
     if (threadIdx.x == 0) {
         float t = 0.f;
         for (int w = 0; w < kThreads / 64; ++w) t += wdot[w];
-        part[seg * nchunks + chunk] = t;
-    }
-}
-
-__global__ __launch_bounds__(kMaxClasses) void lovasz_finalize(const float* __restrict__ part, const int* __restrict__ total,
-                                                               int c, int nchunks, int mode,
-                                                               const int32_t* __restrict__ include,
-                                                               const float* __restrict__ class_weight,
-                                                               float* __restrict__ stats) {
+        part[slot] = t;
+    }
+}
+
+__device__ __forceinline__ void lovasz_finalize_head(const float* __restrict__ part, const int* __restrict__ total, int c,
+                                                     int nchunks, int stride, int mode, const int32_t* __restrict__ include,
+                                                     const float* __restrict__ class_weight, float* __restrict__ stats) {
     __shared__ float loss_c[kMaxClasses];
     __shared__ float w_c[kMaxClasses];
     const int cls = threadIdx.x;
+    __syncthreads();
     if (cls < c) {
         const int seg = c - 1 - cls;
         float s = 0.f;
-        for (int i = 0; i < nchunks; ++i) s += part[seg * nchunks + i];
+        for (int i = 0; i < nchunks; ++i) s += part[(int64_t)seg * stride + i];
         bool use = mode == 0 ? total[seg] > 0 : true;
         if (include) use = include[cls] != 0;
         const float w = use ? (class_weight ? class_weight[cls] : 1.f) : 0.f;
@@ -163,6 +175,14 @@
         stats[1] = (float)used;
         for (int j = 0; j < c; ++j) stats[2 + j] = (w_c[j] >= 0.f && used) ? w_c[j] / (float)used : 0.f;
     }
+}
+
+__global__ __launch_bounds__(kMaxClasses) void lovasz_finalize(const float* __restrict__ part, const int* __restrict__ total,
+                                                               int c, int nchunks, int mode,
+                                                               const int32_t* __restrict__ include,
+                                                               const float* __restrict__ class_weight,
+                                                               float* __restrict__ stats) {
+    lovasz_finalize_head(part, total, c, nchunks, nchunks, mode, include, class_weight, stats);
 }
 
 __global__ __launch_bounds__(kThreads) void lovasz_bwd(const float* __restrict__ x, const float* __restrict__ coef,
@@ -244,6 +264,10 @@
     float* part = ws.take<float>(cc);
     int* total = ws.take<int>((size_t)c);
     const int ni = (int)n;
+    SortedHeads hs = {};
+    hs.n[0] = ni;
+    hs.count = 1;
+    hs.stride = pl.nchunks;
     if (n > 0) {
         hipLaunchKernelGGL(lovasz_keys, dim3((unsigned)ceil_div64(n, kThreads)), dim3(kThreads), 0, st, logits, labels, ni, c,
                            ignore_index, k0, v0);
@@ -253,15 +277,15 @@
         size_t bytes = pl.sort_bytes;
         SEG3D_CHECK_HIP(rocprim::radix_sort_pairs_desc(sort_tmp, bytes, kb, vb, t, 0u, 32u + class_bits(c), st));
         const dim3 grid((unsigned)pl.nchunks, (unsigned)c);
-        hipLaunchKernelGGL(lovasz_count, grid, dim3(kThreads), 0, st, vb.current(), ni, pl.nchunks, chunk_cnt);
-        SEG3D_CHECK_LAUNCH();
-        hipLaunchKernelGGL(lovasz_offsets, dim3((unsigned)c), dim3(64), 0, st, chunk_cnt, pl.nchunks, chunk_off, total);
-        SEG3D_CHECK_LAUNCH();
-        hipLaunchKernelGGL(lovasz_grad, grid, dim3(kThreads), 0, st, kb.current(), vb.current(), ni, c, pl.nchunks, chunk_off,
-                           total, coef, part);
+        hipLaunchKernelGGL(lovasz_count, grid, dim3(kThreads), 0, st, vb.current(), hs, chunk_cnt);
+        SEG3D_CHECK_LAUNCH();
+        hipLaunchKernelGGL(lovasz_offsets, dim3((unsigned)c), dim3(64), 0, st, chunk_cnt, hs, chunk_off, total);
+        SEG3D_CHECK_LAUNCH();
+        hipLaunchKernelGGL(lovasz_grad, grid, dim3(kThreads), 0, st, kb.current(), vb.current(), hs, c, chunk_off, total, coef,
+                           part);
         SEG3D_CHECK_LAUNCH();
     } else {
-        hipLaunchKernelGGL(lovasz_offsets, dim3((unsigned)c), dim3(64), 0, st, chunk_cnt, 0, chunk_off, total);
+        hipLaunchKernelGGL(lovasz_offsets, dim3((unsigned)c), dim3(64), 0, st, chunk_cnt, hs, chunk_off, total);
         SEG3D_CHECK_LAUNCH();
     }
     hipLaunchKernelGGL(lovasz_finalize, dim3(1), dim3(kMaxClasses), 0, st, part, total, c, pl.nchunks, classes_mode, include,
@@ -280,3 +304,266 @@
     SEG3D_CHECK_LAUNCH();
     return SEG3D_OK;
 }
+
+namespace {
+
+struct RowHeads {
+    const float* x[kMaxHeads];
+    const int64_t* y[kMaxHeads];
+    float* dx[kMaxHeads];
+    int64_t row0[kMaxHeads];
+    int n[kMaxHeads];
+    int blk0[kMaxHeads];
+    int nblk[kMaxHeads];
+    float weight[kMaxHeads];
+    int count;
+};
+
+__device__ __forceinline__ int head_of_block(const RowHeads& hs, int gb) {
+    int h = 0;
+    while (h < hs.count - 1 && gb >= hs.blk0[h] + hs.nblk[h]) ++h;
+    return h;
+}
+
+__global__ __launch_bounds__(kThreads) void criterion_rows(RowHeads hs, int blk_base, int c, int64_t ignore_index,
+                                                           float keep_thresh, float* __restrict__ lse ,
+                                                           float* __restrict__ ce_part ,
+                                                           unsigned long long* __restrict__ keys, uint32_t* __restrict__ vals) {
+    const int gb = blk_base + blockIdx.x;
+    const int h = head_of_block(hs, gb);
+    const int n = hs.n[h];
+    const float* x = hs.x[h];
+    const int64_t* label = hs.y[h];
+    const int64_t row0 = hs.row0[h];
+    unsigned long long* hkeys = keys + row0 * c;
+    uint32_t* hvals = vals + row0 * c;
+    float loss = 0.f, cnt = 0.f;
+    for (int64_t r = (int64_t)(gb - hs.blk0[h]) * kThreads + threadIdx.x; r < n; r += (int64_t)hs.nblk[h] * kThreads) {
+        const float* row = x + r * c;
+        float m, s, l;
+        softmax_stats(row, c, &m, &s);
+        const int64_t y = label[r];
+        const bool counted = ce_row(row, c, m, s, y, ignore_index, keep_thresh, &l);
+        lse[row0 + r] = counted ? l : INFINITY;
+        if (counted) {
+            loss += l - row[y];
+            cnt += 1.f;
+        }
+        lovasz_row_pairs(row, c, m, s, y, ignore_index, (int)r, n, (unsigned long long)h << 37, hkeys, hvals);
+    }
+    block_sum2(&loss, &cnt);
+    if (threadIdx.x == 0) {
+        ce_part[2 * gb] = loss;
+        ce_part[2 * gb + 1] = cnt;
+    }
+}
+
+__global__ __launch_bounds__(kThreads) void criterion_finalize(RowHeads hs, SortedHeads sh, int c, const float* __restrict__ ce_part,
+                                                               const float* __restrict__ part, const int* __restrict__ total,
+                                                               float w_ce, float w_lovasz, float* __restrict__ stats) {
+    for (int h = 0; h < hs.count; ++h) {
+        float* st = stats + 1 + h * (4 + c);
+        ce_finalize_block(ce_part + 2 * hs.blk0[h], hs.nblk[h], st);
+        lovasz_finalize_head(part + (int64_t)h * c * sh.stride, total + h * c, c, (hs.n[h] + kChunk - 1) / kChunk, sh.stride, 0,
+                             nullptr, nullptr, st + 2);
+    }
+    if (threadIdx.x == 0) {
+        float loss = 0.f;
+        for (int h = 0; h < hs.count; ++h) {
+            const float* st = stats + 1 + h * (4 + c);
+            loss = loss + hs.weight[h] * st[0] * w_ce;
+            loss = loss + hs.weight[h] * st[2] * w_lovasz;
+        }
+        stats[0] = loss;
+    }
+}
+
+__global__ __launch_bounds__(kThreads) void criterion_bwd(RowHeads hs, int c, const float* __restrict__ lse,
+                                                          const float* __restrict__ coef, const float* __restrict__ stats,
+                                                          const float* __restrict__ gout, float w_ce, float w_lovasz) {
+    const int h = head_of_block(hs, blockIdx.x);
+    const int r = (blockIdx.x - hs.blk0[h]) * kThreads + threadIdx.x;
+    if (r >= hs.n[h]) return;
+    const float* st = stats + 1 + h * (4 + c);
+    const float g_ce = gout[0] * w_ce * hs.weight[h], g = gout[0] * w_lovasz * hs.weight[h];
+    const float cnt = st[1];
+    const float scale = cnt > 0.f ? g_ce / cnt : 0.f;
+    const float* row = hs.x[h] + (int64_t)r * c;
+    float m, s;
+    softmax_stats(row, c, &m, &s);
+    const float* cf = coef + (hs.row0[h] + r) * c;
+    const float* cs = st + 4;
+    float dot = 0.f;
+    for (int j = 0; j < c; ++j) dot += expf(row[j] - m) / s * (cf[j] * cs[j] * g);
+    const float l = lse[hs.row0[h] + r];
+    const int64_t y = hs.y[h][r];
+    float* out = hs.dx[h] + (int64_t)r * c;
+    for (int j = 0; j < c; ++j) {
+        float a = 0.f;
+        if (l != INFINITY) a = (expf(row[j] - l) - (j == y ? 1.f : 0.f)) * scale;
+        out[j] = a + expf(row[j] - m) / s * (cf[j] * cs[j] * g - dot);
+    }
+}
+
+constexpr unsigned kCriterionKeyBits = 40;
+
+struct CriterionPlan {
+    RowHeads rows;
+    SortedHeads sorted;
+    int64_t total_rows, pairs;
+    int blocks;
+    size_t sort_bytes;
+    Key *k0, *k1;
+    uint32_t *v0, *v1;
+    void* sort_tmp;
+    int *chunk_cnt, *chunk_off, *total;
+    float *part, *ce_part;
+    size_t rows_bytes;
+    size_t bytes;
+};
+
+bool criterion_plan(const seg3d_criterion_head* heads, int n_heads, int c, void* workspace, CriterionPlan* pl) {
+    if (!heads || n_heads < 1 || n_heads > kMaxHeads || c <= 0 || c > 32) return false;
+    int64_t rows = 0;
+    int blocks = 0, stride = 0;
+    for (int h = 0; h < n_heads; ++h) {
+        const int64_t n = heads[h].rows;
+        if (n < 0 || heads[h].row_offset != rows || (n > 0 && !heads[h].logits)) return false;
+        if ((rows + n) * c >= (int64_t)1 << 31) return false;
+        pl->rows.x[h] = heads[h].logits;
+        pl->rows.y[h] = heads[h].labels;
+        pl->rows.dx[h] = nullptr;
+        pl->rows.row0[h] = rows;
+        pl->rows.n[h] = (int)n;
+        pl->rows.weight[h] = heads[h].weight;
+        int nb = (int)ceil_div64(n, kThreads);
+        if (nb > kCeMaxBlocks) nb = kCeMaxBlocks;
+        pl->rows.blk0[h] = blocks;
+        pl->rows.nblk[h] = nb;
+        blocks += nb;
+        pl->sorted.n[h] = (int)n;
+        pl->sorted.row0[h] = rows;
+        const int nchunks = (int)ceil_div64(n, kChunk);
+        if (nchunks > stride) stride = nchunks;
+        rows += n;
+    }
+    int64_t behind = 0;
+    for (int h = n_heads - 1; h >= 0; --h) {
+        pl->sorted.sorted0[h] = behind;
+        behind += (int64_t)pl->sorted.n[h] * c;
+    }
+    pl->rows.count = pl->sorted.count = n_heads;
+    pl->sorted.stride = stride;
+    pl->total_rows = rows;
+    pl->pairs = rows * c;
+    pl->blocks = blocks;
+    const size_t t = (size_t)pl->pairs, cc = (size_t)n_heads * c * (size_t)stride;
+    WsCarver ws(workspace);
+    pl->k0 = ws.take<Key>(t);
+    pl->v0 = ws.take<uint32_t>(t);
+    pl->ce_part = ws.take<float>((size_t)2 * (blocks > 0 ? blocks : 1));
+    pl->rows_bytes = ws.off;
+    pl->k1 = ws.take<Key>(t);
+    pl->v1 = ws.take<uint32_t>(t);
+    pl->chunk_cnt = ws.take<int>(cc);
+    pl->chunk_off = ws.take<int>(cc);
+    pl->part = ws.take<float>(cc);
+    pl->total = ws.take<int>((size_t)n_heads * c);
+    pl->sort_tmp = ws.take<char>(0);
+    pl->sort_bytes = 0;
+    pl->bytes = ws.off + 256;
+    return true;
+}
+
+bool criterion_sort_scratch(CriterionPlan* pl) {
+    if (pl->pairs > 0) {
+        rocprim::double_buffer<Key> k(nullptr, nullptr);
+        rocprim::double_buffer<uint32_t> v(nullptr, nullptr);
+        size_t bytes = 0;
+        if (rocprim::radix_sort_pairs_desc(nullptr, bytes, k, v, (size_t)pl->pairs, 0u, kCriterionKeyBits) != hipSuccess) return false;
+        pl->sort_bytes = bytes;
+        pl->bytes += align_up(bytes, 256);
+    }
+    return true;
+}
+
+}
+
+extern "C" size_t seg3d_criterion_workspace_bytes(const seg3d_criterion_head* heads, int32_t n_heads, int32_t c) {
+    CriterionPlan pl;
+    return criterion_plan(heads, n_heads, c, nullptr, &pl) && criterion_sort_scratch(&pl) ? pl.bytes : 0;
+}
+
+extern "C" int seg3d_criterion_rows_fwd(const seg3d_criterion_head* heads, int32_t n_heads, int32_t head_begin, int32_t head_end,
+                                        int32_t c, int64_t ignore_index, float keep_thresh, float* lse, void* workspace,
+                                        size_t workspace_bytes, void* stream) {
+    CriterionPlan pl;
+    if (!criterion_plan(heads, n_heads, c, workspace, &pl)) return SEG3D_EINVAL;
+    if (head_begin < 0 || head_end > n_heads || head_begin > head_end) return SEG3D_EINVAL;
+    if (!workspace || workspace_bytes < pl.rows_bytes) return SEG3D_EWORKSPACE;
+    for (int h = head_begin; h < head_end; ++h)
+        if (heads[h].rows > 0 && !heads[h].labels) return SEG3D_EINVAL;
+    if (head_begin == head_end) return SEG3D_OK;
+    const int b0 = pl.rows.blk0[head_begin], b1 = pl.rows.blk0[head_end - 1] + pl.rows.nblk[head_end - 1];
+    if (b1 == b0) return SEG3D_OK;
+    if (!lse) return SEG3D_EINVAL;
+    hipLaunchKernelGGL(criterion_rows, dim3((unsigned)(b1 - b0)), dim3(kThreads), 0, as_stream(stream), pl.rows, b0, c, ignore_index,
+                       keep_thresh, lse, pl.ce_part, pl.k0, pl.v0);
+    SEG3D_CHECK_LAUNCH();
+    return SEG3D_OK;
+}
+
+extern "C" int seg3d_criterion_finish_fwd(const seg3d_criterion_head* heads, int32_t n_heads, int32_t c, float w_ce,
+                                          float w_lovasz, float* coef, float* stats, void* workspace, size_t workspace_bytes,
+                                          void* stream) {
+    CriterionPlan pl;
+    if (!criterion_plan(heads, n_heads, c, workspace, &pl) || !stats) return SEG3D_EINVAL;
+    if (!criterion_sort_scratch(&pl)) return SEG3D_ELAUNCH;
+    if (!workspace || workspace_bytes < pl.bytes) return SEG3D_EWORKSPACE;
+    if (pl.pairs > 0 && !coef) return SEG3D_EINVAL;
+    hipStream_t st = as_stream(stream);
+    if (pl.pairs > 0) {
+        rocprim::double_buffer<Key> kb(pl.k0, pl.k1);
+        rocprim::double_buffer<uint32_t> vb(pl.v0, pl.v1);
+        size_t bytes = pl.sort_bytes;
+        SEG3D_CHECK_HIP(rocprim::radix_sort_pairs_desc(pl.sort_tmp, bytes, kb, vb, (size_t)pl.pairs, 0u, kCriterionKeyBits, st));
+        const dim3 grid((unsigned)pl.sorted.stride, (unsigned)c, (unsigned)n_heads);
+        hipLaunchKernelGGL(lovasz_count, grid, dim3(kThreads), 0, st, vb.current(), pl.sorted, pl.chunk_cnt);
+        SEG3D_CHECK_LAUNCH();
+        hipLaunchKernelGGL(lovasz_offsets, dim3((unsigned)c, (unsigned)n_heads), dim3(64), 0, st, pl.chunk_cnt, pl.sorted,
+                           pl.chunk_off, pl.total);
+        SEG3D_CHECK_LAUNCH();
+        hipLaunchKernelGGL(lovasz_grad, grid, dim3(kThreads), 0, st, kb.current(), vb.current(), pl.sorted, c, pl.chunk_off,
+                           pl.total, coef, pl.part);
+        SEG3D_CHECK_LAUNCH();
+    } else {
+        hipLaunchKernelGGL(lovasz_offsets, dim3((unsigned)c, (unsigned)n_heads), dim3(64), 0, st, pl.chunk_cnt, pl.sorted,
+                           pl.chunk_off, pl.total);
+        SEG3D_CHECK_LAUNCH();
+    }
+    hipLaunchKernelGGL(criterion_finalize, dim3(1), dim3(kThreads), 0, st, pl.rows, pl.sorted, c, pl.ce_part, pl.part, pl.total,
+                       w_ce, w_lovasz, stats);
+    SEG3D_CHECK_LAUNCH();
+    return SEG3D_OK;
+}
+
+extern "C" int seg3d_criterion_bwd(const seg3d_criterion_head* heads, float* const* dlogits, int32_t n_heads, int32_t c,
+                                   float w_ce, float w_lovasz, const float* lse, const float* coef, const float* stats,
+                                   const float* grad_out, void* stream) {
+    CriterionPlan pl;
+    if (!criterion_plan(heads, n_heads, c, nullptr, &pl) || !dlogits || !stats || !grad_out) return SEG3D_EINVAL;
+    if (pl.total_rows == 0) return SEG3D_OK;
+    if (!lse || !coef) return SEG3D_EINVAL;
+    int blocks = 0;
+    for (int h = 0; h < n_heads; ++h) {
+        if (pl.rows.n[h] > 0 && (!dlogits[h] || !heads[h].labels)) return SEG3D_EINVAL;
+        pl.rows.dx[h] = dlogits[h];
+        pl.rows.blk0[h] = blocks;
+        pl.rows.nblk[h] = (int)ceil_div64(pl.rows.n[h], kThreads);
+        blocks += pl.rows.nblk[h];
+    }
+    hipLaunchKernelGGL(criterion_bwd, dim3((unsigned)blocks), dim3(kThreads), 0, as_stream(stream), pl.rows, c, lse, coef, stats,
+                       grad_out, w_ce, w_lovasz);
+    SEG3D_CHECK_LAUNCH();
+    return SEG3D_OK;
+}
diff --git a/openseg3d_amd/csrc/voxelize.hip b/openseg3d_amd/csrc/voxelize.hip
--- a/openseg3d_amd/csrc/voxelize.hip
+++ b/openseg3d_amd/csrc/voxelize.hip
@@ -273,7 +273,7 @@
     return cart2polar_impl<double>(points, n_points, row_stride, xyz_col, out, stream);
 }
 
-int seg3d_abi_version(void) { return 47; }
+int seg3d_abi_version(void) { return 48; }
 
 namespace {
 thread_local char g_last_error[320] = "";
diff --git a/openseg3d_amd/losses.py b/openseg3d_amd/losses.py
--- a/openseg3d_amd/losses.py
+++ b/openseg3d_amd/losses.py
@@ -225,6 +225,24 @@
     return losses
 
 
+def _batched_plan(criterion, heads):
+    if len(criterion) != 2:
+        return None
+    (ce, w_ce), (lovasz, w_lovasz) = criterion
+    if type(ce) is not OHEMCrossEntropyLoss or type(lovasz) is not LovaszLoss:
+        return None
+    if ce.class_weight is not None or ce.keep_ratio or not ce.keep_thresh:
+        return None
+    if (lovasz.loss_type != "multi_class" or lovasz.per_image or lovasz.classes != "present" or lovasz.class_weight is not None
+            or lovasz.loss_weight != 1.0 or lovasz.ignore_index != ce.ignore_index):
+        return None
+    if len(heads) > ops.CRITERION_MAX_HEADS or any(not ops.criterion_fits(x, y) for x, y, _ in heads):
+        return None
+    if len({x.shape[1] for x, _, _ in heads}) != 1 or len({x.device for x, _, _ in heads}) != 1:
+        return None
+    return {"ignore_index": ce.ignore_index, "keep_thresh": ce.keep_thresh, "w_ce": w_ce, "w_lovasz": w_lovasz}
+
+
 AUX_OVERLAP = os.environ.get("SEG3D_AUX_OVERLAP", "1") != "0"
 
 
@@ -240,13 +258,23 @@
             aux_gt = ops.aux_voxel_labels(pred_result["voxel_coords"], pred_result["aux_voxel_coords"],
                                           data_dict["voxel_labels"], data_dict["batch_size"], cfg.DATASET.VOXEL_SIZE,
                                           cfg.DATASET.POINT_CLOUD_RANGE)
+    heads = [(pred_result["point_out"], data_dict["point_labels"], 1.0)]
+    if "voxel_out" in pred_result:
+        heads.append((pred_result["voxel_out"], data_dict["voxel_labels"], 1.0))
+    plan = _batched_plan(criterion, heads + ([(pred_result["aux_voxel_out"], aux_gt, cfg.MODEL.AUX_LOSS_WEIGHT)]
+                                             if aux_gt is not None else []))
+    if plan is not None:
+        if aux_gt is not None:
+            def aux_labels():
+                if side is not None:
+                    main.wait_stream(side)
+                return aux_gt
+            heads.append((pred_result["aux_voxel_out"], aux_labels, cfg.MODEL.AUX_LOSS_WEIGHT))
+        return ops.criterion_batched(heads, **plan)
     loss = 0
-    for fn, w in criterion:
-        loss = loss + fn(pred_result["point_out"], data_dict["point_labels"]) * w
-    if "voxel_out" in pred_result:
-        voxel_gt = data_dict["voxel_labels"]
+    for x, y, _ in heads:
         for fn, w in criterion:
-            loss = loss + fn(pred_result["voxel_out"], voxel_gt) * w
+            loss = loss + fn(x, y) * w
     if aux_gt is not None:
         if side is not None:
             main.wait_stream(side)
diff --git a/openseg3d_amd/ops.py b/openseg3d_amd/ops.py
--- a/openseg3d_amd/ops.py
+++ b/openseg3d_amd/ops.py
@@ -1910,8 +1910,42 @@
     return (batch_col.view(-1, 1) == ids.view(1, -1)).sum(dim=0).cumsum(0).to(torch.int32)
 
 
+_F64x3 = ctypes.c_double * 3
+
+
+def lattice_nearest(voxel_coords, coarse_coords, voxel_size, point_cloud_range, scale, labels=None):
+    _need_gpu(voxel_coords, coarse_coords, labels)
+    fine, coarse = _i32c(voxel_coords), _i32c(coarse_coords)
+    if fine.dim() != 2 or fine.shape[1] != 4 or coarse.dim() != 2 or coarse.shape[1] != 4:
+        raise _lib.Seg3dError("lattice_nearest: [*, 4] (b, z, y, x) coordinates expected")
+    m, ma = fine.shape[0], coarse.shape[0]
+    idx = torch.empty((ma,), dtype=torch.int32, device=fine.device)
+    out = None
+    if labels is not None:
+        if labels.dtype != torch.int64 or labels.dim() != 1 or labels.shape[0] != m:
+            raise _lib.Seg3dError("lattice_nearest: labels must be int64 [M]")
+        labels = labels.contiguous()
+        out = torch.empty((ma,), dtype=torch.int64, device=fine.device)
+    ws_bytes = _lib.query("seg3d_lattice_nearest_workspace_bytes", m)
+    ws = _workspace(ws_bytes, fine.device)
+    _lib.call("seg3d_lattice_nearest", _ptr(fine), m, _ptr(coarse), ma, _F64x3(*(float(v) for v in voxel_size)),
+              _F64x3(*(float(v) for v in point_cloud_range[0:3])), int(scale), _ptr(labels), _ptr(idx), _ptr(out), _ptr(ws),
+              ws_bytes, _stream())
+    return idx, out
+
+
+def _lattice_lookup_ok(voxel_coords, aux_voxel_coords, voxel_labels, aux_scale):
+    ints = (torch.int32, torch.int64)
+    return (voxel_coords.is_cuda and aux_voxel_coords.is_cuda and voxel_labels.is_cuda and voxel_coords.dtype in ints
+            and aux_voxel_coords.dtype in ints and voxel_labels.dtype == torch.int64 and voxel_labels.dim() == 1
+            and voxel_labels.shape[0] == voxel_coords.shape[0] and voxel_coords.shape[0] > 0
+            and float(aux_scale).is_integer() and 1 <= aux_scale <= 4096)
+
+
 def aux_voxel_labels(voxel_coords, aux_voxel_coords, voxel_labels, batch_size, voxel_size, point_cloud_range,
                      aux_scale=8.0):
+    if _lattice_lookup_ok(voxel_coords, aux_voxel_coords, voxel_labels, aux_scale):
+        return lattice_nearest(voxel_coords, aux_voxel_coords, voxel_size, point_cloud_range, int(aux_scale), voxel_labels)[1]
     centers = get_voxel_centers(voxel_coords[:, 1:], 1.0, voxel_size, point_cloud_range).contiguous()
     aux_centers = get_voxel_centers(aux_voxel_coords[:, 1:], aux_scale, voxel_size, point_cloud_range).contiguous()
     off = _sample_offsets_nosync(voxel_coords[:, 0], batch_size)
@@ -2071,6 +2105,90 @@
         gg = _f32c(g.reshape(1))
         _lib.call("seg3d_lovasz_softmax_bwd", _ptr(x), _ptr(coef), _ptr(stats), _ptr(gg), n, c, _ptr(dx), _stream())
         return dx, None, None, None, None, None
+
+
+class CriterionHead(ctypes.Structure):
+    _fields_ = [("logits", ctypes.c_void_p), ("labels", ctypes.c_void_p), ("row_offset", ctypes.c_int64),
+                ("rows", ctypes.c_int64), ("weight", ctypes.c_float)]
+
+
+CRITERION_MAX_HEADS, CRITERION_MAX_CLASSES = 4, 32
+
+
+class _CriterionFn(torch.autograd.Function):
+
+    @staticmethod
+    def forward(ctx, meta, *logits):
+        labels, weights, ignore_index, keep_thresh, w_ce, w_lovasz = meta
+        xs = [_f32c(x) for x in logits]
+        c, dev = xs[0].shape[1], xs[0].device
+        table = (CriterionHead * len(xs))()
+        rows = 0
+        for h, x in enumerate(xs):
+            table[h] = CriterionHead(x.data_ptr(), None, rows, x.shape[0], float(weights[h]))
+            rows += x.shape[0]
+        tp = ctypes.cast(table, ctypes.c_void_p)
+        ws_bytes = _lib.query("seg3d_criterion_workspace_bytes", tp, len(xs), c)
+        if ws_bytes == 0:
+            raise _lib.Seg3dError(f"seg3d_criterion_workspace_bytes = 0: {len(xs)} heads, {rows} rows, {c} classes")
+        ws = _workspace(ws_bytes, dev)
+        lse = torch.empty((rows,), dtype=torch.float32, device=dev)
+        coef = torch.empty((rows, c), dtype=torch.float32, device=dev)
+        stats = torch.empty((1 + len(xs) * (4 + c),), dtype=torch.float32, device=dev)
+        labs, issued = [], 0
+
+        def issue(upto):
+            _lib.call("seg3d_criterion_rows_fwd", tp, len(xs), issued, upto, c, int(ignore_index), float(keep_thresh), _ptr(lse),
+                      _ptr(ws), ws_bytes, _stream())
+
+        for h, y in enumerate(labels):
+            if callable(y):
+                if h > issued:
+                    issue(h)
+                    issued = h
+                y = y()
+            if y.dtype != torch.int64 or y.dim() != 1 or y.shape[0] != xs[h].shape[0] or y.device != dev:
+                raise ValueError("criterion: int64 [n] labels on the logits' device, one per row")
+            y = y.contiguous()
+            labs.append(y)
+            table[h].labels = y.data_ptr()
+        issue(len(xs))
+        _lib.call("seg3d_criterion_finish_fwd", tp, len(xs), c, float(w_ce), float(w_lovasz), _ptr(coef), _ptr(stats), _ptr(ws),
+                  ws_bytes, _stream())
+        ctx.save_for_backward(lse, coef, stats, *xs, *labs)
+        ctx.meta = (len(xs), c, tuple(float(w) for w in weights), float(w_ce), float(w_lovasz))
+        return stats[0]
+
+    @staticmethod
+    def backward(ctx, g):
+        n_heads, c, weights, w_ce, w_lovasz = ctx.meta
+        lse, coef, stats = ctx.saved_tensors[:3]
+        xs, labs = ctx.saved_tensors[3:3 + n_heads], ctx.saved_tensors[3 + n_heads:]
+        table = (CriterionHead * n_heads)()
+        rows = 0
+        for h, x in enumerate(xs):
+            table[h] = CriterionHead(x.data_ptr(), labs[h].data_ptr(), rows, x.shape[0], weights[h])
+            rows += x.shape[0]
+        dxs = [torch.empty_like(x) for x in xs]
+        ptrs = (ctypes.c_void_p * n_heads)(*[dx.data_ptr() for dx in dxs])
+        gg = _f32c(g.reshape(1))
+        _lib.call("seg3d_criterion_bwd", ctypes.cast(table, ctypes.c_void_p), ctypes.cast(ptrs, ctypes.c_void_p), n_heads, c,
+                  w_ce, w_lovasz, _ptr(lse), _ptr(coef), _ptr(stats), _ptr(gg), _stream())
+        return (None, *dxs)
+
+
+def criterion_fits(logits, labels):
+    return (logits.is_cuda and logits.dim() == 2 and logits.dtype == torch.float32 and 0 < logits.shape[1] <= CRITERION_MAX_CLASSES
+            and (callable(labels) or _loss_args_ok(logits, labels, CRITERION_MAX_CLASSES)))
+
+
+def criterion_batched(heads, ignore_index=255, keep_thresh=0.7, w_ce=1.0, w_lovasz=1.0):
+    heads = list(heads)
+    if not 1 <= len(heads) <= CRITERION_MAX_HEADS or any(not criterion_fits(x, y) for x, y, _ in heads) or \
+            len({x.shape[1] for x, _, _ in heads}) != 1 or len({x.device for x, _, _ in heads}) != 1:
+        raise ValueError("criterion_batched: 1..4 heads of float32 [n, C <= 32] logits with int64 [n] labels on one GPU")
+    meta = ([y for _, y, _ in heads], [w for _, _, w in heads], ignore_index, keep_thresh if keep_thresh else 0.0, w_ce, w_lovasz)
+    return _CriterionFn.apply(meta, *[x for x, _, _ in heads])
 
 
 def lovasz_softmax(logits, labels, ignore_index=255, classes="present", class_weight=None):
```

After: 4.271 million points/s, median of 6. +2.2%, better.
